# yang-song/score_sde_pytorch

Hardware: AMD Instinct MI355X
Metric: pc_sampler_images_per_sec (higher is better)
Workload: dtype f32 via 3-way bf16 split, fp32 accumulate (the 1x1 / NIN / Linear GEMMs and the attention forward as exact-fp32 products on the BF16 matrix pipe, fp32 softmax; 3x3 convolutions and the attention backward on the fp32-MFMA kernels); 1 GPU; configs/ve/cifar10_ncsnpp_continuous PC sampler (reverse_diffusion+langevin), batch 256/GPU, N=1000, 32x32; 1 step = 1 PC iteration = 2 U-Net evaluations; batch_per_gpu=256, sde_steps=1000, state_finite=True, matrix_mode=bf16x6, parallelism=replicas x1 (no collectives)

## Files before the change

### include/ssde.h

```cpp
#ifndef SSDE_H_
#define SSDE_H_

#include <stddef.h>
#include <stdint.h>

#ifdef __cplusplus
extern "C" {
#endif

#define SSDE_ABI_VERSION 13

enum {
  SSDE_PRO_NONE = 0,
  SSDE_PRO_GN = 1,
  SSDE_PRO_GN_SILU = 2,
  SSDE_PRO_SILU = 3
};

typedef struct ssde_src {
  const float* p0;
  const float* p1;
  int32_t c0, c1;
  int32_t pro_mode;
  int32_t gn_groups;
  const float* gn_mean;
  const float* gn_rstd;
  const float* gn_gamma;
  const float* gn_beta;
  uint32_t drop_thresh;
  float drop_scale;
  const uint32_t* drop_seed;
  uint32_t drop_salt;
  int32_t _pad;
} ssde_src;

typedef struct ssde_conv_args {
  ssde_src main;
  ssde_src aux;
  const float* w_main;
  const float* w_aux;
  int32_t n, h_in, w_in;
  int32_t h_out, w_out, c_out;
  int32_t ksize;
  int32_t stride;
  int32_t pad;
  int32_t tile;
  const float* bias;
  const float* chan_add;
  int32_t chan_add_ld;
  int32_t resid_post;
  const float* resid;
  float out_scale;
  uint32_t flags;
  float* dst;
  float* gn_part;
  float* wino_v;
  const float* gn_in_part0;
  const float* gn_in_part1;
  int32_t gn_in_slices0, gn_in_slices1;
  float gn_in_eps;
  int32_t pad_end;
  float* wino_ws;
  int64_t wino_ws_floats;
} ssde_conv_args;

enum { SSDE_CONVF_V_GIVEN = 1u,
       SSDE_CONVF_BF16X6 = 2u,
       SSDE_CONVF_NO_KSPLIT = 4u,
       SSDE_CONVF_BKC8 = 8u,
       SSDE_CONVF_GEMM_PIPE = 16u,
       SSDE_CONVF_NO_GEMM_PIPE = 32u,
       SSDE_CONVF_X6_BM64 = 64u,
       SSDE_CONVF_X6_PF2 = 128u,
       SSDE_CONVF_NO_SMALL_COUT = 256u,
       SSDE_CONVF_X6_WIDE = 512u,
       SSDE_CONVF_X6_NO_WIDE = 1024u,
       SSDE_CONVF_KSPLIT2 = 2048u,
       SSDE_CONVF_KSPLIT4 = 4096u };
enum { SSDE_TILE_AUTO = 0, SSDE_TILE_256x64 = 1, SSDE_TILE_128x64 = 2, SSDE_TILE_64x64 = 3, SSDE_TILE_256x32 = 4,
       SSDE_TILE_WINOGRAD = 5,
       SSDE_TILE_WINOGRAD4 = 6,
       SSDE_TILE_WINOGRAD4R = 9,
       SSDE_TILE_WINOGRAD4P = 10 };

typedef struct ssde_gn_stats_args {
  const float* p0; const float* p1; int32_t c0, c1;
  int32_t n, hw, groups; float eps;
  float* mean; float* rstd;
  float* scratch;
  int32_t slices;
  uint32_t flags;
} ssde_gn_stats_args;
enum { SSDE_GNSTATF_ANY_WIDTH = 1u };

typedef struct ssde_gn_apply_args {
  ssde_src src;
  int32_t n, hw;
  float* dst;
} ssde_gn_apply_args;

typedef struct ssde_gn_apply_bwd_args {
  ssde_src src;
  const float* dy;
  int32_t n, hw;
  float* sums;
  float* dgamma; float* dbeta;
  float* scratch;
  int32_t slices; int32_t _pad0;
  float* g0; float* g1;
  int32_t acc0, acc1;
} ssde_gn_apply_bwd_args;

typedef struct ssde_gn_finalize_args {
  const float* part0; const float* part1;
  int32_t c0, c1, slices0, slices1;
  int32_t n, groups; float eps; int32_t _pad0;
  float* mean; float* rstd;
} ssde_gn_finalize_args;

#define SSDE_FIR_MAX_TAPS 16
enum {
  SSDE_FIRF_GENERAL = 1,
  SSDE_FIRF_TILED = 2
};
typedef struct ssde_upfirdn_args {
  ssde_src src;
  int32_t n, h_in, w_in, c;
  int32_t h_out, w_out;
  int32_t up, down, pad0, pad1;
  int32_t kh, kw;
  float k[16];
  float* dst;
  int32_t accumulate;
  uint32_t flags;
  float* dst2;
  const float* taps;
} ssde_upfirdn_args;

#define SSDE_ATTN_L_MAX 16384
typedef struct ssde_attn_args {
  const float* qkv; float* dst;
  int32_t n, l, c; float scale;
  uint32_t flags;
  int32_t _pad0;
} ssde_attn_args;
enum { SSDE_ATTNF_BF16X6 = 1u,
       SSDE_ATTNF_STREAM = 2u };
enum { SSDE_ATTN_ROUTE_F32 = 0, SSDE_ATTN_ROUTE_X6 = 1, SSDE_ATTN_ROUTE_STREAM = 2 };

typedef struct ssde_embed_args {
  const float* cond;
  const float* w;
  float* dst;
  int32_t n, dim, kind, _pad0;
} ssde_embed_args;

typedef struct ssde_to_nhwc_args {
  const float* src; float* dst; int32_t n, c, h, w, c_pad; float a, b;
  int32_t mode;
  const float* v;
} ssde_to_nhwc_args;
typedef struct ssde_to_nchw_args {
  const float* src; float* dst; int32_t n, c, h, w, c_src;
  int32_t mode;
  const float* v;
  float alpha;
  int32_t accumulate;
} ssde_to_nchw_args;

typedef struct ssde_bias_act_args {
  const float* src; const float* bias; float* dst;
  int64_t numel; int32_t channels; int32_t inner;
  int32_t act;
  float alpha, scale;
  int32_t grad;
  const float* ref;
} ssde_bias_act_args;

typedef struct ssde_sumsq_args {
  const float* a; const float* b; float* out_a; float* out_b; int32_t n, per;
} ssde_sumsq_args;
typedef struct ssde_randn_args {
  float* dst; int64_t numel; uint64_t seed; const int32_t* step_ptr; int32_t stream_id; int32_t _pad0;
  const uint64_t* seed_ptr;
} ssde_randn_args;
typedef struct ssde_langevin_args {
  float* x; float* x_mean; const float* grad; const float* noise;
  const float* grad_sumsq; const float* noise_sumsq;
  const float* alpha_tab; const int32_t* step_ptr;
  int32_t n, per; float snr; int32_t _pad0;
} ssde_langevin_args;
typedef struct ssde_predictor_args {
  float* x; float* x_mean; const float* score; const float* noise;
  const float* coef; const int32_t* step_ptr;
  int64_t numel;
} ssde_predictor_args;
typedef struct ssde_sample_update_args {
  const float* x; const float* y; const float* z; const float* a; const float* b; const float* c;
  float* x_mean; float* x_out; int32_t n; int32_t per;
} ssde_sample_update_args;
typedef struct ssde_fill_args {
  float* dst; const float* tab; const int32_t* step_ptr; int32_t n; int32_t _pad0;
} ssde_fill_args;
typedef struct ssde_step_inc_args { int32_t* step_ptr; int32_t delta; int32_t _pad0; } ssde_step_inc_args;
typedef struct ssde_project_args {
  float* x; float* x_mean; const float* data; const float* mask; const float* noise;
  const float* coef; const int32_t* step_ptr;
  int32_t n, c, hw;
  int32_t use_matrix;
  float M[9], invM[9];
} ssde_project_args;



typedef struct ssde_wgrad_args {
  ssde_src src;
  const float* g;
  int32_t g_ld, g_off;
  int32_t n, h_in, w_in, h_out, w_out;
  int32_t c_out;
  int32_t ksize;
  int32_t stride, pad;
  int32_t cin_store;
  int32_t transpose_out;
  int32_t splits;
  float scale;
  uint32_t flags;
  float* dw;
  float* scratch;
  int64_t scratch_floats;
  const float* v_pre;
  int32_t pad_end;
  int32_t _pad0;
} ssde_wgrad_args;

enum { SSDE_WGRADF_DIRECT = 1u,
       SSDE_WGRADF_F2 = 2u,
       SSDE_WGRADF_F4_FORCE = 4u,
       SSDE_WGRADF_NO_STREAMK = 8u,
       SSDE_WGRADF_NO_XCD_ORDER = 16u,
       SSDE_WGRADF_1X1_CHUNKED = 32u,
       SSDE_WGRADF_XVEC1 = 64u };

typedef struct ssde_colsum_args {
  const float* g; int32_t g_ld, g_off;
  int32_t n, hw, c;
  float scale;
  float* per_sample;
  int32_t ps_ld, ps_off;
  float* total;
  float* total2;
  float* scratch;
  uint32_t flags;
  int32_t _pad0;
} ssde_colsum_args;
enum { SSDE_COLSUMF_DEFER = 1u };

#define SSDE_FINISH_JOBS 16
typedef struct ssde_colsum_job {
  const float* part;
  float* per_sample;
  float* total; float* total2;
  int32_t n, slices, c, ps_ld, ps_off, _pad0;
} ssde_colsum_job;
typedef struct ssde_colsum_finish_args { int32_t count, _pad0; ssde_colsum_job job[SSDE_FINISH_JOBS]; } ssde_colsum_finish_args;
typedef struct ssde_gn_bwd_job {
  const float* scratch;
  float* dgamma; float* dbeta;
  int32_t rows, c;
} ssde_gn_bwd_job;
typedef struct ssde_gn_bwd_finish_args { int32_t count, _pad0; ssde_gn_bwd_job job[SSDE_FINISH_JOBS]; } ssde_gn_bwd_finish_args;

typedef struct ssde_gn_bwd_reduce_args {
  ssde_src src;
  const float* dp;
  int32_t n, hw;
  float* sums;
  float* dgamma; float* dbeta;
  float* scratch;
  int32_t slices;
  uint32_t flags;
  float* g0; float* g1;
  int32_t acc0, acc1;
  float scale; int32_t _pad1;
} ssde_gn_bwd_reduce_args;

enum { SSDE_GNBWDF_THREE_KERNELS = 1u,
       SSDE_GNBWDF_DEFER_PARAMS = 2u };

typedef struct ssde_prologue_bwd_args {
  ssde_src src;
  const float* dp;
  int32_t dp_ld, dp_off;
  int32_t n, hw;
  const float* sums;
  float scale;
  int32_t acc0, acc1;
  float* g0; float* g1;
} ssde_prologue_bwd_args;

typedef struct ssde_attn_bwd_args {
  const float* qkv;
  const float* o;
  const float* d_o;
  float* dqkv;
  float* stats;
  int32_t n, l, c; float scale;
} ssde_attn_bwd_args;

typedef struct ssde_perturb_args {
  const float* x; const float* z; const float* a; const float* s; float* dst; int32_t n, per;
} ssde_perturb_args;
typedef struct ssde_dsm_loss_args {
  const float* score; const float* z; const float* s; const float* g2;
  float* dscore;
  float* losses;
  float* loss;
  int32_t n, per; int32_t reduce_mean; int32_t likelihood_weighting;
  float grad_scale;
  int32_t _pad0;
} ssde_dsm_loss_args;

typedef struct ssde_sumsq_flat_args { const float* x; int64_t numel; float* partial; float* out; } ssde_sumsq_flat_args;
typedef struct ssde_adam_args {
  float* p; const float* g; float* m; float* v; float* ema;
  int64_t numel;
  const float* hyper;
  const float* gnorm_sq;
} ssde_adam_args;

typedef struct ssde_memset_args { void* dst; int64_t bytes; int32_t value; int32_t _pad0; } ssde_memset_args;

enum { SSDE_PACK_CONV3 = 1, SSDE_PACK_WINO3 = 2, SSDE_PACK_MATRIX = 3, SSDE_PACK_VECTOR = 4,
       SSDE_PACK_WINO4 = 5 ,
       SSDE_PACK_WINO4R = 6 ,
       SSDE_PACK_WINO4P = 7  };
typedef struct ssde_pack_desc {
  const float* src;
  const float* src2;
  float* dst;
  int32_t kind;
  int32_t cout, cin;
  int32_t cout_l, cin_l;
  int32_t flags;
  int32_t r_off, c_off;
  int64_t n;
} ssde_pack_desc;
typedef struct ssde_pack_args { const ssde_pack_desc* table; int32_t count; int32_t kind; int64_t max_n; } ssde_pack_args;
typedef struct ssde_axpy_args {
  const float* x; const float* gate; float* dst; int64_t numel; float alpha; int32_t acc;
} ssde_axpy_args;

typedef struct ssde_rk_coefs { double v[7]; } ssde_rk_coefs;
typedef struct ssde_rk_combine_args {
  const double* y; const double* k; int64_t n; int32_t terms; int32_t _pad0; ssde_rk_coefs coef; double* dst; float* dst32;
  int64_t n32;
} ssde_rk_combine_args;
typedef struct ssde_rk_error_args {
  const double* y; const double* y_new; const double* k; int64_t n; ssde_rk_coefs coef; double atol, rtol;
  double* partial; int32_t partial_len; int32_t _pad0; double* out;
} ssde_rk_error_args;
#define SSDE_RK_MAX_TERMS 12
#define SSDE_RK_MAX_ROWS 13
typedef struct ssde_rk_combine_rows_args {
  const double* y; const double* k; int64_t n; int32_t terms; int32_t _pad0; double coef[SSDE_RK_MAX_TERMS]; double* dst; float* dst32;
  int64_t n32;
} ssde_rk_combine_rows_args;
typedef struct ssde_rk_error_rows_args {
  const double* y; const double* y_new; const double* k; int64_t n; int32_t rows; int32_t pair;
  double coef[SSDE_RK_MAX_ROWS]; double coef2[SSDE_RK_MAX_ROWS]; double h_abs; double atol, rtol;
  double* partial; int32_t partial_len; int32_t _pad0; double* out;
} ssde_rk_error_rows_args;
typedef struct ssde_ode_dyn {
  float label, std;
  float a, g2;
  double* dst;
} ssde_ode_dyn;
typedef struct ssde_pf_drift_args {
  const float* x; const float* score; double* dst; int64_t numel; float a, g2;
  const ssde_ode_dyn* dyn;
} ssde_pf_drift_args;
typedef struct ssde_hutch_div_args {
  const float* gx; const float* eps; double* dst; int64_t dst_off; int32_t n; int32_t per; float a, g2;
  const ssde_ode_dyn* dyn;
} ssde_hutch_div_args;

int ssde_conv2d(const ssde_conv_args* a, void* stream);
int ssde_groupnorm_stats(const ssde_gn_stats_args* a, void* stream);
int ssde_gn_finalize(const ssde_gn_finalize_args* a, void* stream);
int ssde_gn_apply(const ssde_gn_apply_args* a, void* stream);
int ssde_gn_apply_bwd(const ssde_gn_apply_bwd_args* a, void* stream);
int ssde_conv_gn_slices(const ssde_conv_args* a);
int64_t ssde_conv_ws_floats(const ssde_conv_args* a);
int ssde_upfirdn2d(const ssde_upfirdn_args* a, void* stream);
int ssde_attention(const ssde_attn_args* a, void* stream);
int ssde_attention_route(const ssde_attn_args* a);
int ssde_embed(const ssde_embed_args* a, void* stream);
int ssde_to_nhwc(const ssde_to_nhwc_args* a, void* stream);
int ssde_to_nchw(const ssde_to_nchw_args* a, void* stream);
int ssde_fused_bias_act(const ssde_bias_act_args* a, void* stream);
int ssde_sumsq(const ssde_sumsq_args* a, void* stream);
int ssde_randn(const ssde_randn_args* a, void* stream);
int ssde_langevin_update(const ssde_langevin_args* a, void* stream);
int ssde_predictor_update(const ssde_predictor_args* a, void* stream);
int ssde_sample_update(const ssde_sample_update_args* a, void* stream);
int ssde_fill_from_table(const ssde_fill_args* a, void* stream);
int ssde_step_inc(const ssde_step_inc_args* a, void* stream);
int ssde_project_update(const ssde_project_args* a, void* stream);
int ssde_rk_combine(const ssde_rk_combine_args* a, void* stream);
int ssde_rk_error_norm(const ssde_rk_error_args* a, void* stream);
int ssde_rk_combine_rows(const ssde_rk_combine_rows_args* a, void* stream);
int ssde_rk_error_norm_rows(const ssde_rk_error_rows_args* a, void* stream);
int ssde_pf_drift(const ssde_pf_drift_args* a, void* stream);
int ssde_hutch_div(const ssde_hutch_div_args* a, void* stream);
int ssde_conv_wgrad(const ssde_wgrad_args* a, void* stream);
int ssde_wgrad_wants_winograd4(const ssde_wgrad_args* a);
int ssde_colsum(const ssde_colsum_args* a, void* stream);
int ssde_colsum_finish(const ssde_colsum_finish_args* a, void* stream);
int ssde_gn_bwd_finish(const ssde_gn_bwd_finish_args* a, void* stream);
int ssde_gn_bwd_scratch_rows(const ssde_gn_bwd_reduce_args* a);
int ssde_gn_bwd_reduce(const ssde_gn_bwd_reduce_args* a, void* stream);
int ssde_prologue_bwd(const ssde_prologue_bwd_args* a, void* stream);
int ssde_attention_bwd(const ssde_attn_bwd_args* a, void* stream);
int ssde_perturb(const ssde_perturb_args* a, void* stream);
int ssde_dsm_loss(const ssde_dsm_loss_args* a, void* stream);
int ssde_sumsq_flat(const ssde_sumsq_flat_args* a, void* stream);
int ssde_adam_clip_ema(const ssde_adam_args* a, void* stream);
int ssde_memset(const ssde_memset_args* a, void* stream);
int ssde_axpy(const ssde_axpy_args* a, void* stream);
int ssde_pack_weights(const ssde_pack_args* a, void* stream);

enum {
  SSDE_OP_CONV = 1, SSDE_OP_GN_STATS = 2, SSDE_OP_UPFIRDN = 3, SSDE_OP_ATTN = 4, SSDE_OP_EMBED = 5,
  SSDE_OP_TO_NHWC = 6, SSDE_OP_TO_NCHW = 7, SSDE_OP_BIAS_ACT = 8, SSDE_OP_SUMSQ = 9, SSDE_OP_RANDN = 10,
  SSDE_OP_LANGEVIN = 11, SSDE_OP_PREDICTOR = 12, SSDE_OP_FILL = 13, SSDE_OP_STEP_INC = 14,
  SSDE_OP_WGRAD = 15, SSDE_OP_COLSUM = 16, SSDE_OP_GN_BWD_REDUCE = 17, SSDE_OP_PROLOGUE_BWD = 18,
  SSDE_OP_ATTN_BWD = 19, SSDE_OP_PERTURB = 20, SSDE_OP_DSM_LOSS = 21, SSDE_OP_SUMSQ_FLAT = 22,
  SSDE_OP_ADAM = 23, SSDE_OP_MEMSET = 24, SSDE_OP_AXPY = 25, SSDE_OP_PACK = 26, SSDE_OP_PROJECT = 27,
  SSDE_OP_GN_FINALIZE = 28, SSDE_OP_PF_DRIFT = 29, SSDE_OP_HUTCH_DIV = 30, SSDE_OP_COLSUM_FINISH = 31, SSDE_OP_GN_BWD_FINISH = 32,
  SSDE_OP_GN_APPLY = 33, SSDE_OP_GN_APPLY_BWD = 34
};
typedef struct ssde_op {
  int32_t kind; int32_t flops_class;
  union {
    ssde_conv_args conv; ssde_gn_stats_args gn; ssde_upfirdn_args fir; ssde_attn_args attn;
    ssde_embed_args embed; ssde_to_nhwc_args to_nhwc; ssde_to_nchw_args to_nchw;
    ssde_bias_act_args bias_act; ssde_sumsq_args sumsq; ssde_randn_args randn;
    ssde_langevin_args langevin; ssde_predictor_args predictor; ssde_fill_args fill;
    ssde_step_inc_args step_inc;
    ssde_wgrad_args wgrad; ssde_colsum_args colsum; ssde_gn_bwd_reduce_args gn_bwd; ssde_prologue_bwd_args pro_bwd;
    ssde_attn_bwd_args attn_bwd; ssde_perturb_args perturb; ssde_dsm_loss_args dsm_loss;
    ssde_sumsq_flat_args sumsq_flat; ssde_adam_args adam; ssde_memset_args memset; ssde_axpy_args axpy;
    ssde_pack_args pack; ssde_project_args project; ssde_gn_finalize_args gn_fin;
    ssde_pf_drift_args pf_drift; ssde_hutch_div_args hutch_div;
    ssde_colsum_finish_args colsum_fin; ssde_gn_bwd_finish_args gn_bwd_fin;
    ssde_gn_apply_args gn_apply; ssde_gn_apply_bwd_args gn_apply_bwd;
  } u;
} ssde_op;

int ssde_program_run(const ssde_op* ops, int32_t n_ops, void* stream);
int ssde_program_run_timed(const ssde_op* ops, int32_t n_ops, void* stream, float* ms);
int ssde_graph_capture(const ssde_op* ops, int32_t n_ops, void* stream, void** graph_out);
int ssde_graph_launch(void* graph, void* stream);
int ssde_graph_destroy(void* graph);

enum { SSDE_REGION_ZERO = 0,
       SSDE_REGION_CONST = 1 };
enum { SSDE_RELOC_OP = 0, SSDE_RELOC_REFRESH_OP = 1, SSDE_RELOC_REGION = 2 };
enum { SSDE_PLAN_UNET = 0, SSDE_PLAN_PC = 1, SSDE_PLAN_TRAIN = 2,
       SSDE_PLAN_ODE = 3,
       SSDE_PLAN_LIKELIHOOD = 4 };
enum { SSDE_IO_X = 0, SSDE_IO_COND = 1, SSDE_IO_SIGMA = 2, SSDE_IO_STD = 3, SSDE_IO_OUT = 4, SSDE_IO_XMEAN = 5,
       SSDE_IO_STEP = 6, SSDE_IO_SEED = 7,
       SSDE_IO_BATCH = 8, SSDE_IO_Z = 9, SSDE_IO_A = 10, SSDE_IO_S = 11, SSDE_IO_G2 = 12, SSDE_IO_LOSS = 13, SSDE_IO_HYPER = 14,
       SSDE_IO_DROP_SEED = 15, SSDE_IO_GOUT = 16, SSDE_IO_GX = 17, SSDE_IO_GRAD = 18, SSDE_IO_PARAMS = 19,
       SSDE_IO_ODE_DYN = 20, SSDE_IO_ODE_K = 21, SSDE_IO_ODE_STATE = 22, SSDE_IO_ODE_PROBE = 23, SSDE_IO_SLOTS = 24 };
#define SSDE_ODE_PARTIALS 1024
typedef struct ssde_plan_header {
  char magic[8];
  int32_t abi_version, sizeof_op;
  int32_t n_regions, n_ops, n_refresh_ops, n_relocs, n_params;
  int32_t kind;
  int32_t batch, channels, height, width;
  int32_t nfe_per_iteration;
  int32_t sde_steps;
  int32_t io[SSDE_IO_SLOTS];
  int32_t seg[4];
  int64_t n_flat;
  int64_t data_bytes;
// ... 50 lines not shown
```

### score_sde_pytorch_amd/_lib.py

```python
import ctypes as C
import os

_HERE = os.path.dirname(os.path.abspath(__file__))
LIB_PATH = os.environ.get("SSDE_LIB_PATH") or os.path.join(_HERE, "libssde_hip.so")
ABI_VERSION = 13

PRO_NONE, PRO_GN, PRO_GN_SILU, PRO_SILU = 0, 1, 2, 3
TILE_AUTO, TILE_256x64, TILE_128x64, TILE_64x64, TILE_256x32, TILE_WINOGRAD, TILE_WINOGRAD4 = 0, 1, 2, 3, 4, 5, 6
TILE_WINOGRAD4R = 9
TILE_WINOGRAD4P = 10
TILES_WINOGRAD4 = (TILE_WINOGRAD4, TILE_WINOGRAD4R, TILE_WINOGRAD4P)
CONVF_V_GIVEN, CONVF_BF16X6, CONVF_NO_KSPLIT, CONVF_BKC8, CONVF_GEMM_PIPE, CONVF_NO_GEMM_PIPE, CONVF_X6_BM64, CONVF_X6_PF2, \
    CONVF_NO_SMALL_COUT, CONVF_X6_WIDE, CONVF_X6_NO_WIDE, CONVF_KSPLIT2, CONVF_KSPLIT4 = 1, 2, 4, 8, 16, 32, 64, 128, 256, 512, 1024, 2048, 4096
WGRADF_DIRECT, WGRADF_F2, WGRADF_F4_FORCE, WGRADF_NO_STREAMK, WGRADF_NO_XCD_ORDER, WGRADF_1X1_CHUNKED, WGRADF_XVEC1 = 1, 2, 4, 8, 16, 32, 64
GNBWDF_THREE_KERNELS, GNBWDF_DEFER_PARAMS = 1, 2
(OP_CONV, OP_GN_STATS, OP_UPFIRDN, OP_ATTN, OP_EMBED, OP_TO_NHWC, OP_TO_NCHW, OP_BIAS_ACT, OP_SUMSQ,
 OP_RANDN, OP_LANGEVIN, OP_PREDICTOR, OP_FILL, OP_STEP_INC, OP_WGRAD, OP_COLSUM, OP_GN_BWD_REDUCE, OP_PROLOGUE_BWD,
 OP_ATTN_BWD, OP_PERTURB, OP_DSM_LOSS, OP_SUMSQ_FLAT, OP_ADAM, OP_MEMSET, OP_AXPY, OP_PACK, OP_PROJECT,
 OP_GN_FINALIZE, OP_PF_DRIFT, OP_HUTCH_DIV, OP_COLSUM_FINISH, OP_GN_BWD_FINISH, OP_GN_APPLY, OP_GN_APPLY_BWD) = range(1, 35)
GNSTATF_ANY_WIDTH = 1
FIRF_GENERAL, FIRF_TILED = 1, 2
FIR_MAX_TAPS = 16
FINISH_JOBS = 16
COLSUMF_DEFER = 1
PACK_CONV3, PACK_WINO3, PACK_MATRIX, PACK_VECTOR, PACK_WINO4, PACK_WINO4R, PACK_WINO4P = 1, 2, 3, 4, 5, 6, 7

_fp = C.c_void_p


class Src(C.Structure):
    _fields_ = [("p0", _fp), ("p1", _fp), ("c0", C.c_int32), ("c1", C.c_int32),
                ("pro_mode", C.c_int32), ("gn_groups", C.c_int32),
                ("gn_mean", _fp), ("gn_rstd", _fp), ("gn_gamma", _fp), ("gn_beta", _fp),
                ("drop_thresh", C.c_uint32), ("drop_scale", C.c_float), ("drop_seed", _fp),
                ("drop_salt", C.c_uint32), ("_pad", C.c_int32)]


class ConvArgs(C.Structure):
    _fields_ = [("main", Src), ("aux", Src), ("w_main", _fp), ("w_aux", _fp),
                ("n", C.c_int32), ("h_in", C.c_int32), ("w_in", C.c_int32),
                ("h_out", C.c_int32), ("w_out", C.c_int32), ("c_out", C.c_int32),
                ("ksize", C.c_int32), ("stride", C.c_int32), ("pad", C.c_int32), ("tile", C.c_int32),
                ("bias", _fp), ("chan_add", _fp), ("chan_add_ld", C.c_int32), ("resid_post", C.c_int32),
                ("resid", _fp), ("out_scale", C.c_float), ("flags", C.c_uint32), ("dst", _fp), ("gn_part", _fp), ("wino_v", _fp),
                ("gn_in_part0", _fp), ("gn_in_part1", _fp), ("gn_in_slices0", C.c_int32), ("gn_in_slices1", C.c_int32),
                ("gn_in_eps", C.c_float), ("pad_end", C.c_int32), ("wino_ws", _fp), ("wino_ws_floats", C.c_int64)]


class GnStatsArgs(C.Structure):
    _fields_ = [("p0", _fp), ("p1", _fp), ("c0", C.c_int32), ("c1", C.c_int32),
                ("n", C.c_int32), ("hw", C.c_int32), ("groups", C.c_int32), ("eps", C.c_float),
                ("mean", _fp), ("rstd", _fp), ("scratch", _fp), ("slices", C.c_int32), ("flags", C.c_uint32)]


class GnApplyArgs(C.Structure):
    _fields_ = [("src", Src), ("n", C.c_int32), ("hw", C.c_int32), ("dst", _fp)]


class GnApplyBwdArgs(C.Structure):
    _fields_ = [("src", Src), ("dy", _fp), ("n", C.c_int32), ("hw", C.c_int32), ("sums", _fp), ("dgamma", _fp), ("dbeta", _fp),
                ("scratch", _fp), ("slices", C.c_int32), ("_pad0", C.c_int32), ("g0", _fp), ("g1", _fp),
                ("acc0", C.c_int32), ("acc1", C.c_int32)]


class RkCombineArgs(C.Structure):
    _fields_ = [("y", _fp), ("k", _fp), ("n", C.c_int64), ("terms", C.c_int32), ("_pad0", C.c_int32), ("coef", C.c_double * 7),
                ("dst", _fp), ("dst32", _fp), ("n32", C.c_int64)]


class RkErrorArgs(C.Structure):
    _fields_ = [("y", _fp), ("y_new", _fp), ("k", _fp), ("n", C.c_int64), ("coef", C.c_double * 7), ("atol", C.c_double),
                ("rtol", C.c_double), ("partial", _fp), ("partial_len", C.c_int32), ("_pad0", C.c_int32), ("out", _fp)]


class RkCombineRowsArgs(C.Structure):
    _fields_ = [("y", _fp), ("k", _fp), ("n", C.c_int64), ("terms", C.c_int32), ("_pad0", C.c_int32), ("coef", C.c_double * 12),
                ("dst", _fp), ("dst32", _fp), ("n32", C.c_int64)]


class RkErrorRowsArgs(C.Structure):
    _fields_ = [("y", _fp), ("y_new", _fp), ("k", _fp), ("n", C.c_int64), ("rows", C.c_int32), ("pair", C.c_int32),
                ("coef", C.c_double * 13), ("coef2", C.c_double * 13), ("h_abs", C.c_double), ("atol", C.c_double), ("rtol", C.c_double),
                ("partial", _fp), ("partial_len", C.c_int32), ("_pad0", C.c_int32), ("out", _fp)]


class PfDriftArgs(C.Structure):
    _fields_ = [("x", _fp), ("score", _fp), ("dst", _fp), ("numel", C.c_int64), ("a", C.c_float), ("g2", C.c_float), ("dyn", _fp)]


class OdeDyn(C.Structure):
    _fields_ = [("label", C.c_float), ("std", C.c_float), ("a", C.c_float), ("g2", C.c_float), ("dst", _fp)]


class HutchDivArgs(C.Structure):
    _fields_ = [("gx", _fp), ("eps", _fp), ("dst", _fp), ("dst_off", C.c_int64), ("n", C.c_int32), ("per", C.c_int32),
                ("a", C.c_float), ("g2", C.c_float), ("dyn", _fp)]


class GnFinalizeArgs(C.Structure):
    _fields_ = [("part0", _fp), ("part1", _fp), ("c0", C.c_int32), ("c1", C.c_int32), ("slices0", C.c_int32), ("slices1", C.c_int32),
                ("n", C.c_int32), ("groups", C.c_int32), ("eps", C.c_float), ("_pad0", C.c_int32), ("mean", _fp), ("rstd", _fp)]


class UpfirdnArgs(C.Structure):
    _fields_ = [("src", Src), ("n", C.c_int32), ("h_in", C.c_int32), ("w_in", C.c_int32), ("c", C.c_int32),
                ("h_out", C.c_int32), ("w_out", C.c_int32),
                ("up", C.c_int32), ("down", C.c_int32), ("pad0", C.c_int32), ("pad1", C.c_int32),
                ("kh", C.c_int32), ("kw", C.c_int32), ("k", C.c_float * 16), ("dst", _fp),
                ("accumulate", C.c_int32), ("flags", C.c_uint32), ("dst2", _fp), ("taps", _fp)]


class AttnArgs(C.Structure):
    _fields_ = [("qkv", _fp), ("dst", _fp), ("n", C.c_int32), ("l", C.c_int32), ("c", C.c_int32), ("scale", C.c_float),
                ("flags", C.c_uint32), ("_pad0", C.c_int32)]


class EmbedArgs(C.Structure):
    _fields_ = [("cond", _fp), ("w", _fp), ("dst", _fp), ("n", C.c_int32), ("dim", C.c_int32),
                ("kind", C.c_int32), ("_pad0", C.c_int32)]


class ToNhwcArgs(C.Structure):
    _fields_ = [("src", _fp), ("dst", _fp), ("n", C.c_int32), ("c", C.c_int32), ("h", C.c_int32), ("w", C.c_int32),
                ("c_pad", C.c_int32), ("a", C.c_float), ("b", C.c_float), ("mode", C.c_int32), ("v", _fp)]


class ToNchwArgs(C.Structure):
    _fields_ = [("src", _fp), ("dst", _fp), ("n", C.c_int32), ("c", C.c_int32), ("h", C.c_int32), ("w", C.c_int32),
                ("c_src", C.c_int32), ("mode", C.c_int32), ("v", _fp), ("alpha", C.c_float), ("accumulate", C.c_int32)]


class BiasActArgs(C.Structure):
    _fields_ = [("src", _fp), ("bias", _fp), ("dst", _fp), ("numel", C.c_int64), ("channels", C.c_int32),
                ("inner", C.c_int32), ("act", C.c_int32), ("alpha", C.c_float), ("scale", C.c_float), ("grad", C.c_int32),
                ("ref", _fp)]


class SumsqArgs(C.Structure):
    _fields_ = [("a", _fp), ("b", _fp), ("out_a", _fp), ("out_b", _fp), ("n", C.c_int32), ("per", C.c_int32)]


class RandnArgs(C.Structure):
    _fields_ = [("dst", _fp), ("numel", C.c_int64), ("seed", C.c_uint64), ("step_ptr", _fp),
                ("stream_id", C.c_int32), ("_pad0", C.c_int32), ("seed_ptr", _fp)]


class LangevinArgs(C.Structure):
    _fields_ = [("x", _fp), ("x_mean", _fp), ("grad", _fp), ("noise", _fp), ("grad_sumsq", _fp), ("noise_sumsq", _fp),
                ("alpha_tab", _fp), ("step_ptr", _fp), ("n", C.c_int32), ("per", C.c_int32), ("snr", C.c_float),
                ("_pad0", C.c_int32)]


class PredictorArgs(C.Structure):
    _fields_ = [("x", _fp), ("x_mean", _fp), ("score", _fp), ("noise", _fp), ("coef", _fp), ("step_ptr", _fp),
                ("numel", C.c_int64)]


class SampleUpdateArgs(C.Structure):
    _fields_ = [("x", _fp), ("y", _fp), ("z", _fp), ("a", _fp), ("b", _fp), ("c", _fp), ("x_mean", _fp), ("x_out", _fp),
                ("n", C.c_int32), ("per", C.c_int32)]


class FillArgs(C.Structure):
    _fields_ = [("dst", _fp), ("tab", _fp), ("step_ptr", _fp), ("n", C.c_int32), ("_pad0", C.c_int32)]


class StepIncArgs(C.Structure):
    _fields_ = [("step_ptr", _fp), ("delta", C.c_int32), ("_pad0", C.c_int32)]


class ProjectArgs(C.Structure):
    _fields_ = [("x", _fp), ("x_mean", _fp), ("data", _fp), ("mask", _fp), ("noise", _fp), ("coef", _fp), ("step_ptr", _fp),
                ("n", C.c_int32), ("c", C.c_int32), ("hw", C.c_int32), ("use_matrix", C.c_int32),
                ("M", C.c_float * 9), ("invM", C.c_float * 9)]


class WgradArgs(C.Structure):
    _fields_ = [("src", Src), ("g", _fp), ("g_ld", C.c_int32), ("g_off", C.c_int32),
                ("n", C.c_int32), ("h_in", C.c_int32), ("w_in", C.c_int32), ("h_out", C.c_int32), ("w_out", C.c_int32),
                ("c_out", C.c_int32), ("ksize", C.c_int32), ("stride", C.c_int32), ("pad", C.c_int32),
                ("cin_store", C.c_int32), ("transpose_out", C.c_int32), ("splits", C.c_int32), ("scale", C.c_float),
                ("flags", C.c_uint32), ("dw", _fp), ("scratch", _fp), ("scratch_floats", C.c_int64), ("v_pre", _fp),
                ("pad_end", C.c_int32), ("_pad0", C.c_int32)]


class ColsumArgs(C.Structure):
    _fields_ = [("g", _fp), ("g_ld", C.c_int32), ("g_off", C.c_int32), ("n", C.c_int32), ("hw", C.c_int32),
                ("c", C.c_int32), ("scale", C.c_float), ("per_sample", _fp), ("ps_ld", C.c_int32), ("ps_off", C.c_int32),
                ("total", _fp), ("total2", _fp), ("scratch", _fp), ("flags", C.c_uint32), ("_pad0", C.c_int32)]


class ColsumJob(C.Structure):
    _fields_ = [("part", _fp), ("per_sample", _fp), ("total", _fp), ("total2", _fp), ("n", C.c_int32), ("slices", C.c_int32),
                ("c", C.c_int32), ("ps_ld", C.c_int32), ("ps_off", C.c_int32), ("_pad0", C.c_int32)]


class ColsumFinishArgs(C.Structure):
    _fields_ = [("count", C.c_int32), ("_pad0", C.c_int32), ("job", ColsumJob * FINISH_JOBS)]


class GnBwdJob(C.Structure):
    _fields_ = [("scratch", _fp), ("dgamma", _fp), ("dbeta", _fp), ("rows", C.c_int32), ("c", C.c_int32)]


class GnBwdFinishArgs(C.Structure):
    _fields_ = [("count", C.c_int32), ("_pad0", C.c_int32), ("job", GnBwdJob * FINISH_JOBS)]


class GnBwdReduceArgs(C.Structure):
    _fields_ = [("src", Src), ("dp", _fp), ("n", C.c_int32), ("hw", C.c_int32), ("sums", _fp),
                ("dgamma", _fp), ("dbeta", _fp), ("scratch", _fp), ("slices", C.c_int32), ("flags", C.c_uint32),
                ("g0", _fp), ("g1", _fp), ("acc0", C.c_int32), ("acc1", C.c_int32), ("scale", C.c_float), ("_pad1", C.c_int32)]


class PrologueBwdArgs(C.Structure):
    _fields_ = [("src", Src), ("dp", _fp), ("dp_ld", C.c_int32), ("dp_off", C.c_int32), ("n", C.c_int32), ("hw", C.c_int32),
                ("sums", _fp), ("scale", C.c_float), ("acc0", C.c_int32), ("acc1", C.c_int32), ("g0", _fp), ("g1", _fp)]


class AttnBwdArgs(C.Structure):
    _fields_ = [("qkv", _fp), ("o", _fp), ("d_o", _fp), ("dqkv", _fp), ("stats", _fp),
                ("n", C.c_int32), ("l", C.c_int32), ("c", C.c_int32), ("scale", C.c_float)]


class PerturbArgs(C.Structure):
    _fields_ = [("x", _fp), ("z", _fp), ("a", _fp), ("s", _fp), ("dst", _fp), ("n", C.c_int32), ("per", C.c_int32)]


class DsmLossArgs(C.Structure):
    _fields_ = [("score", _fp), ("z", _fp), ("s", _fp), ("g2", _fp), ("dscore", _fp), ("losses", _fp), ("loss", _fp),
                ("n", C.c_int32), ("per", C.c_int32), ("reduce_mean", C.c_int32), ("likelihood_weighting", C.c_int32),
                ("grad_scale", C.c_float), ("_pad0", C.c_int32)]


class SumsqFlatArgs(C.Structure):
    _fields_ = [("x", _fp), ("numel", C.c_int64), ("partial", _fp), ("out", _fp)]


class AdamArgs(C.Structure):
    _fields_ = [("p", _fp), ("g", _fp), ("m", _fp), ("v", _fp), ("ema", _fp), ("numel", C.c_int64),
                ("hyper", _fp), ("gnorm_sq", _fp)]


class MemsetArgs(C.Structure):
    _fields_ = [("dst", _fp), ("bytes", C.c_int64), ("value", C.c_int32), ("_pad0", C.c_int32)]


class AxpyArgs(C.Structure):
    _fields_ = [("x", _fp), ("gate", _fp), ("dst", _fp), ("numel", C.c_int64), ("alpha", C.c_float), ("acc", C.c_int32)]


class PackDesc(C.Structure):
    _fields_ = [("src", _fp), ("src2", _fp), ("dst", _fp), ("kind", C.c_int32), ("cout", C.c_int32), ("cin", C.c_int32),
                ("cout_l", C.c_int32), ("cin_l", C.c_int32), ("flags", C.c_int32), ("r_off", C.c_int32), ("c_off", C.c_int32),
                ("n", C.c_int64)]


class PackArgs(C.Structure):
    _fields_ = [("table", _fp), ("count", C.c_int32), ("kind", C.c_int32), ("max_n", C.c_int64)]


OPS = [(OP_CONV, "conv", ConvArgs, "ssde_conv2d"), (OP_GN_STATS, "gn", GnStatsArgs, "ssde_groupnorm_stats"),
       (OP_UPFIRDN, "fir", UpfirdnArgs, "ssde_upfirdn2d"), (OP_ATTN, "attn", AttnArgs, "ssde_attention"),
       (OP_EMBED, "embed", EmbedArgs, "ssde_embed"), (OP_TO_NHWC, "to_nhwc", ToNhwcArgs, "ssde_to_nhwc"),
       (OP_TO_NCHW, "to_nchw", ToNchwArgs, "ssde_to_nchw"), (OP_BIAS_ACT, "bias_act", BiasActArgs, "ssde_fused_bias_act"),
       (OP_SUMSQ, "sumsq", SumsqArgs, "ssde_sumsq"), (OP_RANDN, "randn", RandnArgs, "ssde_randn"),
       (OP_LANGEVIN, "langevin", LangevinArgs, "ssde_langevin_update"),
       (OP_PREDICTOR, "predictor", PredictorArgs, "ssde_predictor_update"), (OP_FILL, "fill", FillArgs, "ssde_fill_from_table"),
       (OP_STEP_INC, "step_inc", StepIncArgs, "ssde_step_inc"), (OP_WGRAD, "wgrad", WgradArgs, "ssde_conv_wgrad"),
       (OP_COLSUM, "colsum", ColsumArgs, "ssde_colsum"), (OP_GN_BWD_REDUCE, "gn_bwd", GnBwdReduceArgs, "ssde_gn_bwd_reduce"),
       (OP_PROLOGUE_BWD, "pro_bwd", PrologueBwdArgs, "ssde_prologue_bwd"), (OP_ATTN_BWD, "attn_bwd", AttnBwdArgs, "ssde_attention_bwd"),
       (OP_PERTURB, "perturb", PerturbArgs, "ssde_perturb"), (OP_DSM_LOSS, "dsm_loss", DsmLossArgs, "ssde_dsm_loss"),
       (OP_SUMSQ_FLAT, "sumsq_flat", SumsqFlatArgs, "ssde_sumsq_flat"), (OP_ADAM, "adam", AdamArgs, "ssde_adam_clip_ema"),
       (OP_MEMSET, "memset", MemsetArgs, "ssde_memset"), (OP_AXPY, "axpy", AxpyArgs, "ssde_axpy"),
       (OP_PACK, "pack", PackArgs, "ssde_pack_weights"), (OP_PROJECT, "project", ProjectArgs, "ssde_project_update"),
       (OP_GN_FINALIZE, "gn_fin", GnFinalizeArgs, "ssde_gn_finalize"), (OP_PF_DRIFT, "pf_drift", PfDriftArgs, "ssde_pf_drift"),
       (OP_HUTCH_DIV, "hutch_div", HutchDivArgs, "ssde_hutch_div"), (OP_COLSUM_FINISH, "colsum_fin", ColsumFinishArgs, "ssde_colsum_finish"),
       (OP_GN_BWD_FINISH, "gn_bwd_fin", GnBwdFinishArgs, "ssde_gn_bwd_finish"), (OP_GN_APPLY, "gn_apply", GnApplyArgs, "ssde_gn_apply"),
       (OP_GN_APPLY_BWD, "gn_apply_bwd", GnApplyBwdArgs, "ssde_gn_apply_bwd")]


class _OpUnion(C.Union):
    _fields_ = [(member, args) for _, member, args, _ in OPS]


class Op(C.Structure):
    _fields_ = [("kind", C.c_int32), ("flops_class", C.c_int32), ("u", _OpUnion)]


_UNION_FIELD = {kind: member for kind, member, _, _ in OPS}
ARGS = {kind: args for kind, _, args, _ in OPS}

EXPORTS = ["ssde_conv2d", "ssde_groupnorm_stats", "ssde_upfirdn2d", "ssde_attention", "ssde_attention_route", "ssde_embed", "ssde_to_nhwc",
           "ssde_to_nchw", "ssde_fused_bias_act", "ssde_sumsq", "ssde_randn", "ssde_langevin_update",
           "ssde_predictor_update", "ssde_fill_from_table", "ssde_step_inc", "ssde_program_run",
           "ssde_program_run_timed", "ssde_graph_capture", "ssde_graph_launch", "ssde_graph_destroy",
           "ssde_abi_version", "ssde_sizeof_op", "ssde_last_error", "ssde_conv_lds_bytes",
           "ssde_conv_wgrad", "ssde_colsum", "ssde_gn_bwd_reduce", "ssde_prologue_bwd", "ssde_attention_bwd",
           "ssde_perturb", "ssde_dsm_loss", "ssde_sumsq_flat", "ssde_adam_clip_ema", "ssde_memset", "ssde_axpy",
           "ssde_wgrad_scratch_floats", "ssde_wgrad_wants_winograd4", "ssde_pack_weights", "ssde_project_update", "ssde_gn_finalize", "ssde_conv_gn_slices", "ssde_conv_ws_floats", "ssde_rk_combine", "ssde_rk_error_norm", "ssde_rk_combine_rows", "ssde_rk_error_norm_rows", "ssde_pf_drift", "ssde_hutch_div", "ssde_sample_update", "ssde_mfma_probe", "ssde_colsum_finish", "ssde_gn_bwd_finish", "ssde_gn_bwd_scratch_rows",
           "ssde_gn_apply", "ssde_gn_apply_bwd",
           "ssde_plan_load", "ssde_plan_load_file", "ssde_plan_destroy", "ssde_plan_info", "ssde_plan_param",
           "ssde_plan_refresh_weights", "ssde_unet_forward", "ssde_pc_reset", "ssde_pc_run", "ssde_pc_state",
           "ssde_train_step", "ssde_train_forward", "ssde_unet_backward", "ssde_plan_copy_io",
           "ssde_ode_reset", "ssde_ode_eval", "ssde_ode_solve", "ssde_ode_solve_method", "ssde_ode_state"]

_lib = None


def conv_route_flags(env=None):
    e = os.environ if env is None else env
    f = 0
    if e.get("SSDE_MATRIX", "").startswith("b"):
        f |= CONVF_BF16X6
    if e.get("SSDE_CONV_KSPLIT", "1") == "0":
        f |= CONVF_NO_KSPLIT
    if e.get("SSDE_CONV_BKC64", "") == "8":
        f |= CONVF_BKC8
    if e.get("SSDE_GEMM_PIPE", "") == "0":
        f |= CONVF_NO_GEMM_PIPE
    if e.get("SSDE_GEMM_PIPE", "") == "2":
        f |= CONVF_GEMM_PIPE
    if e.get("SSDE_X6_BM", "") == "64":
        f |= CONVF_X6_BM64
    if e.get("SSDE_X6_PF", "") == "2":
        f |= CONVF_X6_PF2
    if e.get("SSDE_CONV_SMALL", "1") == "0":
        f |= CONVF_NO_SMALL_COUT
    if e.get("SSDE_X6_WIDE", "") == "1":
        f |= CONVF_X6_WIDE
    if e.get("SSDE_X6_WIDE", "") == "0":
        f |= CONVF_X6_NO_WIDE
    return f


ATTNF_BF16X6, ATTNF_STREAM = 1, 2
ATTN_ROUTE_F32, ATTN_ROUTE_X6, ATTN_ROUTE_STREAM = 0, 1, 2
ATTN_L_MAX = 16384


def attn_route_flags(env=None):
    e = os.environ if env is None else env
    x6 = ATTNF_BF16X6 if e.get("SSDE_MATRIX", "").startswith("b") and e.get("SSDE_ATTN_X6", "1") != "0" else 0
    return x6 | (ATTNF_STREAM if e.get("SSDE_ATTN_STREAM", "0") == "1" else 0)


def wgrad_route_flags(env=None):
    e = os.environ if env is None else env
    f = {"0": WGRADF_DIRECT, "2": WGRADF_F2, "44": WGRADF_F4_FORCE}.get(e.get("SSDE_WGRAD_WINOGRAD", ""), 0)
    if e.get("SSDE_WGRAD4_STREAMK", "1") == "0":
        f |= WGRADF_NO_STREAMK
    if e.get("SSDE_WGRAD4_XCD", "1") == "0":
        f |= WGRADF_NO_XCD_ORDER
    if e.get("SSDE_WGRAD_1X1_PIPELINED", "1") == "0":
        f |= WGRADF_1X1_CHUNKED
    if e.get("SSDE_WGRAD4_XVEC", "2") == "1":
        f |= WGRADF_XVEC1
    return f


def gn_bwd_route_flags(env=None):
    e = os.environ if env is None else env
    return GNBWDF_THREE_KERNELS if e.get("SSDE_GN_BWD_FUSED", "1") == "0" else 0


class SsdeError(RuntimeError):
    pass


def bind(lib):
    for name in EXPORTS:
        if not hasattr(lib, name):
            raise SsdeError("libssde_hip.so does not export %s" % name)
    lib.ssde_last_error.restype = C.c_char_p
    lib.ssde_program_run.argtypes = [C.POINTER(Op), C.c_int32, C.c_void_p]
    lib.ssde_program_run_timed.argtypes = [C.POINTER(Op), C.c_int32, C.c_void_p, C.POINTER(C.c_float)]
    lib.ssde_graph_capture.argtypes = [C.POINTER(Op), C.c_int32, C.c_void_p, C.POINTER(C.c_void_p)]
    lib.ssde_graph_launch.argtypes = [C.c_void_p, C.c_void_p]
    lib.ssde_graph_destroy.argtypes = [C.c_void_p]
    for _, _, typ, name in OPS:
        if name is not None:
            getattr(lib, name).argtypes = [C.POINTER(typ), C.c_void_p]
    lib.ssde_rk_combine.argtypes = [C.POINTER(RkCombineArgs), C.c_void_p]
    lib.ssde_rk_error_norm.argtypes = [C.POINTER(RkErrorArgs), C.c_void_p]
    lib.ssde_rk_combine_rows.argtypes = [C.POINTER(RkCombineRowsArgs), C.c_void_p]
    lib.ssde_rk_error_norm_rows.argtypes = [C.POINTER(RkErrorRowsArgs), C.c_void_p]
    lib.ssde_sample_update.argtypes = [C.POINTER(SampleUpdateArgs), C.c_void_p]
    lib.ssde_conv_lds_bytes.argtypes = [C.POINTER(ConvArgs)]
    lib.ssde_attention_route.argtypes = [C.POINTER(AttnArgs)]
    lib.ssde_conv_gn_slices.argtypes = [C.POINTER(ConvArgs)]
    lib.ssde_conv_ws_floats.argtypes = [C.POINTER(ConvArgs)]
    lib.ssde_conv_ws_floats.restype = C.c_int64
    lib.ssde_wgrad_scratch_floats.argtypes = [C.POINTER(WgradArgs)]
    lib.ssde_wgrad_scratch_floats.restype = C.c_int64
    lib.ssde_wgrad_wants_winograd4.argtypes = [C.POINTER(WgradArgs)]
    lib.ssde_gn_bwd_scratch_rows.argtypes = [C.POINTER(GnBwdReduceArgs)]
    if lib.ssde_abi_version() != ABI_VERSION:
        raise SsdeError("ABI mismatch: library %d, binding %d" % (lib.ssde_abi_version(), ABI_VERSION))
    if lib.ssde_sizeof_op() != C.sizeof(Op):
        raise SsdeError("struct layout mismatch: sizeof(ssde_op) library %d, ctypes %d" % (lib.ssde_sizeof_op(), C.sizeof(Op)))
    return lib


def load():
    global _lib
    if _lib is not None:
        return _lib
    if not os.path.exists(LIB_PATH):
        raise SsdeError(
            "libssde_hip.so not found at %s -- build it with `python -c 'import __graft_entry__ as g; g.build()'` "
            "(score_sde_pytorch_amd has no CPU/eager fallback)" % LIB_PATH)
    lib = bind(C.CDLL(LIB_PATH))
    _lib = lib
    return lib


def check(rc, what=""):
    if rc != 0:
        msg = load().ssde_last_error()
        raise SsdeError("%s failed (%d): %s" % (what or "libssde_hip call", rc, msg.decode() if msg else "?"))


def pointer_offsets(struct_cls, base=0):
    out = []
    for name, typ in struct_cls._fields_:
        off = base + getattr(struct_cls, name).offset
        if typ is C.c_void_p:
            out.append(off)
        elif isinstance(typ, type) and issubclass(typ, C.Structure):
            out.extend(pointer_offsets(typ, off))
        elif isinstance(typ, type) and issubclass(typ, C.Array) and issubclass(typ._type_, C.Structure):
            for i in range(typ._length_):
                out.extend(pointer_offsets(typ._type_, off + i * C.sizeof(typ._type_)))
    return out


_OP_PTRS = {}


def _op_pointer_offsets(kind):
    if kind not in _OP_PTRS:
        _OP_PTRS[kind] = pointer_offsets(ARGS[kind], Op.u.offset)
    return _OP_PTRS[kind]


def pointers_at(raw, offsets, base=0):
    for off in offsets:
        addr = int.from_bytes(raw[base + off:base + off + 8], "little")
        if addr:
            yield base + off, addr


def op_pointers(op):
    return pointers_at(bytes(op), _op_pointer_offsets(int(op.kind)))


def make_op(kind, args, flops_class=0):
    op = Op()
    op.kind = kind
    op.flops_class = flops_class
    setattr(op.u, _UNION_FIELD[kind], args)
    return op


def make(kind, **fields):
# ... 14 lines not shown
```

### score_sde_pytorch_amd/csrc/backward.hip

```cpp
#include "ssde_common.h"

namespace {

inline unsigned grid_for(size_t total, int block = 256, unsigned cap = 256 * 16) {
  size_t b = (total + block - 1) / block;
  if (b < 1) b = 1;
  return (unsigned)(b > cap ? cap : b);
}

__global__ __launch_bounds__(256) void colsum_kernel(const float* __restrict__ g, int g_ld, int g_off, int hw, int c,
                                                     float scale, float* __restrict__ out, int out_ld, int out_off) {
  SSDE_LDS(smem);
  float4* red = reinterpret_cast<float4*>(smem);
  const int n = blockIdx.z, slices = gridDim.y, slice = blockIdx.y;
  const int cl = blockIdx.x * 64 + (threadIdx.x & 63);
  const int pl = threadIdx.x >> 6;
  const int col = g_off + cl * 4;
  const int per_slice = (hw + slices - 1) / slices;
  const int p0 = slice * per_slice, p1 = min(hw, p0 + per_slice);
  float4 s = make_float4(0.f, 0.f, 0.f, 0.f);
  if (cl * 4 < c && col + 4 <= g_ld) {
    const float* base = g + (size_t)n * hw * g_ld + col;
    int px = p0 + pl;
    for (; px + 12 < p1; px += 16) {
// ... 743 lines not shown
}

extern "C" int ssde_sumsq_flat(const ssde_sumsq_flat_args* a, void* stream) {
  SSDE_REQUIRE(a && a->x && a->partial && a->out && a->numel > 0, "sumsq_flat: bad args (partial needs %d floats)", kSumsqBlocks);
  hipStream_t st = static_cast<hipStream_t>(stream);
  const int blocks = (int)grid_for((size_t)a->numel / 4, 256, kSumsqBlocks);
  hipLaunchKernelGGL(sumsq_partial_kernel, dim3(blocks), dim3(256), 64, st, a->x, (size_t)a->numel, a->partial);
  SSDE_LAUNCH_CHECK();
  hipLaunchKernelGGL(sumsq_final_kernel, dim3(1), dim3(256), 64, st, a->partial, blocks, a->out);
  SSDE_LAUNCH_CHECK();
  return SSDE_OK;
}

extern "C" int ssde_adam_clip_ema(const ssde_adam_args* a, void* stream) {
  SSDE_REQUIRE(a && a->p && a->g && a->m && a->v && a->hyper && a->numel > 0, "adam: bad args");
  hipLaunchKernelGGL(adam_kernel, dim3(grid_for((size_t)a->numel, 256, 256 * 32)), dim3(256), 0, static_cast<hipStream_t>(stream),
                     a->p, a->g, a->m, a->v, a->ema, (size_t)a->numel, a->hyper, a->gnorm_sq);
  SSDE_LAUNCH_CHECK();
  return SSDE_OK;
}

extern "C" int ssde_memset(const ssde_memset_args* a, void* stream) {
  SSDE_REQUIRE(a && a->dst && a->bytes >= 0, "memset: bad args");
  if (a->bytes == 0) return SSDE_OK;
  SSDE_HIP_CHECK(hipMemsetAsync(a->dst, a->value, (size_t)a->bytes, static_cast<hipStream_t>(stream)));
  return SSDE_OK;
}

extern "C" int ssde_axpy(const ssde_axpy_args* a, void* stream) {
  SSDE_REQUIRE(a && a->x && a->dst && a->numel > 0, "axpy: bad args");
  hipLaunchKernelGGL(axpy_kernel, dim3(grid_for((size_t)a->numel)), dim3(256), 0, static_cast<hipStream_t>(stream),
                     a->x, a->gate, a->dst, (size_t)a->numel, a->alpha, a->acc);
  SSDE_LAUNCH_CHECK();
  return SSDE_OK;
}

namespace {

__device__ __forceinline__ float pack_w3(const ssde_pack_desc& d, int co, int ci, int ky, int kx) {
  if (d.flags & 1) {
    if (ci >= d.cout || co >= d.cin) return 0.f;
    return d.src[((size_t)(ci * d.cin + co) * 3 + (2 - ky)) * 3 + (2 - kx)];
  }
  if (co >= d.cout || ci >= d.cin) return 0.f;
  return d.src[((size_t)(co * d.cin + ci) * 3 + ky) * 3 + kx];
}

__global__ __launch_bounds__(256) void pack_conv3_kernel(const ssde_pack_desc* __restrict__ table) {
  const ssde_pack_desc d = table[blockIdx.y];
  const int cpad = (d.cout_l + 63) / 64 * 64;
  for (size_t idx = (size_t)blockIdx.x * 256 + threadIdx.x; idx < (size_t)d.n; idx += (size_t)gridDim.x * 256) {
    const int e = (int)(idx & 7);
    const int co = (int)((idx >> 3) % cpad);
    const size_t r = (idx >> 3) / cpad;
    const int tap = (int)(r % 9), c8 = (int)(r / 9);
    d.dst[idx] = pack_w3(d, co, c8 * 8 + e, tap / 3, tap % 3);
  }
}

__global__ __launch_bounds__(256) void pack_wino3_kernel(const ssde_pack_desc* __restrict__ table) {
  const ssde_pack_desc d = table[blockIdx.y];
  const int ntl = (d.cout_l + 63) / 64;
  const float G[4][3] = {{1.f, 0.f, 0.f}, {0.5f, 0.5f, 0.5f}, {0.5f, -0.5f, 0.5f}, {0.f, 0.f, 1.f}};
  const size_t items = (size_t)d.n >> 5;
  for (size_t it = (size_t)blockIdx.x * 256 + threadIdx.x; it < items; it += (size_t)gridDim.x * 256) {
    const int cs = (int)(it & 63);
    const int q = (int)((it >> 6) & 3);
    const size_t r = it >> 8;
    const int nt = (int)(r % ntl), c8 = (int)(r / ntl);
    const int co = nt * 64 + (cs ^ ((q & 1) << 4));
    float u[2][16];
#pragma unroll
    for (int e = 0; e < 2; ++e) {
      const int ci = c8 * 8 + 2 * q + e;
      float w[3][3];
#pragma unroll
      for (int k = 0; k < 3; ++k)
#pragma unroll
        for (int l = 0; l < 3; ++l) w[k][l] = pack_w3(d, co, ci, k, l);
#pragma unroll
      for (int pa = 0; pa < 4; ++pa)
#pragma unroll
        for (int pb = 0; pb < 4; ++pb) {
          float acc = 0.f;
#pragma unroll
          for (int k = 0; k < 3; ++k) {
            float t = 0.f;
#pragma unroll
            for (int l = 0; l < 3; ++l) t += w[k][l] * G[pb][l];
            acc += G[pa][k] * t;
          }
          u[e][pa * 4 + pb] = acc;
        }
    }
#pragma unroll
    for (int pos = 0; pos < 16; ++pos)
      *reinterpret_cast<float2*>(d.dst + ((((r * 16 + pos) * 4 + q) * 64 + cs) << 1)) = make_float2(u[0][pos], u[1][pos]);
  }
}

template <int kForm>
__global__ __launch_bounds__(256) void pack_wino4_kernel(const ssde_pack_desc* __restrict__ table) {
  const ssde_pack_desc d = table[blockIdx.y];
  const int ntl = (d.cout_l + 63) / 64;
  const size_t nq = (size_t)d.n / ((size_t)36 * ntl * 256);
  const double G[6][3] = {{0.25, 0.0, 0.0}, {-1.0 / 6, -1.0 / 6, -1.0 / 6}, {-1.0 / 6, 1.0 / 6, -1.0 / 6},
                          {1.0 / 24, 1.0 / 12, 1.0 / 6}, {1.0 / 24, -1.0 / 12, 1.0 / 6}, {0.0, 0.0, 1.0}};
  const size_t items = (size_t)d.n / 36;
  for (size_t it = (size_t)blockIdx.x * 256 + threadIdx.x; it < items; it += (size_t)gridDim.x * 256) {
    const int e = (int)(it & 3), cs = (int)((it >> 2) & 63);
    const size_t r = it >> 8;
    const int nt = (int)(r % ntl), c4 = (int)(r / ntl);
    const int co = nt * 64 + cs, ci = c4 * 4 + e;
    double w[3][3], t[6][3];
#pragma unroll
    for (int k = 0; k < 3; ++k)
#pragma unroll
      for (int l = 0; l < 3; ++l) w[k][l] = (double)pack_w3(d, co, ci, k, l);
#pragma unroll
    for (int a = 0; a < 6; ++a)
#pragma unroll
      for (int l = 0; l < 3; ++l) t[a][l] = G[a][0] * w[0][l] + G[a][1] * w[1][l] + G[a][2] * w[2][l];
#pragma unroll
    for (int a = 0; a < 6; ++a)
#pragma unroll
      for (int b = 0; b < 6; ++b)
      {
        const int pos = a * 6 + b, wv = (pos & 3) * 2 + (cs >> 5), j = pos >> 2;
        const float u = (float)(t[a][0] * G[b][0] + t[a][1] * G[b][1] + t[a][2] * G[b][2]);
        if (kForm == 0) {
          d.dst[(((r * 8 + wv) * 9 + j) * 32 + (cs & 31)) * 4 + e] = u;
        } else if (kForm == 2) {
          d.dst[(((size_t)pos * nq + c4) * ((size_t)ntl * 64) + co) * 4 + e] = u;
        } else {
          const int lane = (e >> 1) * 32 + (cs & 31), half = cs >> 5;
          const int w = pos < 32 ? (pos >> 2) : 2 * (pos - 32) + half;
          const size_t base = (r * 8 + w) * (size_t)(9 * 32 * 4);
          d.dst[base + (pos < 32 ? ((pos & 3) * 64 + lane) * 4 + half * 2 + (e & 1) : 1024 + lane * 2 + (e & 1))] = u;
        }
      }
  }
}

__global__ __launch_bounds__(256) void pack_matrix_kernel(const ssde_pack_desc* __restrict__ table) {
  const ssde_pack_desc d = table[blockIdx.y];
  const int ld = (d.cout_l + 63) / 64 * 64;
  for (size_t idx = (size_t)blockIdx.x * 256 + threadIdx.x; idx < (size_t)d.n; idx += (size_t)gridDim.x * 256) {
    const int i = (int)(idx / d.cin), j = (int)(idx % d.cin);
    const int row = ((d.flags & 1) ? j : i) + d.r_off, col = ((d.flags & 1) ? i : j) + d.c_off;
    d.dst[((size_t)(col >> 3) * ld + row) * 8 + (col & 7)] = d.src[idx];
  }
}

__global__ __launch_bounds__(256) void pack_vector_kernel(const ssde_pack_desc* __restrict__ table) {
  const ssde_pack_desc d = table[blockIdx.y];
  for (size_t idx = (size_t)blockIdx.x * 256 + threadIdx.x; idx < (size_t)d.n; idx += (size_t)gridDim.x * 256)
    d.dst[d.r_off + idx] = d.src[idx] + (d.src2 ? d.src2[idx] : 0.f);
}

}

extern "C" int ssde_pack_weights(const ssde_pack_args* a, void* stream) {
  SSDE_REQUIRE(a && a->table && a->count > 0 && a->max_n > 0, "pack_weights: bad args");
  size_t bx = ((size_t)a->max_n + 255) / 256;
  if (bx > 256) bx = 256;
  const dim3 grid((unsigned)bx, (unsigned)a->count);
  hipStream_t st = static_cast<hipStream_t>(stream);
  switch (a->kind) {
    case SSDE_PACK_CONV3: hipLaunchKernelGGL(pack_conv3_kernel, grid, dim3(256), 0, st, a->table); break;
    case SSDE_PACK_WINO3: hipLaunchKernelGGL(pack_wino3_kernel, grid, dim3(256), 0, st, a->table); break;
    case SSDE_PACK_WINO4: hipLaunchKernelGGL(pack_wino4_kernel<0>, grid, dim3(256), 0, st, a->table); break;
    case SSDE_PACK_WINO4R: hipLaunchKernelGGL(pack_wino4_kernel<1>, grid, dim3(256), 0, st, a->table); break;
    case SSDE_PACK_WINO4P: hipLaunchKernelGGL(pack_wino4_kernel<2>, grid, dim3(256), 0, st, a->table); break;
    case SSDE_PACK_MATRIX: hipLaunchKernelGGL(pack_matrix_kernel, grid, dim3(256), 0, st, a->table); break;
    case SSDE_PACK_VECTOR: hipLaunchKernelGGL(pack_vector_kernel, grid, dim3(256), 0, st, a->table); break;
    default: ssde_set_error("pack_weights: unknown kind %d", a->kind); return SSDE_EINVAL;
  }
  SSDE_LAUNCH_CHECK();
  return SSDE_OK;
}
```

### score_sde_pytorch_amd/csrc/conv1x1.hip

```cpp
#include "ssde_common.h"

typedef float f32x16 __attribute__((ext_vector_type(16)));

#ifdef SSDE_GEMM_TRACE
__device__ unsigned long long* g_gemm_trace;
extern "C" int ssde_debug_gemm_trace(void* buf) {
  return hipMemcpyToSymbol(HIP_SYMBOL(g_gemm_trace), &buf, sizeof(buf)) == hipSuccess ? 0 : -5;
}
#define SSDE_GT(slot)                                                                  \
  do {                                                                                 \
    if (gt_on) g_gemm_trace[(slot)] = __builtin_amdgcn_s_memtime();                    \
  } while (0)
__device__ unsigned long long* g_gemm_wg_trace;
extern "C" int ssde_debug_gemm_wg_trace(void* buf) {
  return hipMemcpyToSymbol(HIP_SYMBOL(g_gemm_wg_trace), &buf, sizeof(buf)) == hipSuccess ? 0 : -5;
}
#define SSDE_GW(slot)                                                                                          \
  do {                                                                                                         \
    if (threadIdx.x == 0 && g_gemm_wg_trace != nullptr) {                                                      \
      g_gemm_wg_trace[(size_t)blockIdx.x * 4 + (slot)] = __builtin_amdgcn_s_memtime();                         \
      if ((slot) == 0) g_gemm_wg_trace[(size_t)blockIdx.x * 4 + 3] = __builtin_amdgcn_s_getreg((4 << 0) | (0 << 6) | (31 << 11)) | ((unsigned long long)__builtin_amdgcn_s_getreg((20 << 0) | (0 << 6) | (3 << 11)) << 32); \
    }                                                                                                          \
  } while (0)
#else
// ... 61 lines not shown
  }
  bool bok[NI];
#pragma unroll
  for (int i = 0; i < NI; ++i) bok[i] = (n0 + r0 + i * RS) < p.CoutPad;
  const float* bptr = p.wpk + ((size_t)n0 + r0) * 8 + (f & 1) * 4;

  float4 av[NI], bv[NI];
  float mu[NI], rs[NI];
  float4 gam = make_float4(1.f, 1.f, 1.f, 1.f), bet = make_float4(0.f, 0.f, 0.f, 0.f);
  bool k_ok = false;
  int c_cur = 0;

  auto load_stage = [&](int st) {
    const int c_base = st * BK;
    const bool second = c_base >= s.c0;
    const float* base = second ? s.p1 : s.p0;
    const int C = second ? s.c1 : s.c0;
    const int cthr = (second ? c_base - s.c0 : c_base) + f * 4;
    c_cur = c_base + f * 4;
    k_ok = c_cur < p.K;
    const float* ap = base + (k_ok ? cthr : 0);
#pragma unroll
    for (int i = 0; i < NI; ++i) av[i] = *reinterpret_cast<const float4*>(ap + (size_t)arow[i] * C);
    const int cin8 = min(st * 2 + (f >> 1), ncin8 - 1);
    const float* bp = bptr + (size_t)cin8 * p.CoutPad * 8;
#pragma unroll
    for (int i = 0; i < NI; ++i) bv[i] = *reinterpret_cast<const float4*>(bp + (bok[i] ? i * RS * 8 : 0));
    if (kGn) {
      const int cg = k_ok ? c_cur : 0;
      gam = *reinterpret_cast<const float4*>(s.gn_gamma + cg);
      bet = *reinterpret_cast<const float4*>(s.gn_beta + cg);
#pragma unroll
      for (int i = 0; i < NI; ++i) {
        const int gi = aimg[i] * s.gn_groups + cg / cpg;
        mu[i] = s.gn_mean[gi];
        rs[i] = s.gn_rstd[gi];
      }
    }
  };
  auto store_stage = [&](int st, float* buf) {
    const int cin8 = st * 2 + (f >> 1);
#pragma unroll
    for (int i = 0; i < NI; ++i) {
      float4 v = make_float4(0.f, 0.f, 0.f, 0.f);
      if (aok[i] && k_ok)
        v = ssde_pro_apply(av[i], mu[i], rs[i], gam, bet, (uint32_t)arow[i] * (uint32_t)Ctot + (uint32_t)c_cur, pro);
      float* d = buf + (r0 + i * RS) * LDK + f * 4;
      *reinterpret_cast<float2*>(d) = make_float2(v.x, v.y);
      *reinterpret_cast<float2*>(d + 2) = make_float2(v.z, v.w);
      float4 w = make_float4(0.f, 0.f, 0.f, 0.f);
      if (bok[i] && cin8 < ncin8) w = bv[i];
      float* e = buf + (BM + r0 + i * RS) * LDK + f * 4;
      *reinterpret_cast<float2*>(e) = make_float2(w.x, w.y);
      *reinterpret_cast<float2*>(e + 2) = make_float2(w.z, w.w);
    }
  };

  f32x16 acc[2][2];
#pragma unroll
  for (int a = 0; a < 2; ++a)
#pragma unroll
    for (int b = 0; b < 2; ++b)
#pragma unroll
      for (int r = 0; r < 16; ++r) acc[a][b][r] = 0.f;

  int aoff[2], boff[2];
#pragma unroll
  for (int a = 0; a < 2; ++a) aoff[a] = (wm0 + a * 32 + li) * LDK + 2 * lh;
#pragma unroll
  for (int b = 0; b < 2; ++b) boff[b] = (BM + wn0 + b * 32 + li) * LDK + 2 * lh;

  SSDE_GT(1);
  load_stage(0);
  store_stage(0, smem);
  __syncthreads();
  SSDE_GT(2);
  for (int st = 0; st < nst; ++st) {
    const float* cur = smem + (st & 1) * kStage;
    const bool has_next = st + 1 < nst;
    if (has_next) load_stage(st + 1);
    float2 af[2][2], bf[2][2];
#pragma unroll
    for (int a = 0; a < 2; ++a) af[0][a] = *reinterpret_cast<const float2*>(cur + aoff[a]);
#pragma unroll
    for (int b = 0; b < 2; ++b) bf[0][b] = *reinterpret_cast<const float2*>(cur + boff[b]);
#pragma unroll
    for (int t = 0; t < BK / 4; ++t) {
      const int c = t & 1;
      if (t + 1 < BK / 4) {
#pragma unroll
        for (int a = 0; a < 2; ++a) af[c ^ 1][a] = *reinterpret_cast<const float2*>(cur + aoff[a] + (t + 1) * 4);
#pragma unroll
        for (int b = 0; b < 2; ++b) bf[c ^ 1][b] = *reinterpret_cast<const float2*>(cur + boff[b] + (t + 1) * 4);
      }
#pragma unroll
      for (int a = 0; a < 2; ++a)
#pragma unroll
        for (int b = 0; b < 2; ++b) acc[a][b] = __builtin_amdgcn_mfma_f32_32x32x2f32(af[c][a].x, bf[c][b].x, acc[a][b], 0, 0, 0);
#pragma unroll
      for (int a = 0; a < 2; ++a)
#pragma unroll
        for (int b = 0; b < 2; ++b) acc[a][b] = __builtin_amdgcn_mfma_f32_32x32x2f32(af[c][a].y, bf[c][b].y, acc[a][b], 0, 0, 0);
      if (t + 1 < BK / 4) __builtin_amdgcn_sched_group_barrier(0x100, 4, 0);
      __builtin_amdgcn_sched_group_barrier(0x008, 8, 0);
    }
    if (st < 8) SSDE_GT(4 + st * 4);
    if (has_next) store_stage(st + 1, smem + ((st + 1) & 1) * kStage);
    if (st < 8) SSDE_GT(5 + st * 4);
    __syncthreads();
    if (st < 8) SSDE_GT(6 + st * 4);
  }
  SSDE_GT(40);

  constexpr int LDT = BN + 4;
  SsdeEpi e{p.bias, p.chan_add, p.chan_add_ld, p.resid, p.resid_post, p.scale, p.dst, p.Cout, p.gn_part};
#pragma unroll
  for (int half = 0; half < 2; ++half) {
    if ((wave >> 1) == half) {
#pragma unroll
      for (int b = 0; b < 2; ++b)
#pragma unroll
        for (int a = 0; a < 2; ++a)
#pragma unroll
          for (int r = 0; r < 16; ++r) {
            const int m = a * 32 + (r & 3) + 8 * (r >> 2) + 4 * lh;
            smem[m * LDT + wn0 + b * 32 + li] = acc[a][b][r];
          }
    }
    __syncthreads();
    ssde_store_tile<64, BN, kThreads, SSDE_GEMM_BATCH>(smem, LDT, n0, e, [&](int row, size_t& pix, int& img) {
      const int m = m0 + half * 64 + row;
      if (m >= p.M) return false;
      pix = (size_t)m;
      img = m / p.HW;
      return true;
    }, p.gn_part ? (p.HW >= 64 ? (m0 >> 6) + half : (m0 + half * 64) / p.HW) : -1, p.HW >= 64 ? 30 : p.lHW, p.gn_entries);
    SSDE_GT(41 + half * 2);
    __syncthreads();
    SSDE_GT(42 + half * 2);
  }
}

#ifndef SSDE_X6_PF2_OCC_LOSS
#define SSDE_X6_PF2_OCC_LOSS 1
#endif
constexpr int XBK = 16;
template <int kBM, int kBN = 128> struct X6 {
  static constexpr int kPlaneA = kBM * XBK * 2, kPlaneB = kBN * XBK * 2;
  static constexpr int kStageBytes = 3 * kPlaneA + 3 * kPlaneB;
  static constexpr int NA = kBM / 64;
  static constexpr int NBW = kBN / 64;
};

template <bool kGn, int kBM, int kPF, int kBN = 128>
__global__ __launch_bounds__(kThreads, kBN == 256 ? 2 : (kBM == 64 ? 4 : 3) - (kPF == 2 ? SSDE_X6_PF2_OCC_LOSS : 0)) void gemm1x1_bf16x6_kernel(const GemmParams p) {
  using X = X6<kBM, kBN>;
  constexpr int NA = X::NA, NB = X::NBW, NBW = X::NBW, RS = 64;
  SSDE_LDS(smem);
  char* lds = reinterpret_cast<char*>(smem);
  const int tid = threadIdx.x, wave = tid >> 6, lane = tid & 63;
  const int li = lane & 31, lh = lane >> 5;
  const int xcd = blockIdx.x & 7, lin = blockIdx.x >> 3;
  const int nt = lin % p.n_tiles, mt = (lin / p.n_tiles) * 8 + xcd;
#ifdef SSDE_GEMM_TRACE
  const bool gt_on = tid == 0 && blockIdx.x == 0 && g_gemm_trace != nullptr;
#endif
  SSDE_GT(0);
  if (mt >= p.m_tiles) return;
  SSDE_GW(0);
  const int m0 = mt * kBM, n0 = nt * kBN;
  const int wm0 = (wave >> 1) * (kBM / 2), wn0 = (wave & 1) * (kBN / 2);
  const ssde_src& s = p.src;
  SsdePro pro = ssde_pro_decode(s);
  pro.gn = kGn;
  const int Ctot = s.c0 + s.c1;
  const int cpg = kGn ? Ctot / s.gn_groups : 1;
  const int nst = (p.K + XBK - 1) / XBK;
  const int ncin8 = (p.K + 7) >> 3;

  const int f = tid & 3, r0 = tid >> 2;
  int arow[NA], aimg[NA];
  bool aok[NA];
#pragma unroll
  for (int i = 0; i < NA; ++i) {
    const int m = m0 + r0 + i * RS;
    aok[i] = m < p.M;
    arow[i] = aok[i] ? m : 0;
    aimg[i] = arow[i] / p.HW;
  }
  bool bok[NB];
#pragma unroll
  for (int i = 0; i < NB; ++i) bok[i] = (n0 + r0 + i * RS) < p.CoutPad;
  const float* bptr = p.wpk + ((size_t)n0 + r0) * 8 + (f & 1) * 4;

  struct ARegs { float4 av[NA]; };
  struct StageRegs {
    float4 bv[NB];
    float mu[NA], rs[NA];
    float4 gam, bet;
  };
  auto load_a = [&](int st, ARegs& A) __attribute__((always_inline)) {
    const int c_base = st * XBK;
    const bool second = c_base >= s.c0;
    const float* base = second ? s.p1 : s.p0;
    const int C = second ? s.c1 : s.c0;
    const int cthr = (second ? c_base - s.c0 : c_base) + f * 4;
    const float* ap = base + (c_base + f * 4 < p.K ? cthr : 0);
#pragma unroll
    for (int i = 0; i < NA; ++i) A.av[i] = *reinterpret_cast<const float4*>(ap + (size_t)arow[i] * C);
  };
  auto load_rest = [&](int st, StageRegs& R) __attribute__((always_inline)) {
    const int c_cur = st * XBK + f * 4;
    const int cin8 = min(st * 2 + (f >> 1), ncin8 - 1);
    const float* bp = bptr + (size_t)cin8 * p.CoutPad * 8;
#pragma unroll
    for (int i = 0; i < NB; ++i) R.bv[i] = *reinterpret_cast<const float4*>(bp + (bok[i] ? i * RS * 8 : 0));
    R.gam = make_float4(1.f, 1.f, 1.f, 1.f); R.bet = make_float4(0.f, 0.f, 0.f, 0.f);
#pragma unroll
    for (int i = 0; i < NA; ++i) { R.mu[i] = 0.f; R.rs[i] = 1.f; }
    if (kGn) {
      const int cg = c_cur < p.K ? c_cur : 0;
      R.gam = *reinterpret_cast<const float4*>(s.gn_gamma + cg);
      R.bet = *reinterpret_cast<const float4*>(s.gn_beta + cg);
#pragma unroll
      for (int i = 0; i < NA; ++i) {
        const int gi = aimg[i] * s.gn_groups + cg / cpg;
        R.mu[i] = s.gn_mean[gi];
        R.rs[i] = s.gn_rstd[gi];
      }
    }
  };
  auto store_stage = [&](int st, const ARegs& A, const StageRegs& R, char* buf) __attribute__((always_inline)) {
    const int cin8 = st * 2 + (f >> 1);
    const int c_cur = st * XBK + f * 4;
    const bool k_ok = c_cur < p.K;
    uint2 q0, q1, q2;
#pragma unroll
    for (int i = 0; i < NA; ++i) {
      float4 v = make_float4(0.f, 0.f, 0.f, 0.f);
      if (aok[i] && k_ok)
        v = ssde_pro_apply(A.av[i], R.mu[i], R.rs[i], R.gam, R.bet, (uint32_t)arow[i] * (uint32_t)Ctot + (uint32_t)c_cur, pro);
      char* d = buf + (r0 + i * RS) * (XBK * 2) + f * 8;
      ssde_split3(v, q0, q1, q2);
      *reinterpret_cast<uint2*>(d) = q0;
      *reinterpret_cast<uint2*>(d + X::kPlaneA) = q1;
      *reinterpret_cast<uint2*>(d + 2 * X::kPlaneA) = q2;
    }
#pragma unroll
    for (int i = 0; i < NB; ++i) {
      float4 w = make_float4(0.f, 0.f, 0.f, 0.f);
      if (bok[i] && cin8 < ncin8) w = R.bv[i];
      char* d = buf + 3 * X::kPlaneA + (r0 + i * RS) * (XBK * 2) + f * 8;
      ssde_split3(w, q0, q1, q2);
      *reinterpret_cast<uint2*>(d) = q0;
      *reinterpret_cast<uint2*>(d + X::kPlaneB) = q1;
      *reinterpret_cast<uint2*>(d + 2 * X::kPlaneB) = q2;
    }
  };

  f32x16 acc[NA][NBW];
#pragma unroll
  for (int a = 0; a < NA; ++a)
#pragma unroll
    for (int b = 0; b < NBW; ++b)
#pragma unroll
      for (int r = 0; r < 16; ++r) acc[a][b][r] = 0.f;
  const int aoff = (wm0 + li) * (XBK * 2) + lh * 16, boff = 3 * X::kPlaneA + (wn0 + li) * (XBK * 2) + lh * 16;
  auto mfma_stage = [&](const char* cur) __attribute__((always_inline)) {
    ssde_u32x4 A[NA][3];
#pragma unroll
    for (int q = 0; q < 3; ++q)
#pragma unroll
      for (int a = 0; a < NA; ++a) A[a][q] = *reinterpret_cast<const ssde_u32x4*>(cur + aoff + q * X::kPlaneA + a * 32 * (XBK * 2));
    constexpr int TI[6] = {0, 2, 1, 0, 1, 0}, TJ[6] = {2, 0, 1, 1, 0, 0};
#pragma unroll
    for (int b0 = 0; b0 < NBW; b0 += 2) {
      ssde_u32x4 B[2][3];
#pragma unroll
      for (int q = 0; q < 3; ++q)
#pragma unroll
        for (int b = 0; b < 2; ++b) B[b][q] = *reinterpret_cast<const ssde_u32x4*>(cur + boff + q * X::kPlaneB + (b0 + b) * 32 * (XBK * 2));
#pragma unroll
      for (int t = 0; t < 6; ++t)
#pragma unroll
        for (int a = 0; a < NA; ++a)
#pragma unroll
          for (int b = 0; b < 2; ++b)
            acc[a][b0 + b] = __builtin_amdgcn_mfma_f32_32x32x16_bf16(__builtin_bit_cast(ssde_bf16x8, A[a][TI[t]]),
                                                                     __builtin_bit_cast(ssde_bf16x8, B[b][TJ[t]]), acc[a][b0 + b], 0, 0, 0);
    }
  };

  SSDE_GT(1);
  char* buf0 = lds;
  char* buf1 = lds + X::kStageBytes;
  StageRegs R;
  if constexpr (kPF == 1) {
    ARegs A0;
    load_a(0, A0); load_rest(0, R);
    store_stage(0, A0, R, buf0);
    __syncthreads();
    SSDE_GT(2);
    for (int st = 0; st < nst; ++st) {
      const bool has_next = st + 1 < nst;
      if (has_next) { load_a(st + 1, A0); load_rest(st + 1, R); }
      mfma_stage((st & 1) ? buf1 : buf0);
      if (st < 8) SSDE_GT(4 + st * 4);
      if (has_next) store_stage(st + 1, A0, R, (st & 1) ? buf0 : buf1);
      if (st < 8) SSDE_GT(5 + st * 4);
      __syncthreads();
      if (st < 8) SSDE_GT(6 + st * 4);
    }
  } else {
    ARegs A0, A1;
    const int last = nst - 1;
    load_a(0, A0); load_rest(0, R);
    load_a(min(1, last), A1);
    store_stage(0, A0, R, buf0);
    __syncthreads();
    SSDE_GT(2);
    for (int st = 0; st < nst; st += 2) {
      load_rest(min(st + 1, last), R);
      __builtin_amdgcn_sched_barrier(0);
      load_a(min(st + 2, last), A0);
      __builtin_amdgcn_sched_barrier(0);
      mfma_stage(buf0);
      if (st < 8) SSDE_GT(4 + st * 4);
      if (st + 1 < nst) store_stage(st + 1, A1, R, buf1);
      if (st < 8) SSDE_GT(5 + st * 4);
      __syncthreads();
      if (st < 8) SSDE_GT(6 + st * 4);
      if (st + 1 >= nst) break;
      load_rest(min(st + 2, last), R);
      __builtin_amdgcn_sched_barrier(0);
      load_a(min(st + 3, last), A1);
      __builtin_amdgcn_sched_barrier(0);
      mfma_stage(buf1);
      if (st + 1 < 8) SSDE_GT(4 + (st + 1) * 4);
      if (st + 2 < nst) store_stage(st + 2, A0, R, buf0);
      if (st + 1 < 8) SSDE_GT(5 + (st + 1) * 4);
      __syncthreads();
      if (st + 1 < 8) SSDE_GT(6 + (st + 1) * 4);
    }
  }
  SSDE_GT(40);
  SSDE_GW(1);

  constexpr int LDT = kBN + 4;
  SsdeEpi e{p.bias, p.chan_add, p.chan_add_ld, p.resid, p.resid_post, p.scale, p.dst, p.Cout, p.gn_part};
#pragma unroll
  for (int half = 0; half < kBM / 64; ++half) {
    if (kBM == 64 || (wave >> 1) == half) {
#pragma unroll
      for (int b = 0; b < NBW; ++b)
#pragma unroll
        for (int a = 0; a < NA; ++a)
#pragma unroll
          for (int r = 0; r < 16; ++r) {
            const int m = (kBM == 64 ? wm0 : 0) + a * 32 + (r & 3) + 8 * (r >> 2) + 4 * lh;
            smem[m * LDT + wn0 + b * 32 + li] = acc[a][b][r];
          }
    }
    __syncthreads();
    ssde_store_tile<64, kBN, kThreads, SSDE_GEMM_BATCH>(smem, LDT, n0, e, [&](int row, size_t& pix, int& img) {
      const int m = m0 + half * 64 + row;
      if (m >= p.M) return false;
      pix = (size_t)m;
      img = m / p.HW;
      return true;
    }, p.gn_part ? (p.HW >= 64 ? (m0 >> 6) + half : (m0 + half * 64) / p.HW) : -1, p.HW >= 64 ? 30 : p.lHW, p.gn_entries);
    SSDE_GT(41 + half * 2);
    __syncthreads();
    SSDE_GT(42 + half * 2);
  }
  SSDE_GW(2);
}

constexpr int kSlabLd = 68;
constexpr int kSlabFloats = 8 * kSlabLd;

template <bool kGn, bool kX6>
__global__ __launch_bounds__(kThreads, 2) void gemm1x1_pipe_kernel(const GemmParams p) {
  SSDE_LDS(smem);
  constexpr int kStageB = kX6 ? X6<128>::kStageBytes : kStage * 4;
  constexpr int KB = 16;
  char* lds = reinterpret_cast<char*>(smem);
  const int tid = threadIdx.x, wave = tid >> 6, lane = tid & 63;
  const int li = lane & 31, lh = lane >> 5;
  float* slab = reinterpret_cast<float*>(lds + 2 * kStageB) + wave * kSlabFloats;
  const int wm0 = (wave >> 1) * 64, wn0 = (wave & 1) * 64;
  const ssde_src& s = p.src;
  SsdePro pro = ssde_pro_decode(s);
  pro.gn = kGn;
  const int Ctot = s.c0 + s.c1;
  const int cpg = kGn ? Ctot / s.gn_groups : 1;
  const int nst = (p.K + KB - 1) / KB;
  const int ncin8 = (p.K + 7) >> 3;
  const int f = tid & 3, r0 = tid >> 2;
  constexpr int NI = 2, RS = 64;
  const int d_row = lane >> 4, d_c4 = lane & 15;

  struct Pending {
    int m0, n0, done;
    bool valid;
    float4 bias4;
    float4 rnext[2];
    float st_p, st_s1, st_s2, st_n;
  };
  Pending pd;
  pd.valid = false; pd.done = 8; pd.m0 = pd.n0 = 0;
  pd.bias4 = make_float4(0.f, 0.f, 0.f, 0.f);
  pd.rnext[0] = pd.rnext[1] = make_float4(0.f, 0.f, 0.f, 0.f);
  pd.st_p = pd.st_s1 = pd.st_s2 = pd.st_n = 0.f;

  auto unit_row = [&](int u, int k) {
    int r = wm0 + (u >> 2) * 32 + (u & 3) * 8 + d_row;
    SSDE_OPAQUE_VGPR(r);
    return r + 4 * k;
  };
  auto fetch_resid = [&](int u) __attribute__((always_inline)) {
#pragma unroll
    for (int k = 0; k < 2; ++k) {
      const int m = pd.m0 + unit_row(u, k), j = pd.n0 + wn0 + d_c4 * 4;
      pd.rnext[k] = make_float4(0.f, 0.f, 0.f, 0.f);
      if (p.resid && u < 8 && m < p.M && j < p.Cout) pd.rnext[k] = *reinterpret_cast<const float4*>(p.resid + (size_t)m * p.Cout + j);
    }
  };
  auto drain_unit = [&](auto A_, auto Q_, f32x16 (&acc)[2][2]) __attribute__((always_inline)) {
    constexpr int a = decltype(A_)::value, q = decltype(Q_)::value, u = a * 4 + q;
    const float4 rr[2] = {pd.rnext[0], pd.rnext[1]};
    fetch_resid(u + 1);
    SSDE_WAVE_SYNC();
#pragma unroll
    for (int b = 0; b < 2; ++b)
#pragma unroll
      for (int r = 0; r < 4; ++r) slab[(r + 4 * lh) * kSlabLd + b * 32 + li] = acc[a][b][4 * q + r];
    SSDE_WAVE_SYNC();
    const int j = pd.n0 + wn0 + d_c4 * 4;
    const int img = p.chan_add ? (pd.m0 + unit_row(u, 0) - d_row) / p.HW : 0;
#pragma unroll
    for (int k = 0; k < 2; ++k) {
      const float4 t = *reinterpret_cast<const float4*>(slab + (d_row + 4 * k) * kSlabLd + d_c4 * 4);
      const int m = pd.m0 + unit_row(u, k);
      if (m < p.M && j < p.Cout) {
        float4 ca = make_float4(0.f, 0.f, 0.f, 0.f);
        if (p.chan_add) ca = *reinterpret_cast<const float4*>(p.chan_add + (size_t)img * p.chan_add_ld + j);
        float v[4] = {t.x + pd.bias4.x + ca.x, t.y + pd.bias4.y + ca.y, t.z + pd.bias4.z + ca.z, t.w + pd.bias4.w + ca.w};
        if (!p.resid_post) { v[0] += rr[k].x; v[1] += rr[k].y; v[2] += rr[k].z; v[3] += rr[k].w; }
#pragma unroll
        for (int e = 0; e < 4; ++e) v[e] *= p.scale;
        if (p.resid_post) { v[0] += rr[k].x; v[1] += rr[k].y; v[2] += rr[k].z; v[3] += rr[k].w; }
        *reinterpret_cast<float4*>(p.dst + (size_t)m * p.Cout + j) = make_float4(v[0], v[1], v[2], v[3]);
        if (p.gn_part) {
          if (pd.st_n == 0.f) pd.st_p = v[0];
          const float d0 = v[0] - pd.st_p, d1 = v[1] - pd.st_p, d2 = v[2] - pd.st_p, d3 = v[3] - pd.st_p;
          pd.st_s1 += (d0 + d1) + (d2 + d3);
          pd.st_s2 += (d0 * d0 + d1 * d1) + (d2 * d2 + d3 * d3);
          pd.st_n += 4.f;
        }
      }
    }
  };
  auto drain_next = [&](f32x16 (&acc)[2][2]) __attribute__((always_inline)) {
    using std::integral_constant;
    switch (pd.done) {
      case 0: drain_unit(integral_constant<int, 0>{}, integral_constant<int, 0>{}, acc); break;
      case 1: drain_unit(integral_constant<int, 0>{}, integral_constant<int, 1>{}, acc); break;
      case 2: drain_unit(integral_constant<int, 0>{}, integral_constant<int, 2>{}, acc); break;
      case 3: drain_unit(integral_constant<int, 0>{}, integral_constant<int, 3>{}, acc); break;
      case 4: drain_unit(integral_constant<int, 1>{}, integral_constant<int, 0>{}, acc); break;
      case 5: drain_unit(integral_constant<int, 1>{}, integral_constant<int, 1>{}, acc); break;
      case 6: drain_unit(integral_constant<int, 1>{}, integral_constant<int, 2>{}, acc); break;
      default: drain_unit(integral_constant<int, 1>{}, integral_constant<int, 3>{}, acc); break;
    }
    ++pd.done;
  };
  auto finish_tile = [&](f32x16 (&acc)[2][2]) __attribute__((always_inline)) {
    while (pd.done < 8) drain_next(acc);
    if (p.gn_part) {
      float n = pd.st_n, m = 0.f, M2 = 0.f;
      if (n > 0.f) { const float rn = __builtin_amdgcn_rcpf(n); m = pd.st_p + pd.st_s1 * rn; M2 = pd.st_s2 - pd.st_s1 * pd.st_s1 * rn; M2 = M2 < 0.f ? 0.f : M2; }
      for (int o = 16; o < 64; o <<= 1) {
        const float nb = __shfl_xor(n, o, 64), mb = __shfl_xor(m, o, 64), Mb = __shfl_xor(M2, o, 64);
        if (lane & o) { float tn = nb, tm = mb, tM = Mb; ssde_stat_merge(tn, tm, tM, n, m, M2); n = tn; m = tm; M2 = tM; }
        else ssde_stat_merge(n, m, M2, nb, mb, Mb);
      }
      const int entry = (pd.m0 + wm0) >> 6, j = pd.n0 + wn0 + 4 * lane;
      if (lane < 16 && j < p.Cout && entry < p.gn_entries) {
#pragma unroll
        for (int slot = 0; slot < 4; ++slot) {
          float* o = p.gn_part + (((size_t)entry * 4 + slot) * (p.Cout >> 2) + (j >> 2)) * 3;
          o[0] = slot == 0 ? m : 0.f; o[1] = slot == 0 ? M2 : 0.f; o[2] = slot == 0 ? n : 0.f;
        }
      }
    }
    pd.valid = false;
  };

  auto run_tile = [&](int vb, f32x16 (&acc)[2][2], f32x16 (&old)[2][2]) __attribute__((always_inline)) {
    const int xcd = vb & 7, lin = vb >> 3;
    const int nt = lin % p.n_tiles, mt = (lin / p.n_tiles) * 8 + xcd;
    const int m0 = mt * BM, n0 = nt * BN;
    int arow[NI], aimg[NI];
    bool aok[NI], bok[NI];
#pragma unroll
    for (int i = 0; i < NI; ++i) {
      const int m = m0 + r0 + i * RS;
      aok[i] = m < p.M;
      arow[i] = aok[i] ? m : 0;
      aimg[i] = arow[i] / p.HW;
      bok[i] = (n0 + r0 + i * RS) < p.CoutPad;
    }
    const float* bptr = p.wpk + ((size_t)n0 + r0) * 8 + (f & 1) * 4;
    float4 av[NI], bv[NI];
    float mu[NI] = {0.f, 0.f}, rs[NI] = {1.f, 1.f};
    float4 gam = make_float4(1.f, 1.f, 1.f, 1.f), bet = make_float4(0.f, 0.f, 0.f, 0.f);
    auto load_stage = [&](int st) __attribute__((always_inline)) {
      const int c_base = st * KB;
      const bool second = c_base >= s.c0;
      const float* base = second ? s.p1 : s.p0;
      const int C = second ? s.c1 : s.c0;
      const int cthr = (second ? c_base - s.c0 : c_base) + f * 4;
      const int c_cur = c_base + f * 4;
      const float* ap = base + (c_cur < p.K ? cthr : 0);
#pragma unroll
      for (int i = 0; i < NI; ++i) av[i] = *reinterpret_cast<const float4*>(ap + (size_t)arow[i] * C);
      const int cin8 = min(st * 2 + (f >> 1), ncin8 - 1);
      const float* bp = bptr + (size_t)cin8 * p.CoutPad * 8;
#pragma unroll
      for (int i = 0; i < NI; ++i) bv[i] = *reinterpret_cast<const float4*>(bp + (bok[i] ? i * RS * 8 : 0));
      if (kGn) {
        const int cg = c_cur < p.K ? c_cur : 0;
        gam = *reinterpret_cast<const float4*>(s.gn_gamma + cg);
        bet = *reinterpret_cast<const float4*>(s.gn_beta + cg);
#pragma unroll
        for (int i = 0; i < NI; ++i) {
          const int gi = aimg[i] * s.gn_groups + cg / cpg;
          mu[i] = s.gn_mean[gi];
          rs[i] = s.gn_rstd[gi];
        }
      }
    };
    auto store_stage = [&](int st, char* buf) __attribute__((always_inline)) {
      const int cin8 = st * 2 + (f >> 1), c_cur = st * KB + f * 4;
      const bool k_ok = c_cur < p.K;
#pragma unroll
      for (int i = 0; i < NI; ++i) {
        float4 v = make_float4(0.f, 0.f, 0.f, 0.f);
        if (aok[i] && k_ok)
          v = ssde_pro_apply(av[i], mu[i], rs[i], gam, bet, (uint32_t)arow[i] * (uint32_t)Ctot + (uint32_t)c_cur, pro);
        float4 w = make_float4(0.f, 0.f, 0.f, 0.f);
        if (bok[i] && cin8 < ncin8) w = bv[i];
        if constexpr (kX6) {
          using X = X6<128>;
          uint2 q0, q1, q2;
          char* d = buf + (r0 + i * RS) * (KB * 2) + f * 8;
          ssde_split3(v, q0, q1, q2);
          *reinterpret_cast<uint2*>(d) = q0;
          *reinterpret_cast<uint2*>(d + X::kPlaneA) = q1;
          *reinterpret_cast<uint2*>(d + 2 * X::kPlaneA) = q2;
          ssde_split3(w, q0, q1, q2);
          *reinterpret_cast<uint2*>(d + 3 * X::kPlaneA) = q0;
          *reinterpret_cast<uint2*>(d + 3 * X::kPlaneA + X::kPlaneB) = q1;
          *reinterpret_cast<uint2*>(d + 3 * X::kPlaneA + 2 * X::kPlaneB) = q2;
        } else {
          float* fb = reinterpret_cast<float*>(buf);
          float* d = fb + (r0 + i * RS) * LDK + f * 4;
          *reinterpret_cast<float2*>(d) = make_float2(v.x, v.y);
          *reinterpret_cast<float2*>(d + 2) = make_float2(v.z, v.w);
          float* e = fb + (BM + r0 + i * RS) * LDK + f * 4;
          *reinterpret_cast<float2*>(e) = make_float2(w.x, w.y);
          *reinterpret_cast<float2*>(e + 2) = make_float2(w.z, w.w);
        }
      }
    };
    auto mfma_stage = [&](const char* cur) __attribute__((always_inline)) {
      if constexpr (kX6) {
        using X = X6<128>;
        const int aoff = (wm0 + li) * (KB * 2) + lh * 16, boff = 3 * X::kPlaneA + (wn0 + li) * (KB * 2) + lh * 16;
        ssde_u32x4 A[2][3], B[2][3];
#pragma unroll
        for (int q = 0; q < 3; ++q)
#pragma unroll
          for (int a = 0; a < 2; ++a) {
            A[a][q] = *reinterpret_cast<const ssde_u32x4*>(cur + aoff + q * X::kPlaneA + a * 32 * (KB * 2));
            B[a][q] = *reinterpret_cast<const ssde_u32x4*>(cur + boff + q * X::kPlaneB + a * 32 * (KB * 2));
          }
        constexpr int TI[6] = {0, 2, 1, 0, 1, 0}, TJ[6] = {2, 0, 1, 1, 0, 0};
#pragma unroll
        for (int t = 0; t < 6; ++t)
#pragma unroll
          for (int a = 0; a < 2; ++a)
#pragma unroll
            for (int b = 0; b < 2; ++b)
              acc[a][b] = __builtin_amdgcn_mfma_f32_32x32x16_bf16(__builtin_bit_cast(ssde_bf16x8, A[a][TI[t]]),
                                                                  __builtin_bit_cast(ssde_bf16x8, B[b][TJ[t]]), acc[a][b], 0, 0, 0);
      } else {
        const float* cf = reinterpret_cast<const float*>(cur);
        int aoff[2], boff[2];
#pragma unroll
        for (int a = 0; a < 2; ++a) { aoff[a] = (wm0 + a * 32 + li) * LDK + 2 * lh; boff[a] = (BM + wn0 + a * 32 + li) * LDK + 2 * lh; }
        float2 af[2][2], bf[2][2];
#pragma unroll
        for (int a = 0; a < 2; ++a) { af[0][a] = *reinterpret_cast<const float2*>(cf + aoff[a]); bf[0][a] = *reinterpret_cast<const float2*>(cf + boff[a]); }
#pragma unroll
        for (int t = 0; t < KB / 4; ++t) {
          const int c = t & 1;
          if (t + 1 < KB / 4) {
#pragma unroll
            for (int a = 0; a < 2; ++a) {
              af[c ^ 1][a] = *reinterpret_cast<const float2*>(cf + aoff[a] + (t + 1) * 4);
              bf[c ^ 1][a] = *reinterpret_cast<const float2*>(cf + boff[a] + (t + 1) * 4);
            }
          }
#pragma unroll
          for (int a = 0; a < 2; ++a)
#pragma unroll
            for (int b = 0; b < 2; ++b) acc[a][b] = __builtin_amdgcn_mfma_f32_32x32x2f32(af[c][a].x, bf[c][b].x, acc[a][b], 0, 0, 0);
#pragma unroll
          for (int a = 0; a < 2; ++a)
#pragma unroll
            for (int b = 0; b < 2; ++b) acc[a][b] = __builtin_amdgcn_mfma_f32_32x32x2f32(af[c][a].y, bf[c][b].y, acc[a][b], 0, 0, 0);
        }
      }
    };
#pragma unroll
    for (int a = 0; a < 2; ++a)
#pragma unroll
      for (int b = 0; b < 2; ++b)
#pragma unroll
        for (int r = 0; r < 16; ++r) acc[a][b][r] = 0.f;
    char* buf0 = lds;
    char* buf1 = lds + kStageB;
    load_stage(0);
    store_stage(0, buf0);
    __syncthreads();
    for (int st = 0; st < nst; ++st) {
      const bool has_next = st + 1 < nst;
      if (has_next) load_stage(st + 1);
      mfma_stage((st & 1) ? buf1 : buf0);
      if (pd.valid) {
        const int target = ((st + 1) * 8 + nst - 1) / nst;
        while (pd.done < target && pd.done < 8) drain_next(old);
      }
      if (has_next) store_stage(st + 1, (st & 1) ? buf0 : buf1);
      __syncthreads();
    }
    if (pd.valid) finish_tile(old);
    pd.valid = true; pd.done = 0; pd.m0 = m0; pd.n0 = n0;
    pd.st_p = pd.st_s1 = pd.st_s2 = pd.st_n = 0.f;
    pd.bias4 = make_float4(0.f, 0.f, 0.f, 0.f);
    const int j = n0 + wn0 + d_c4 * 4;
    if (p.bias && j < p.Cout) pd.bias4 = *reinterpret_cast<const float4*>(p.bias + j);
    fetch_resid(0);
  };

  f32x16 acc[2][2], old[2][2];
  const int total_vb = ((p.m_tiles + 7) / 8) * 8 * p.n_tiles;
  for (int vb = blockIdx.x; vb < total_vb; vb += gridDim.x) {
    if (((vb >> 3) / p.n_tiles) * 8 + (vb & 7) >= p.m_tiles) continue;
    run_tile(vb, acc, old);
#pragma unroll
    for (int a = 0; a < 2; ++a)
#pragma unroll
      for (int b = 0; b < 2; ++b) old[a][b] = acc[a][b];
  }
  if (pd.valid) finish_tile(old);
}

struct GemmPlan {
  GemmParams p;
  bool gn, x6, pipe;
  int xbm, xpf, xbn;
  int grid;
};

int gemm_plan(const ssde_conv_args* a, GemmPlan* g, ssde_conv_plan* pl) {
  const ssde_src& s = a->aux;
  if (int rc = ssde_src_check(s, "conv1x1", "", 32, SSDE_SRC_GN)) return rc;
  g->gn = s.pro_mode == SSDE_PRO_GN || s.pro_mode == SSDE_PRO_GN_SILU;
  SSDE_REQUIRE(a->w_aux && a->dst, "conv1x1: null weights / destination");
  GemmParams& p = g->p;
  p.src = s; p.wpk = a->w_aux;
  p.M = a->n * a->h_out * a->w_out; p.HW = a->h_out * a->w_out; p.K = s.c0 + s.c1;
  p.Cout = a->c_out; p.CoutPad = ssde_cdiv(a->c_out, 64) * 64;
  p.m_tiles = ssde_cdiv(p.M, BM); p.n_tiles = ssde_cdiv(a->c_out, BN);
  ssde_fill_epilogue(p, a);
  const bool gn_ok = a->c_out % 4 == 0 && (p.HW % 64 == 0 || (p.HW >= 8 && p.HW < 64 && 64 % p.HW == 0));
  SSDE_REQUIRE(!a->gn_part || gn_ok, "conv1x1: GroupNorm partials need H*W %% 64 == 0 or a power of two in 8..32");
  pl->gn_slices = !gn_ok ? 0 : p.HW % 64 == 0 ? (p.HW / 64) * 4 : 4;
  pl->ws_floats = 0;
  p.lHW = ssde_ilog2(p.HW);
  p.gn_entries = p.HW >= 64 ? a->n * (p.HW / 64) : a->n;
  const bool x6 = g->x6 = (a->flags & SSDE_CONVF_BF16X6) != 0;
  {
    const int total = ssde_cdiv(p.m_tiles, 8) * 8 * p.n_tiles;
    const int wgs = (2 * ssde_num_cus() + 7) / 8 * 8;
    const bool pipe_ok = !(a->flags & SSDE_CONVF_NO_GEMM_PIPE) && a->c_out % 4 == 0 && (!a->gn_part || p.HW % 64 == 0) && (!a->chan_add || p.HW % 8 == 0);
    const bool wide_first = a->c_out >= 512 && a->c_out % 256 == 0 && !(a->flags & (SSDE_CONVF_X6_NO_WIDE | SSDE_CONVF_X6_BM64 | SSDE_CONVF_X6_PF2)) &&
                            (long long)ssde_cdiv(p.M, 128) * (a->c_out / 256) >= 2ll * ssde_num_cus();
    const bool pays = x6 && p.K >= 512 && (long long)p.m_tiles * p.n_tiles > wgs && !wide_first;
    g->pipe = pipe_ok && x6 && (pays || (a->flags & SSDE_CONVF_GEMM_PIPE));
    if (g->pipe) {
      pl->lds_bytes = 2 * X6<128>::kStageBytes + 4 * kSlabFloats * 4;
      g->grid = total < wgs ? total : wgs;
      return SSDE_OK;
    }
  }
  int xbm = 128, xpf = 1, xbn = BN;
  if (x6) {
    if (a->flags & SSDE_CONVF_X6_BM64) xbm = 64;
    if (a->flags & SSDE_CONVF_X6_PF2) xpf = 2;
    if ((long long)ssde_cdiv(p.M, 128) * ssde_cdiv(a->c_out, BN) <= ssde_num_cus() && !(a->flags & SSDE_CONVF_X6_WIDE)) xbm = 64;
    const bool wide_fits = a->c_out % 256 == 0 && xbm == 128 && xpf == 1;
    const bool wide_pays = (long long)ssde_cdiv(p.M, 128) * (a->c_out / 256) >= 2ll * ssde_num_cus();
    if (!(a->flags & SSDE_CONVF_X6_NO_WIDE) && wide_fits && (wide_pays || (a->flags & SSDE_CONVF_X6_WIDE))) xbn = 256;
    p.m_tiles = ssde_cdiv(p.M, xbm);
    p.n_tiles = ssde_cdiv(a->c_out, xbn);
  }
  g->xbm = xbm; g->xpf = xpf; g->xbn = xbn;
  const int lds_ops = x6 ? 2 * (xbn == 256 ? X6<128, 256>::kStageBytes : xbm == 64 ? X6<64>::kStageBytes : X6<128>::kStageBytes) : 2 * kStage * 4;
  const int lds_epi = 64 * (xbn + 4) * 4;
  pl->lds_bytes = lds_ops > lds_epi ? lds_ops : lds_epi;
  g->grid = ssde_cdiv(p.m_tiles, 8) * 8 * p.n_tiles;
  return SSDE_OK;
}

template <auto Kfn>
int gemm_go(const GemmPlan& g, int lds, hipStream_t st) {
  return ssde_launch_lds<Kfn>("conv1x1", dim3(g.grid), dim3(kThreads), lds, st, g.p);
}

}

bool ssde_conv1x1_wants(const ssde_conv_args* a) {
  if (a->ksize != 0 || a->aux.p0 == nullptr || a->tile != SSDE_TILE_AUTO) return false;
  const long long M = (long long)a->n * a->h_out * a->w_out;
  return a->c_out >= 96 && M >= 128 && M < (1ll << 31);
}

int ssde_conv1x1_plan(const ssde_conv_args* a, ssde_conv_plan* pl) {
  GemmPlan g;
  return gemm_plan(a, &g, pl);
}

int ssde_conv1x1_launch(const ssde_conv_args* a, hipStream_t st) {
  GemmPlan g;
  ssde_conv_plan pl;
  if (int rc = gemm_plan(a, &g, &pl)) return rc;
  const int lds = pl.lds_bytes;
  const bool gn = g.gn;
  if (g.pipe) return gn ? gemm_go<gemm1x1_pipe_kernel<true, true>>(g, lds, st) : gemm_go<gemm1x1_pipe_kernel<false, true>>(g, lds, st);
  if (!g.x6) return gn ? gemm_go<gemm1x1_kernel<true>>(g, lds, st) : gemm_go<gemm1x1_kernel<false>>(g, lds, st);
  if (g.xbn == 256) return gn ? gemm_go<gemm1x1_bf16x6_kernel<true, 128, 1, 256>>(g, lds, st) : gemm_go<gemm1x1_bf16x6_kernel<false, 128, 1, 256>>(g, lds, st);
  if (g.xbm == 128 && g.xpf == 1) return gn ? gemm_go<gemm1x1_bf16x6_kernel<true, 128, 1>>(g, lds, st) : gemm_go<gemm1x1_bf16x6_kernel<false, 128, 1>>(g, lds, st);
  if (g.xbm == 128) return gn ? gemm_go<gemm1x1_bf16x6_kernel<true, 128, 2>>(g, lds, st) : gemm_go<gemm1x1_bf16x6_kernel<false, 128, 2>>(g, lds, st);
  if (g.xpf == 1) return gn ? gemm_go<gemm1x1_bf16x6_kernel<true, 64, 1>>(g, lds, st) : gemm_go<gemm1x1_bf16x6_kernel<false, 64, 1>>(g, lds, st);
  return gn ? gemm_go<gemm1x1_bf16x6_kernel<true, 64, 2>>(g, lds, st) : gemm_go<gemm1x1_bf16x6_kernel<false, 64, 2>>(g, lds, st);
}
```

### score_sde_pytorch_amd/csrc/conv_mfma.hip

```cpp
#include "ssde_common.h"

typedef float f32x16 __attribute__((ext_vector_type(16)));

namespace {

struct ConvGeom {
  int N, Hin, Win, Hout, Wout, Cout, CoutPad;
  int stride, pad;
  int lTW, lTH;
  int tiles_x, tiles_per_img;
  int m_tiles, n_tiles;
};

struct ConvKParams {
  ssde_src main, aux;
  const float* w_main;
  const float* w_aux;
  ConvGeom g;
  const float* bias;
  const float* chan_add;
  int chan_add_ld;
  const float* resid;
  int resid_post;
  float scale;
// ... 321 lines not shown
  int gn_slices;
};

int halo_px(int bm, int w_out, int h_out, int stride, int ks, int* lTW, int* lTH) {
  int tw = ssde_pow2_floor(w_out < 16 ? w_out : 16);
  int th = bm / tw; if (th > h_out) th = h_out;
  th = ssde_pow2_floor(th);
  *lTW = ssde_ilog2(tw); *lTH = ssde_ilog2(th);
  const int imgs = bm / (tw * th);
  return imgs * ((th - 1) * stride + ks) * ((tw - 1) * stride + ks);
}

int make_plan(const ssde_conv_args* a, ConvPlan* pl) {
  SSDE_REQUIRE(a && a->dst, "conv: null args");
  pl->has3 = a->ksize != 0;
  pl->has1 = a->aux.p0 != nullptr;
  SSDE_REQUIRE(pl->has3 || pl->has1, "conv: neither a k x k nor a 1 x 1 source");
  SSDE_REQUIRE(a->ksize == 0 || a->ksize == 3, "conv: ksize must be 0 or 3 (1x1 goes through aux)");
  SSDE_REQUIRE(a->n > 0 && a->h_out > 0 && a->w_out > 0 && a->c_out > 0, "conv: bad output shape");
  if (pl->has3) {
    if (int rc = ssde_src_check(a->main, "conv", "main ", 32, SSDE_SRC_NEEDS_C0 | SSDE_SRC_GN)) return rc;
    SSDE_REQUIRE(a->w_main, "conv: w_main missing");
    SSDE_REQUIRE(a->stride == 1 || a->stride == 2, "conv: stride must be 1 or 2");
    SSDE_REQUIRE(a->pad_end == 0 || a->pad_end == 1, "conv: pad_end must be 0 or 1 (got %d)", a->pad_end);
    SSDE_REQUIRE((a->h_in + 2 * a->pad + a->pad_end - 3) / a->stride + 1 >= a->h_out &&
                 (a->w_in + 2 * a->pad + a->pad_end - 3) / a->stride + 1 >= a->w_out,
                 "conv: output %dx%d larger than input %dx%d stride %d pad %d pad_end %d allows", a->h_out, a->w_out, a->h_in, a->w_in,
                 a->stride, a->pad, a->pad_end);
  }
  if (pl->has1) {
    if (int rc = ssde_src_check(a->aux, "conv", "aux ", 32, SSDE_SRC_NEEDS_C0 | SSDE_SRC_GN)) return rc;
    SSDE_REQUIRE(a->w_aux, "conv: w_aux missing");
  }
  const int M = a->n * a->h_out * a->w_out;
  int tile = a->tile;
  if (tile == SSDE_TILE_AUTO) {
    if (a->c_out <= 32) tile = SSDE_TILE_256x32;
    else {
      const int nt = ssde_cdiv(a->c_out, 64);
      if (ssde_cdiv(M, 256) * nt >= 512) tile = SSDE_TILE_256x64;
      else if (ssde_cdiv(M, 128) * nt >= 384) tile = SSDE_TILE_128x64;
      else tile = SSDE_TILE_64x64;
    }
    if (a->w_out * a->h_out * a->n < kTiles[tile].bm && tile != SSDE_TILE_256x32) tile = SSDE_TILE_64x64;
  }
  SSDE_REQUIRE(tile >= 1 && tile <= 4, "conv: bad tile id %d", tile);
  int lTW = 0, lTH = 0;
  pl->bkc = 8;
  const bool deep_ok = !(a->flags & SSDE_CONVF_BKC8);
  if (pl->has3) {
    while (true) {
      const int px = halo_px(kTiles[tile].bm, a->w_out, a->h_out, a->stride, 3, &lTW, &lTH);
      pl->bkc = (deep_ok && tile == SSDE_TILE_64x64 && px * (SSDE_CONV_BKC64 / 4) <= 5 * kThreads) ? SSDE_CONV_BKC64 : 8;
      if (px * 2 <= 5 * kThreads) break;
      SSDE_REQUIRE(tile != SSDE_TILE_64x64, "conv: halo too large for any tile");
      tile = (tile == SSDE_TILE_256x32) ? SSDE_TILE_64x64 : tile + 1;
    }
  } else {
    halo_px(kTiles[tile].bm, a->w_out, a->h_out, 1, 1, &lTW, &lTH);
  }
  const int bm = kTiles[tile].bm, bn = kTiles[tile].bn;
  const int tw = 1 << lTW, th = 1 << lTH, imgs = bm / (tw * th);

  ConvKParams& kp = pl->kp;
  kp.main = a->main; kp.aux = a->aux; kp.w_main = a->w_main; kp.w_aux = a->w_aux;
  ConvGeom& g = kp.g;
  g.N = a->n; g.Hin = a->h_in; g.Win = a->w_in; g.Hout = a->h_out; g.Wout = a->w_out;
  g.Cout = a->c_out; g.CoutPad = ssde_cdiv(a->c_out, 64) * 64;
  g.stride = pl->has3 ? a->stride : 1; g.pad = pl->has3 ? a->pad : 0;
  g.lTW = lTW; g.lTH = lTH;
  g.tiles_x = ssde_cdiv(a->w_out, tw);
  g.tiles_per_img = g.tiles_x * ssde_cdiv(a->h_out, th);
  g.m_tiles = ssde_cdiv(a->n, imgs) * g.tiles_per_img;
  g.n_tiles = ssde_cdiv(a->c_out, bn);
  ssde_fill_epilogue(kp, a);
  const bool gn_ok = a->c_out % 4 == 0 && (imgs == 1 || (g.tiles_per_img == 1 && tw * th >= kThreads / (bn / 4)));
  pl->gn_slices = gn_ok ? g.tiles_per_img * (kThreads / 64) : 0;
  SSDE_REQUIRE(!a->gn_part || pl->gn_slices > 0, "conv: GroupNorm partials need one image per tile and c_out %% 4 == 0");

  int lds = 0;
  if (pl->has3) {
    const int px = imgs * ((th - 1) * g.stride + 3) * ((tw - 1) * g.stride + 3);
    const int lda = pl->bkc + 4;
    lds = (((px * lda + 3) & ~3) + 9 * bn * lda) * 4;
  }
  if (pl->has1) {
    const int l1 = (bm * 36 + bn * 36) * 4;
    if (l1 > lds) lds = l1;
  }
  const int epi_bytes = bm * (bn + 4) * 4 + 16;
  pl->lds_bytes = lds > epi_bytes ? lds : epi_bytes;
  pl->tile = tile;
  const bool split_ok = !(a->flags & SSDE_CONVF_NO_KSPLIT);
  const int wgs = ssde_cdiv(g.m_tiles, 8) * 8 * g.n_tiles;
  const int ctot = pl->has3 ? a->main.c0 + a->main.c1 : 0;
  kp.ksplit = (split_ok && pl->has3 && tile == SSDE_TILE_64x64 && wgs <= 320 && ctot >= 128 && a->c_out % 4 == 0 &&
               a->resid != a->dst && g.m_tiles * g.n_tiles <= kSyncSlots / 4) ? 2 : 1;
  kp.sync = nullptr;
  pl->grid = wgs * kp.ksplit;
  return SSDE_OK;
}

template <int WM, int WN, int TM, int TN, int BKC3 = 8>
int launch_cfg(ConvPlan& pl, hipStream_t st) {
  dim3 grid(pl.grid), block(kThreads);
  if (pl.kp.ksplit == 2) {
    pl.kp.sync = ssde_conv_sync_slots(pl.kp.g.m_tiles * pl.kp.g.n_tiles);
    SSDE_REQUIRE(pl.kp.sync, "conv: no hand-over slots for a split reduction");
  }
  if (pl.has3 && pl.has1) return ssde_launch_lds<conv_mfma_kernel<WM, WN, TM, TN, true, true, BKC3>>("conv", grid, block, pl.lds_bytes, st, pl.kp);
  if (pl.has3) return ssde_launch_lds<conv_mfma_kernel<WM, WN, TM, TN, true, false, BKC3>>("conv", grid, block, pl.lds_bytes, st, pl.kp);
  return ssde_launch_lds<conv_mfma_kernel<WM, WN, TM, TN, false, true, BKC3>>("conv", grid, block, pl.lds_bytes, st, pl.kp);
}

int direct_plan(const ssde_conv_args* a, ssde_conv_plan* out) {
  ConvPlan pl;
  if (int rc = make_plan(a, &pl)) return rc;
  *out = ssde_conv_plan{pl.lds_bytes, pl.gn_slices, 0};
  return SSDE_OK;
}

int direct_launch(const ssde_conv_args* a, hipStream_t st) {
  ConvPlan pl;
  if (int rc = make_plan(a, &pl)) return rc;
  switch (pl.tile) {
    case SSDE_TILE_256x64: return launch_cfg<4, 1, 2, 2>(pl, st);
    case SSDE_TILE_128x64: return launch_cfg<4, 1, 1, 2>(pl, st);
    case SSDE_TILE_64x64:  return pl.bkc == 8 ? launch_cfg<2, 2, 1, 1>(pl, st) : launch_cfg<2, 2, 1, 1, SSDE_CONV_BKC64>(pl, st);
    case SSDE_TILE_256x32: return launch_cfg<4, 1, 2, 1>(pl, st);
  }
  ssde_set_error("conv: unreachable tile %d", pl.tile);
  return SSDE_EINVAL;
}

template <int TILE> bool wants_tile(const ssde_conv_args* a) { return a->tile == TILE; }
const ssde_conv_route kRoutes[] = {
    {"f2", wants_tile<SSDE_TILE_WINOGRAD>, ssde_conv_wino_plan, ssde_conv_wino_launch, false},
    {"f4", wants_tile<SSDE_TILE_WINOGRAD4>, ssde_conv_wino4_plan, ssde_conv_wino4_launch, false},
    {"f4r", wants_tile<SSDE_TILE_WINOGRAD4R>, ssde_conv_wino4r_plan, ssde_conv_wino4r_launch, false},
    {"f4p", wants_tile<SSDE_TILE_WINOGRAD4P>, ssde_conv_wino4p_plan, ssde_conv_wino4p_launch, false},
    {"1x1", [](const ssde_conv_args* a) { return a->dst && ssde_conv1x1_wants(a); }, ssde_conv1x1_plan, ssde_conv1x1_launch, true},
    {"small", [](const ssde_conv_args* a) { return a->dst && ssde_conv_small_wants(a); }, ssde_conv_small_plan, ssde_conv_small_launch, true},
    {"direct", [](const ssde_conv_args*) { return true; }, direct_plan, direct_launch, true},
};

const ssde_conv_route* route_of(const ssde_conv_args* a) {
  const ssde_conv_route* r = kRoutes + sizeof(kRoutes) / sizeof(kRoutes[0]) - 1;
  if (!a) return r;
  for (r = kRoutes; !r->wants(a); ++r) {}
  if (a->pad_end != 0 && !r->takes_pad_end) {
    ssde_set_error("conv: pad_end %d with Winograd tile %d (end padding runs on the direct kernel only)", a->pad_end, a->tile);
    return nullptr;
  }
  return r;
}

}

unsigned* ssde_conv_sync_slots(int need) {
  static std::atomic<unsigned> cursor{0};
  if (need <= 0 || need > kSyncSlots / 4) return nullptr;
  unsigned cur = cursor.load(std::memory_order_relaxed), at, next;
  do {
    at = cur % (unsigned)kSyncSlots;
    if (at + (unsigned)need > (unsigned)kSyncSlots) at = 0;
    next = at + (unsigned)need;
  } while (!cursor.compare_exchange_weak(cur, next, std::memory_order_relaxed));
  unsigned* base = nullptr;
  if (hipGetSymbolAddress(reinterpret_cast<void**>(&base), HIP_SYMBOL(g_conv_sync)) != hipSuccess) return nullptr;
  return base + 2 * (size_t)at;
}

extern "C" int ssde_conv2d(const ssde_conv_args* a, void* stream) {
  const ssde_conv_route* r = route_of(a);
  if (!r) return SSDE_EINVAL;
  if (a && a->gn_in_part0 && !ssde_wino4_xform_merges_gn(a)) {
    const ssde_src& s = a->main;
    SSDE_REQUIRE(s.gn_mean && s.gn_rstd && s.gn_groups > 0 && a->ksize != 0, "conv: gn_in_part0 needs a k x k main source with a GroupNorm prologue");
    ssde_gn_finalize_args f;
    f.part0 = a->gn_in_part0; f.part1 = s.c1 > 0 ? a->gn_in_part1 : nullptr;
    f.c0 = s.c0; f.c1 = s.c1; f.slices0 = a->gn_in_slices0; f.slices1 = s.c1 > 0 ? a->gn_in_slices1 : 0;
    f.n = a->n; f.groups = s.gn_groups; f.eps = a->gn_in_eps;
    f.mean = const_cast<float*>(s.gn_mean); f.rstd = const_cast<float*>(s.gn_rstd);
    if (int rc = ssde_gn_finalize(&f, stream)) return rc;
  }
  if (a && a->tile == SSDE_TILE_WINOGRAD4R && !(a->flags & SSDE_CONVF_V_GIVEN)) {
    ssde_conv_plan pl;
    if (int rc = r->plan(a, &pl)) return rc;
    if (int rc = ssde_wino4_xform_vq_launch(a, stream)) return rc;
  }
  return r->launch(a, static_cast<hipStream_t>(stream));
}

extern "C" int ssde_conv_gn_slices(const ssde_conv_args* a) {
  if (!a || a->c_out % 4 != 0) return 0;
  ssde_conv_args q = *a;
  q.gn_part = nullptr;
  const ssde_conv_route* r = route_of(&q);
  ssde_conv_plan pl;
  return r && r->plan(&q, &pl) == SSDE_OK ? pl.gn_slices : 0;
}

extern "C" int64_t ssde_conv_ws_floats(const ssde_conv_args* a) {
  const ssde_conv_route* r = route_of(a);
  if (!r) return SSDE_EINVAL;
  ssde_conv_plan pl = {0, 0, 0};
  const int rc = r->plan(a, &pl);
  return rc && a && a->tile == SSDE_TILE_WINOGRAD4P ? rc : pl.ws_floats;
}

extern "C" int ssde_conv_lds_bytes(const ssde_conv_args* a) {
  const ssde_conv_route* r = route_of(a);
  ssde_conv_plan pl;
  if (int rc = r ? r->plan(a, &pl) : SSDE_EINVAL) return rc;
  return pl.lds_bytes;
}
```

### score_sde_pytorch_amd/engine.py

```python
import ctypes as C
import math
import os
from typing import Callable, NamedTuple

import numpy as np
import torch

from . import _lib as L

_FLT = 4
INV_SQRT2 = float(1.0 / np.sqrt(2.0))

FC_OTHER, FC_CONV3, FC_CONV1, FC_ATTN, FC_GN, FC_FIR = 0, 1, 2, 3, 4, 5

W4P_MIN_BATCH = 16


class Buf:
    __slots__ = ("shape", "numel", "name", "persistent", "tensor", "first", "last")

    def __init__(self, shape, name="", persistent=False):
        self.shape = tuple(int(s) for s in shape)
        self.numel = int(np.prod(self.shape))
        self.name = name
        self.persistent = persistent
        self.tensor = None
        self.first = None
        self.last = None


def _walk_refs(value, fn):
    if isinstance(value, Buf):
        fn(value)
    elif isinstance(value, tuple) and len(value) == 2 and isinstance(value[0], Buf):
        fn(value[0])
    elif isinstance(value, dict):
        for v in value.values():
            _walk_refs(v, fn)
    elif isinstance(value, list):
        for v in value:
            _walk_refs(v, fn)


def _ptr(value):
    if value is None:
        return None
    off = 0
    if isinstance(value, tuple):
        value, off = value
    t = value.tensor if isinstance(value, Buf) else value
    assert t is not None, "buffer without storage"
    return t.data_ptr() + off * _FLT


def _fill(struct, fields):
    for k, v in fields.items():
        if k.startswith("_"):
            continue
        cur = getattr(struct, k)
        if isinstance(v, dict):
            _fill(cur, v)
        elif isinstance(v, (list, tuple)) and not (len(v) == 2 and isinstance(v[0], (Buf, torch.Tensor))):
            for i, x in enumerate(v):
                if isinstance(x, dict):
                    _fill(cur[i], x)
                else:
                    cur[i] = x
        elif isinstance(v, (Buf, torch.Tensor, tuple)) or v is None:
            setattr(struct, k, _ptr(v))
        else:
            setattr(struct, k, v)


_ROUTE = {L.OP_CONV: L.conv_route_flags, L.OP_WGRAD: L.wgrad_route_flags, L.OP_GN_BWD_REDUCE: L.gn_bwd_route_flags,
          L.OP_ATTN: L.attn_route_flags}


class ProgramBuilder:
    def __init__(self, device):
        self.device = device
        self.specs = []
        self.keep = []
        self.fir_taps = {}

    def buf(self, *shape, name="", persistent=False):
        return Buf(shape, name, persistent)

    def tensor(self, t):
        self.keep.append(t)
        return t

    def add(self, kind, fields, fclass=FC_OTHER, flops=0.0):
        self.specs.append((kind, fields, fclass, float(flops)))

    def extend(self, other):
        self.specs.extend(other.specs)
        self.keep.extend(other.keep)

    def finalize(self):
        bufs = {}
        fused_fir = _fir_pairs(self.specs)
        for i, (_, fields, _, _) in enumerate(self.specs):
            def mark(b, i=i):
                if b.first is None:
                    b.first = i
                b.last = i
                bufs[id(b)] = b
            _walk_refs(fields, mark)
            if fused_fir.get(i) is not None:
                _walk_refs({"dst2": fused_fir[i]}, mark)
        by_first, by_last = {}, {}
        for b in bufs.values():
            by_first.setdefault(b.first, []).append(b)
            by_last.setdefault(b.last, []).append(b)
        free, blocks = [], []
        for i in range(len(self.specs)):
            for b in by_first.get(i, []):
                if b.tensor is not None:
                    continue
                need = (b.numel + 1023) // 1024 * 1024
                if b.persistent:
                    b.tensor = torch.zeros(need, dtype=torch.float32, device=self.device)
                    blocks.append(b.tensor)
                    continue
                best = None
                for j, t in enumerate(free):
                    if t.numel() >= need and (best is None or t.numel() < free[best].numel()):
                        best = j
                if best is not None and free[best].numel() <= 2 * need:
                    b.tensor = free.pop(best)
                else:
                    b.tensor = torch.zeros(need, dtype=torch.float32, device=self.device)
                    blocks.append(b.tensor)
            for b in by_last.get(i, []):
                if not b.persistent:
                    free.append(b.tensor)
        self.blocks = blocks
        self.arena_bytes = sum(t.numel() for t in blocks) * _FLT
        ops, classes, flops, starts = [], [], [], []
        for si, (kind, fields, fclass, fl) in enumerate(self.specs):
            starts.append(len(ops))
            if si in fused_fir:
                if fused_fir[si] is None:
                    continue
                fields = dict(fields, dst2=fused_fir[si])
            for sub_fields, sub_class, sub_fl in _expand(kind, fields, fclass, fl):
                args = L.ARGS[kind]()
                _fill(args, sub_fields)
                if kind in _ROUTE and "flags" not in sub_fields:
                    args.flags = _ROUTE[kind]()
                ops.append(L.make_op(kind, args, sub_class))
                classes.append(sub_class)
                flops.append(sub_fl)
        prog = Program(L.op_array(ops), classes, flops, self)
        prog.spec_start = starts + [len(ops)]
        return prog


def _fir_pairs(specs):
    out = {}
    if os.environ.get("SSDE_FUSE_FIR", "1") == "0":
        return out
    same = ("n", "h_in", "w_in", "c", "h_out", "w_out", "up", "down", "pad0", "pad1", "kh", "kw", "k")
    for i in range(len(specs) - 1):
        (k0, f0, _, _), (k1, f1, _, _) = specs[i], specs[i + 1]
        if k0 != L.OP_UPFIRDN or k1 != L.OP_UPFIRDN or i in out:
            continue
        s0, s1 = f0["src"], f1["src"]
        if s0["p0"] is not s1["p0"] or s0["p1"] is not s1["p1"] or s0["c0"] != s1["c0"] or s0["c1"] != s1["c1"]:
            continue
        if s0["pro_mode"] == L.PRO_NONE or s1["pro_mode"] != L.PRO_NONE or f0["dst"] is f1["dst"]:
            continue
        if f0.get("accumulate") or f1.get("accumulate") or any(f0[k] != f1[k] for k in same) or f0.get("taps") is not f1.get("taps"):
            continue
        out[i], out[i + 1] = f1["dst"], None
    return out


def _expand(kind, fields, fclass, fl):
    if kind != L.OP_CONV or fields.get("_split_tmp") is None:
        return [(fields, fclass, fl)]
    px = fields["n"] * fields["h_out"] * fields["w_out"]
    fl1 = 2.0 * px * (fields["aux"]["c0"] + fields["aux"]["c1"]) * fields["c_out"]
    a = dict(fields)
    a.update(aux=_NOSRC, w_aux=None, resid=None, resid_post=0, out_scale=1.0, dst=fields["_split_tmp"], gn_part=None)
    b = dict(fields)
    b.update(main=_NOSRC, w_main=None, ksize=0, bias=None, chan_add=None, chan_add_ld=0, resid=fields["_split_tmp"],
             resid_post=0, tile=L.TILE_AUTO, wino_v=None, gn_in_part0=None, gn_in_part1=None, gn_in_slices0=0, gn_in_slices1=0,
             wino_ws=None, wino_ws_floats=0)
    return [(a, fclass, fl - fl1), (b, FC_CONV1, fl1)]


class OpList(list):
    __slots__ = ("classes", "flops")


class Program:
    def __init__(self, ops, classes, flops, owner):
        self.ops, self.n = ops, len(ops)
        self.classes, self.flops = classes, flops
        self._owner = owner
        self._graph = None

    @classmethod
    def of(cls, parts, owner):
        ops, classes, flops = [], [], []
        for part in parts:
            if isinstance(part, Program):
                part = part[:]
            elif isinstance(part, L.Op):
                part = [part]
            ops.extend(part)
            classes.extend(getattr(part, "classes", None) or [FC_OTHER] * len(part))
            flops.extend(getattr(part, "flops", None) or [0.0] * len(part))
        return cls(L.op_array(ops), classes, flops, owner)

    def __getitem__(self, span):
        out = OpList(self.ops[span])
        out.classes, out.flops = self.classes[span], self.flops[span]
        return out

    def _at(self, start):
        return C.cast(C.byref(self.ops, start * C.sizeof(L.Op)), C.POINTER(L.Op))

    def _launch(self, ops_ptr, count, stream=None):
        lib = L.load()
        if not torch.cuda.is_available():
            raise RuntimeError("libssde_hip programs run on the MI355X only (no CPU fallback)")
        st = torch.cuda.current_stream().cuda_stream if stream is None else stream
        L.check(lib.ssde_program_run(ops_ptr, count, C.c_void_p(st)), "ssde_program_run")

    def run(self, stream=None):
        self._launch(self.ops, self.n, stream)

    def run_range(self, start, count, stream=None):
        assert 0 <= start and start + count <= self.n
        self._launch(self._at(start), count, stream)

    def run_range_timed(self, start, count):
        lib = L.load()
        ms = (C.c_float * count)()
        st = torch.cuda.current_stream().cuda_stream
        L.check(lib.ssde_program_run_timed(self._at(start), count, C.c_void_p(st), ms), "ssde_program_run_timed")
        return list(ms)

    def run_timed(self):
        return self.run_range_timed(0, self.n)

    def capture(self, stream):
        lib = L.load()
        h = C.c_void_p()
        L.check(lib.ssde_graph_capture(self.ops, self.n, C.c_void_p(stream.cuda_stream), C.byref(h)), "ssde_graph_capture")
        self._graph = h
        return h

    def replay(self, stream):
        L.check(L.load().ssde_graph_launch(self._graph, C.c_void_p(stream.cuda_stream)), "ssde_graph_launch")

    def replay_from_current(self, side, times=1):
        cur = torch.cuda.current_stream()
        apart = side.cuda_stream != cur.cuda_stream
        if apart:
            side.wait_stream(cur)
        if self._graph is None:
            self.capture(side)
        for _ in range(times):
            self.replay(side)
        if apart:
            cur.wait_stream(side)

    def __del__(self):
        if getattr(self, "_graph", None):
            try:
                L.load().ssde_graph_destroy(self._graph)
            except Exception:
                pass


class PinnedRing:

    def __init__(self, slots, length, dtype, pinned=None):
        pinned = torch.cuda.is_available() if pinned is None else pinned
        self.bufs = [torch.zeros(length, dtype=dtype, pin_memory=pinned) for _ in range(slots)]
        self.events = [None] * slots
        self.next = 0

    def upload(self, dst, write):
        i = self.next % len(self.bufs)
        self.next += 1
        if self.events[i] is not None:
            self.events[i].synchronize()
        write(self.bufs[i])
        dst.copy_(self.bufs[i], non_blocking=True)
        if dst.is_cuda:
            self.events[i] = self.events[i] or torch.cuda.Event()
            self.events[i].record(torch.cuda.current_stream(dst.device))


def pack_conv_weight(w):
    cout, cin, kh, kw = w.shape
    cin8, cpad, t = (cin + 7) // 8, (cout + 63) // 64 * 64, kh * kw
    full = torch.zeros(cin8 * 8, t, cpad, dtype=torch.float32, device=w.device)
    full[:cin, :, :cout] = w.detach().to(torch.float32).permute(1, 2, 3, 0).reshape(cin, t, cout)
    return full.reshape(cin8, 8, t, cpad).permute(0, 2, 3, 1).contiguous()


_WINO_G = torch.tensor([[1.0, 0.0, 0.0], [0.5, 0.5, 0.5], [0.5, -0.5, 0.5], [0.0, 0.0, 1.0]])


def pack_wino_weight(w):
    cout, cin = w.shape[0], w.shape[1]
    G = _WINO_G.to(w.device, torch.float32)
    u = torch.einsum("ak,ockl,bl->ocab", G, w.detach().to(torch.float32), G)
    c8, nt = (cin + 7) // 8, (cout + 63) // 64
    full = torch.zeros(nt * 64, c8 * 8, 16, dtype=torch.float32, device=w.device)
    full[:cout, :cin] = u.reshape(cout, cin, 16)
    full = full.reshape(nt, 64, c8, 4, 2, 16)
    co = torch.arange(64, device=w.device)
    out = torch.empty(c8, nt, 16, 4, 64, 2, dtype=torch.float32, device=w.device)
    for q in range(4):
        src = full[:, :, :, q]
        out[:, :, :, q, co ^ ((q & 1) << 4)] = src.permute(2, 0, 4, 1, 3)
    return out.contiguous()


_WINO4_G = torch.tensor([[1 / 4, 0, 0], [-1 / 6, -1 / 6, -1 / 6], [-1 / 6, 1 / 6, -1 / 6], [1 / 24, 1 / 12, 1 / 6],
                         [1 / 24, -1 / 12, 1 / 6], [0, 0, 1]], dtype=torch.float64)


def _wino4_u(w):
    cout, cin = w.shape[0], w.shape[1]
    G = _WINO4_G.to(w.device)
    u = torch.einsum("ak,ockl,bl->ocab", G, w.detach().to(torch.float64), G).to(torch.float32)
    full = torch.zeros((cout + 63) // 64 * 64, (cin + 3) // 4 * 4, 36, dtype=torch.float32, device=w.device)
    full[:cout, :cin] = u.reshape(cout, cin, 36)
    return full


def pack_wino4_weight(w):
    return _wino4_u(w).reshape(-1, 2, 32, (w.shape[1] + 3) // 4, 4, 9, 4).permute(3, 0, 6, 1, 5, 2, 4).contiguous()


def pack_wino4r_weight(w):
    c4, nt = (w.shape[1] + 3) // 4, (w.shape[0] + 63) // 64
    v = _wino4_u(w).reshape(nt, 2, 32, c4, 2, 2, 36)
    fp = v[..., :32].reshape(nt, 2, 32, c4, 2, 2, 8, 4).permute(3, 0, 6, 7, 4, 2, 1, 5).reshape(c4, nt, 8, 4 * 64 * 4)
    hp = v[..., 32:].permute(3, 0, 6, 1, 4, 2, 5).reshape(c4, nt, 8, 64 * 2)
    return torch.cat([fp, hp], dim=3).contiguous()


def pack_wino4p_weight(w):
    return _wino4_u(w).unflatten(1, (-1, 4)).permute(3, 1, 0, 2).contiguous()


def pack_matrix(w):
    return pack_conv_weight(w.reshape(w.shape[0], w.shape[1], 1, 1))


class Conv3Route(NamedTuple):
    name: str
    tile: int
    pack_kind: int
    pack: Callable
    takes_v: bool
    needs_ws: bool


DIRECT = Conv3Route("direct", L.TILE_AUTO, L.PACK_CONV3, pack_conv_weight, False, False)
F2 = Conv3Route("f2", L.TILE_WINOGRAD, L.PACK_WINO3, pack_wino_weight, False, False)
F4 = Conv3Route("f4", L.TILE_WINOGRAD4, L.PACK_WINO4, pack_wino4_weight, True, False)
F4R = Conv3Route("f4r", L.TILE_WINOGRAD4R, L.PACK_WINO4R, pack_wino4r_weight, True, False)
F4P = Conv3Route("f4p", L.TILE_WINOGRAD4P, L.PACK_WINO4P, pack_wino4p_weight, False, True)
CONV3_ROUTES = (DIRECT, F2, F4, F4R, F4P)


def conv3_route_of_tile(tile):
    return next((r for r in CONV3_ROUTES if r.tile == tile), DIRECT)


def wino4_v_floats(n, h, w, c):
    return 36 * n * (h // 4) * (w // 4) * c


class _Entry:
    __slots__ = ("packed", "sources", "fn", "stamp", "recipe")

    def __init__(self, packed, sources, fn, stamp, recipe):
        self.packed, self.sources, self.fn, self.stamp, self.recipe = packed, sources, fn, stamp, recipe


class WeightStore:

    def __init__(self, device):
        self.device = device
        self.entries = []
        self.meta = {}
        self._tables = None

    def add(self, sources, fn, meta=None, recipe=None):
        lazy = recipe is not None and self._on_device() and os.environ.get("SSDE_TORCH_PACK", "0") != "1"
        with torch.no_grad():
            if lazy:
                try:
                    shape = fn(*[torch.empty(s.shape, dtype=s.dtype, device="meta") for s in sources]).shape
                except Exception:
                    shape = fn(*[torch.zeros(s.shape, dtype=s.dtype) for s in sources]).shape
                packed = torch.zeros(tuple(shape), dtype=torch.float32, device=self.device)
            else:
                packed = fn(*[s.detach() for s in sources]).to(self.device).contiguous()
        self.entries.append(_Entry(packed, list(sources), fn, None if lazy else self._stamp(sources), recipe))
        if meta is not None:
            self.meta[id(packed)] = meta
        self._tables = None
        return packed

    def _on_device(self):
        return self.device.type == "cuda" if isinstance(self.device, torch.device) else str(self.device).startswith("cuda")

    def conv3(self, param, cin_pad=None, cout_pad=None, route=DIRECT):
        def logical(w):
            w = w.to(torch.float32)
            if cin_pad and w.shape[1] < cin_pad:
                w = torch.nn.functional.pad(w, (0, 0, 0, 0, 0, cin_pad - w.shape[1]))
            if cout_pad and w.shape[0] < cout_pad:
                w = torch.nn.functional.pad(w, (0, 0, 0, 0, 0, 0, 0, cout_pad - w.shape[0]))
            return w
        cout_l, cin_l = max(param.shape[0], cout_pad or 0), max(param.shape[1], cin_pad or 0)
        meta = dict(kind="conv3", sources=[param], logical=logical, dims=(cout_l, cin_l),
                    parts=[dict(param=param, row0=0, rows=param.shape[0], transpose=False)], cin_store=param.shape[1])
        recipe = [dict(kind=route.pack_kind, src=param, cout=param.shape[0], cin=param.shape[1], cout_l=cout_l, cin_l=cin_l, flags=0, n="dst")]
        return self.add([param], lambda w: route.pack(logical(w)), meta, recipe)

    def matrix(self, parts, cin_pad=None):
        params = [p for p, _ in parts]

        def logical(*ws):
            ms = []
            for w, (_, tr) in zip(ws, parts):
                w = w.to(torch.float32)
                w = w.t() if tr else w.reshape(w.shape[0], -1)
                ms.append(w)
            m = torch.cat(ms, dim=0) if len(ms) > 1 else ms[0]
            if cin_pad and m.shape[1] < cin_pad:
                m = torch.nn.functional.pad(m, (0, cin_pad - m.shape[1]))
            return m
        rows, desc = 0, []
        for p_, tr in parts:
            n_rows = p_.shape[1] if tr else p_.shape[0]
            cin = p_.shape[0] if tr else int(np.prod(p_.shape[1:]))
            desc.append(dict(param=p_, row0=rows, rows=n_rows, transpose=tr))
            rows += n_rows
        meta = dict(kind="matrix", sources=params, logical=logical, parts=desc, cin_store=cin,
                    dims=(rows, max(cin, cin_pad or 0)))
        recipe = [dict(kind=L.PACK_MATRIX, src=d["param"], cout=d["param"].shape[0], cin=int(np.prod(d["param"].shape[1:])),
                       cout_l=rows, cin_l=0, flags=int(d["transpose"]), r_off=d["row0"], c_off=0, n="src") for d in desc]
        return self.add(params, lambda *ws: pack_matrix(logical(*ws)), meta, recipe)

    def vector(self, params, mode="cat", pad_to=None):
        def fn(*vs):
            vs = [v.to(torch.float32) for v in vs]
            x = torch.cat(vs) if mode == "cat" else sum(vs[1:], vs[0])
            if pad_to and x.numel() < pad_to:
                x = torch.nn.functional.pad(x, (0, pad_to - x.numel()))
            return x.clone()
        off, desc = 0, []
        for p_ in params:
            desc.append(dict(param=p_, off=0 if mode == "sum" else off, n=p_.numel()))
            off += p_.numel()
        if mode == "sum":
            assert len(params) == 2
            recipe = [dict(kind=L.PACK_VECTOR, src=params[0], src2=params[1], r_off=0, n="src")]
        else:
            recipe = [dict(kind=L.PACK_VECTOR, src=d["param"], r_off=d["off"], n="src") for d in desc]
        return self.add(params, fn, dict(kind="vector", mode=mode, sources=list(params), parts=desc), recipe)

    def derived(self, packed, route=None):
        meta = self.meta[id(packed)]
        key = (id(packed), route)
        if key not in self.meta:
            cout_l, cin_l = meta["dims"]
            if meta["kind"] == "conv3":
                p_ = meta["sources"][0]
                fn = lambda w: route.pack(w.permute(1, 0, 2, 3).flip(2, 3))
                recipe = [dict(kind=route.pack_kind, src=p_, cout=p_.shape[0], cin=p_.shape[1],
                               cout_l=cin_l, cin_l=cout_l, flags=1, n="dst")]
            else:
                fn = lambda m: pack_matrix(m.t().contiguous())
                recipe = [dict(kind=L.PACK_MATRIX, src=d["param"], cout=d["param"].shape[0], cin=int(np.prod(d["param"].shape[1:])),
                               cout_l=cin_l, cin_l=0, flags=int(not d["transpose"]), r_off=0, c_off=d["row0"], n="src")
                          for d in meta["parts"]]
            self.meta[key] = self.add(meta["sources"], lambda *ws: fn(meta["logical"](*ws)), None, recipe)
        return self.meta[key]

    def _source_addresses(self):
        return tuple(s.data_ptr() for e in self.entries if e.recipe is not None for s in e.sources)

    def _build_tables(self):
        descs = {}
        for e in self.entries:
            packed, recipe = e.packed, e.recipe
            if recipe is None:
                continue
            for r in recipe:
                d = L.PackDesc()
                src = r["src"]
                d.src, d.dst, d.kind = src.data_ptr(), packed.data_ptr(), r["kind"]
                d.src2 = r["src2"].data_ptr() if r.get("src2") is not None else None
                d.cout, d.cin = r.get("cout", 0), r.get("cin", 0)
                d.cout_l, d.cin_l, d.flags = r.get("cout_l", 0), r.get("cin_l", 0), r.get("flags", 0)
                d.r_off, d.c_off = r.get("r_off", 0), r.get("c_off", 0)
                d.n = packed.numel() if r["n"] == "dst" else src.numel()
                descs.setdefault(r["kind"], []).append(d)
        tables = []
        for kind, ds in sorted(descs.items()):
            arr = (L.PackDesc * len(ds))(*ds)
            raw = torch.frombuffer(bytearray(bytes(arr)), dtype=torch.uint8).to(self.device)
            args = L.PackArgs()
            args.table, args.count, args.kind, args.max_n = raw.data_ptr(), len(ds), kind, max(int(x.n) for x in ds)
            tables.append((args, raw))
        self._tables = (tables, self._source_addresses())

    def pack_tables(self):
        if self._tables is None or self._tables[1] != self._source_addresses():
            self._build_tables()
        return self._tables[0]

    def pack_ops(self):
        return [L.make_op(L.OP_PACK, args) for args, _ in self.pack_tables()]

    def device_refresh(self):
        from . import hipops
        tables = self.pack_tables()
        lib = L.load()
        for args, _ in tables:
            L.check(lib.ssde_pack_weights(C.byref(args), hipops._stream()), "ssde_pack_weights")
        return bool(tables)

    @staticmethod
    def _stamp(sources):
        return tuple((s.data_ptr(), s._version, getattr(getattr(s, "_ssde_flat", None), "generation", 0)) for s in sources)

    def mark_fresh(self):
        for e in self.entries:
            st = self._stamp(e.sources)
            if e.recipe is None and st != e.stamp:
                self._torch_pack(e)
            e.stamp = st

    def _torch_pack(self, e):
        with torch.no_grad():
            e.packed.copy_(e.fn(*[s.detach() for s in e.sources]).to(self.device))

    def refresh(self, force=False, on_device=None):
        if on_device is None:
            on_device = self._on_device()
        stamps = [self._stamp(e.sources) for e in self.entries]
        stale = [force or st != e.stamp for e, st in zip(self.entries, stamps)]
        done_on_device = on_device and any(old and e.recipe is not None for e, old in zip(self.entries, stale)) and self.device_refresh()
        for e, st, old in zip(self.entries, stamps, stale):
            if old and not (done_on_device and e.recipe is not None):
                self._torch_pack(e)
            e.stamp = st


def _src(t, c, t2=None, c2=0, pro=L.PRO_NONE, gn=None, drop=None):
    d = dict(p0=t, p1=t2, c0=c, c1=c2, pro_mode=pro, gn_groups=0, gn_mean=None, gn_rstd=None, gn_gamma=None, gn_beta=None,
             drop_thresh=0, drop_scale=1.0, drop_seed=None, drop_salt=0)
    if gn is not None:
        d.update(gn_groups=gn["groups"], gn_mean=gn["mean"], gn_rstd=gn["rstd"], gn_gamma=gn["gamma"], gn_beta=gn["beta"])
        d["_gn"] = gn
    if drop is not None:
        p, seed_t, salt = drop
        d.update(drop_thresh=min(int(round(p * 2.0 ** 32)), 2 ** 32 - 1), drop_scale=1.0 / (1.0 - p), drop_seed=seed_t,
                 drop_salt=salt & 0xFFFFFFFF)
    return d


_NOSRC = dict(p0=None, p1=None, c0=0, c1=0, pro_mode=0, gn_groups=0, gn_mean=None, gn_rstd=None, gn_gamma=None, gn_beta=None,
              drop_thresh=0, drop_scale=1.0, drop_seed=None, drop_salt=0)


def fir_taps(k, gain=1.0):
    k = np.asarray(k, dtype=np.float32)
    if k.ndim == 1:
        k = np.outer(k, k)
    k = k / np.sum(k)
    return (k * gain).astype(np.float32)


class Lowering:

    def __init__(self, builder, weights, batch):
        self.b, self.w, self.n = builder, weights, batch
        self.parts = {}
        dev = getattr(builder, "device", None)
        self.cus = 256
        if os.environ.get("SSDE_NUM_CUS"):
            self.cus = int(os.environ["SSDE_NUM_CUS"])
        elif dev is not None and torch.device(dev).type == "cuda" and torch.cuda.is_available():
            self.cus = int(torch.cuda.get_device_properties(torch.device(dev)).multi_processor_count)

    def _gn_slices(self, fields):
        if os.environ.get("SSDE_GN_FUSE", "1") == "0":
            return 0
        return int(L.load().ssde_conv_gn_slices(C.byref(self._query_args(fields))))

    def _query_args(self, fields, last=True):
        sub = _expand(L.OP_CONV, fields, 0, 0.0)[-1 if last else 0][0]
        a = L.ConvArgs()
        dummy = 0x1000
        for src_name in ("main", "aux"):
            src, dst = sub[src_name], getattr(a, src_name)
            dst.p0 = dummy if src["p0"] is not None else None
            dst.p1 = dummy if src["p1"] is not None else None
            dst.c0, dst.c1, dst.pro_mode, dst.gn_groups = src["c0"], src["c1"], src["pro_mode"], src["gn_groups"]
            if src["gn_groups"]:
                dst.gn_mean = dst.gn_rstd = dst.gn_gamma = dst.gn_beta = dummy
            if src["drop_thresh"]:
                dst.drop_thresh, dst.drop_seed = src["drop_thresh"], dummy
        a.w_main = dummy if sub["w_main"] is not None else None
        a.w_aux = dummy if sub["w_aux"] is not None else None
        for k in ("n", "h_in", "w_in", "h_out", "w_out", "c_out", "ksize", "stride", "pad", "tile"):
            setattr(a, k, sub[k])
        a.pad_end = sub.get("pad_end", 0)
        a.dst = dummy
        a.flags = sub.get("flags", L.conv_route_flags())
        return a

    def gn_stats(self, t, c, hw, gn_module, t2=None, c2=0):
        ctot = c + c2
        groups = gn_module.num_groups
        mean = self.b.buf(self.n, groups, name="gn_mean")
        rstd = self.b.buf(self.n, groups, name="gn_rstd")
        p0, p1 = self.parts.get(id(t)), (self.parts.get(id(t2)) if t2 is not None else None)
        if p0 is not None and p0[2] == c and (t2 is None or (p1 is not None and p1[2] == c2)) and (ctot // groups) % 4 == 0:
            fin = dict(part0=p0[0], part1=p1[0] if p1 else None, c0=c, c1=c2, slices0=p0[1], slices1=p1[1] if p1 else 0,
                       n=self.n, groups=groups, eps=float(gn_module.eps), mean=mean, rstd=rstd)
            gamma = self.w.vector([gn_module.weight])
            beta = self.w.vector([gn_module.bias])
            assert ctot == gn_module.num_channels
            gn = dict(groups=groups, mean=mean, rstd=rstd, gamma=gamma, beta=beta, pending=fin)
            if os.environ.get("SSDE_GN_MERGE_IN_CONSUMER", "0") != "1":
                self._materialize_stats(gn)
            return gn
        slices = max(1, min(int(math.ceil(256 / self.n)), hw // 64)) if hw >= 128 else 1
        scratch = self.b.buf(self.n * slices * groups * 2, name="gn_scratch") if slices > 1 else None
        self.b.add(L.OP_GN_STATS, dict(p0=t, p1=t2, c0=c, c1=c2, n=self.n, hw=hw, groups=groups, eps=float(gn_module.eps),
                                       mean=mean, rstd=rstd, scratch=scratch, slices=slices), FC_GN)
        gamma = self.w.vector([gn_module.weight])
        beta = self.w.vector([gn_module.bias])
        assert ctot == gn_module.num_channels
        return dict(groups=groups, mean=mean, rstd=rstd, gamma=gamma, beta=beta, narrow=(ctot // groups) % 4 != 0)

    def src(self, t, c, hw, t2=None, c2=0, pro=L.PRO_NONE, gn=None, drop=None):
        if not (gn is not None and gn.get("narrow")) and not (t2 is not None and c % 32 != 0):
            return _src(t, c, t2, c2, pro=pro, gn=gn, drop=drop)
        self._materialize_stats(gn)
        ctot = c + c2
        dst = self.b.buf(self.n, hw, ctot, name="gn_applied")
        self.b.add(L.OP_GN_APPLY, dict(src=_src(t, c, t2, c2, pro=pro, gn=gn, drop=drop), n=self.n, hw=hw, dst=dst), FC_GN)
        return _src(dst, ctot)

    def _materialize_stats(self, gn, fields=None):
        fin = gn.get("pending") if gn else None
        if fin is None:
            return
        gn["pending"] = None
        if fields is not None:
            fields.update(gn_in_part0=fin["part0"], gn_in_part1=fin["part1"], gn_in_slices0=fin["slices0"],
                          gn_in_slices1=fin["slices1"], gn_in_eps=fin["eps"])
        else:
            self.b.add(L.OP_GN_FINALIZE, fin, FC_GN)

    def conv(self, dst, h_out, w_out, c_out, main=None, w_main=None, h_in=0, w_in=0, stride=1, pad=1,
             aux=None, w_aux=None, bias=None, chan_add=None, chan_add_ld=0, resid=None, scale=1.0, resid_post=0, route=None,
             stats=False, pad_end=0):
        route = route or DIRECT
        assert route is DIRECT or (main is not None and stride == 1 and pad == 1 and pad_end == 0 and (h_in, w_in) == (h_out, w_out))
        split_tmp = self.b.buf(self.n, h_out, w_out, c_out, name="wino_tmp") if route is not DIRECT and aux is not None else None
        px = self.n * h_out * w_out
        flops = 0.0
        if main is not None:
            flops += 2.0 * px * 9 * (main["c0"] + main["c1"]) * c_out
        if aux is not None:
            flops += 2.0 * px * (aux["c0"] + aux["c1"]) * c_out
        fields = dict(
            main=main if main is not None else _NOSRC, aux=aux if aux is not None else _NOSRC,
            w_main=w_main, w_aux=w_aux, n=self.n, h_in=h_in, w_in=w_in, h_out=h_out, w_out=w_out, c_out=c_out,
            ksize=3 if main is not None else 0, stride=stride, pad=pad, pad_end=pad_end, tile=route.tile, bias=bias, chan_add=chan_add,
            chan_add_ld=chan_add_ld, resid_post=resid_post, resid=resid, out_scale=float(scale), dst=dst, gn_part=None,
            wino_v=None, _split_tmp=split_tmp)
        if route.takes_v:
            v_floats = wino4_v_floats(self.n, h_out, w_out, main["c0"] + main["c1"])
            takes = getattr(self, "emit_wino_v", False) and v_floats * 4 < 2 ** 32 and self._wgrad_takes_wino4(fields)
            if route is F4R or takes:
                fields["wino_v"] = self.b.buf(v_floats, name="wino_v")
                fields["_v_for_wgrad"] = bool(takes)
        if route.needs_ws:
            need = int(L.load().ssde_conv_ws_floats(C.byref(self._query_args(fields, last=False))))
            if need <= 0:
                raise L.SsdeError("conv(winograd 4x4, position-batched): %s" % L.load().ssde_last_error().decode())
            fields.update(wino_ws=self.b.buf(need, name="wino_ws"), wino_ws_floats=need)
        if aux is not None:
            self._materialize_stats(aux.get("_gn"))
        if main is not None:
            self._materialize_stats(main.get("_gn"), fields if route is F4R and h_in * w_in >= 64 else None)
        if stats and isinstance(dst, Buf):
            slices = self._gn_slices(fields)
            if slices > 0:
                part = self.b.buf(self.n, slices, c_out // 4, 3, name="gn_part")
                fields["gn_part"] = part
                self.parts[id(dst)] = (part, slices, c_out)
        self.b.add(L.OP_CONV, fields, FC_CONV3 if main is not None else FC_CONV1, flops)

    def _wino4_two_kernels(self, h, w, c_out, c_in):
        return os.environ.get("SSDE_WINO4_TWO", "2") != "0" and wino4_v_floats(self.n, h, w, c_in) * 4 < 2 ** 32 and c_in % 8 == 0

    def _wgrad_takes_wino4(self, f):
        if os.environ.get("SSDE_WINO_V_FROM_FORWARD", "1") == "0":
            return False
        meta = self.w.meta.get(id(f["w_main"]))
        if meta is None or len(meta["parts"]) != 1 or meta["parts"][0]["transpose"]:
            return False
        a = L.WgradArgs()
        s = f["main"]
        a.src.c0, a.src.c1, a.src.pro_mode, a.src.gn_groups = s["c0"], s["c1"], s["pro_mode"], s["gn_groups"]
        a.g_ld, a.g_off = f["c_out"], meta["parts"][0]["row0"]
        a.n, a.h_in, a.w_in, a.h_out, a.w_out = f["n"], f["h_in"], f["w_in"], f["h_out"], f["w_out"]
        a.c_out, a.ksize, a.stride, a.pad = meta["parts"][0]["rows"], 3, f["stride"], f["pad"]
        a.pad_end = f.get("pad_end", 0)
        a.cin_store, a.transpose_out = meta["cin_store"], 0
        a.flags = L.wgrad_route_flags()
        return bool(L.load().ssde_wgrad_wants_winograd4(C.byref(a)))

    def conv3_route(self, h, w, c_out, c_in, aux=False):
        mode = os.environ.get("SSDE_WINOGRAD", "1")
        if mode == "0":
            return DIRECT
        if mode == "1" and h == 4 and w == 4 and not aux and c_in % 32 == 0 and c_out % 64 == 0 and self.n >= W4P_MIN_BATCH:
            return F4P
        legal2 = h % 2 == 0 and w % 2 == 0 and h >= 8 and w >= 8 and c_out >= 32 and c_in >= 8 and c_in % 8 == 0
        legal4 = h % 4 == 0 and w % 4 == 0 and h >= 8 and w >= 8 and c_out >= 32 and c_in >= 8 and c_in % 4 == 0
        two = lambda: self._wino4_two_kernels(h, w, c_out, c_in)
        if mode == "4" and legal4:
            return F4R if two() else F4
        if mode == "2" or mode == "4":
            return F2 if legal2 else DIRECT
        n_tiles = -(-c_out // 64)
        if mode != "3" and legal4 and h >= 16 and w >= 16 and -(-(self.n * h * w) // 512) * n_tiles >= self.cus:
            return F4R if two() else F4
        if mode != "3" and legal4 and c_in % 16 == 0 and c_in >= 256 and c_out % 4 == 0 and os.environ.get("SSDE_CONV_KSPLIT", "1") != "0":
            wgs4 = -(-(-(-(self.n * h * w) // 512)) // 8) * 8 * n_tiles
            if self.cus // 2 < wgs4 * 2 <= self.cus and two():
                return F4R
            if c_in % 32 == 0 and self.cus // 2 < wgs4 * 4 <= self.cus and two():
                return F4R
        return F2 if legal2 and -(-(self.n * h * w) // 256) * n_tiles >= self.cus // 2 else DIRECT

    def upfirdn(self, src, n_ch, h_in, w_in, taps, up=1, down=1, pad=(0, 0), name="fir"):
        kh, kw = taps.shape
        h_out = (h_in * up + pad[0] + pad[1] - kh) // down + 1
        w_out = (w_in * up + pad[0] + pad[1] - kw) // down + 1
        dst = self.b.buf(self.n, h_out, w_out, n_ch, name=name)
        self._materialize_stats(src.get("_gn"))
        self.b.add(L.OP_UPFIRDN, dict(src=src, n=self.n, h_in=h_in, w_in=w_in, c=n_ch, h_out=h_out, w_out=w_out,
                                      up=up, down=down, pad0=pad[0], pad1=pad[1], dst=dst, **self.fir_kernel_fields(taps)), FC_FIR)
        return dst, h_out, w_out

    def fir_kernel_fields(self, taps):
        taps = np.ascontiguousarray(taps, dtype=np.float32)
        kh, kw = taps.shape
        if not (1 <= kh <= L.FIR_MAX_TAPS and 1 <= kw <= L.FIR_MAX_TAPS):
            raise ValueError("upfirdn2d: a %dx%d kernel (fir_kernel of %d taps); at most %d taps per axis"
                             % (kh, kw, max(kh, kw), L.FIR_MAX_TAPS))
        k16, t = [0.0] * 16, None
        if kh <= 4 and kw <= 4:
            k16[:kh * kw] = [float(v) for v in taps.reshape(-1).tolist()]
        else:
            key = (kh, kw, taps.tobytes())
            t = self.b.fir_taps.get(key)
            if t is None:
                t = self.b.fir_taps[key] = self.b.tensor(torch.from_numpy(taps.copy()).to(self.b.device))
        return dict(kh=kh, kw=kw, k=k16, taps=t)


def fir_pads(n_taps, up=False, conv=1):
    p = n_taps - 2 + (conv - 1)
    return ((p + 1) // 2 + (1 if up else 0), p // 2)


class UNetEngine:

    def __init__(self, model, batch, height, width, device, vp_score=False, train=False, input_grad=False,
                 finalize=True):
        L.load()
        self.train, self.input_grad = train, input_grad
        self.model, self.n, self.h, self.w, self.device = model, batch, height, width, device
        cfg = model.config
        self.cfg = cfg
        self.b = ProgramBuilder(device)
        self.weights = WeightStore(device)
        self.low = Lowering(self.b, self.weights, batch)
        self.low.emit_wino_v = bool(getattr(self, "param_grads", False))
        self.channels = model.channels
        self.x_in = self.b.buf(batch, self.channels, height, width, name="x_in", persistent=True)
        self.cond = self.b.buf(batch, name="cond", persistent=True)
        self.sig = self.b.buf(batch, name="sigma", persistent=True) \
            if (model.embedding_type == "positional" and cfg.model.scale_by_sigma) else self.cond
        self.out = self.b.buf(batch, self.channels, height, width, name="out", persistent=True)
        self.vp_score = vp_score
        self.std = self.b.buf(batch, name="std", persistent=True) if vp_score else None
        if vp_score and cfg.model.scale_by_sigma:
            raise NotImplementedError("scale_by_sigma together with a VP score head is not lowered")
        self.drop_seed = None
        if train and float(cfg.model.dropout) > 0:
            self.drop_seed = torch.zeros(1, dtype=torch.int32, device=device)
            self.b.tensor(self.drop_seed)
        self._n_res = 0
        self._emb = self._tproj = None
        self._lower()
        if finalize:
            self.program = self.b.finalize()

    @property
    def cond_only_ops(self):
        return int(self.program.spec_start[getattr(self, "_cond_specs", 0)])

    def _lower(self):
        idx = self._lower_cond()
        body = {"ncsnpp": self._lower_ncsnpp, "ddpm": self._lower_ddpm}[getattr(self.model, "family", "ncsnpp")]
        o, hh, ww = body(idx)
        mode = 2 if self.vp_score else (1 if self.cfg.model.scale_by_sigma else 0)
        vec = self.std if mode == 2 else (self.sig if mode == 1 else None)
        self.b.add(L.OP_TO_NCHW, dict(src=o, dst=self.out, n=self.n, c=self.channels, h=hh, w=ww, c_src=4, mode=mode, v=vec))

    def _lower_cond(self):
        model, b, low, n = self.model, self.b, self.low, self.n
        mods = list(model.all_modules)
        nf = model.nf
        idx = 0
        if not model.conditional and getattr(model, "family", "ncsnpp") == "ddpm":
            self._cond_specs = 0
            self.cond.tensor = torch.zeros((n + 1023) // 1024 * 1024, dtype=torch.float32, device=self.device)
            return idx

        if model.embedding_type == "fourier":
            emb_dim = 2 * nf
            table = self.weights.add([mods[idx].W], lambda w: w.to(torch.float32).clone()); idx += 1
            kind = 0
        else:
            emb_dim = nf
            half = nf // 2
            e = math.log(10000) / (half - 1)
            freqs = torch.exp(torch.arange(half, dtype=torch.float32) * -e)
            table = b.tensor(freqs.to(self.device))
            kind = 1
        emb = b.buf(n, emb_dim, name="emb", persistent=True)
        self._emb = emb
        b.add(L.OP_EMBED, dict(cond=self.cond, w=table, dst=emb, n=n, dim=emb_dim, kind=kind))
        temb = None
        if model.conditional:
            lin0, lin1 = mods[idx], mods[idx + 1]; idx += 2
            t0 = b.buf(n, 4 * nf, name="temb0", persistent=True)
            low.conv(t0, 1, 1, 4 * nf, aux=_src(emb, emb_dim), w_aux=self.weights.matrix([(lin0.weight, False)]),
                     bias=self.weights.vector([lin0.bias]))
            temb = b.buf(n, 4 * nf, name="temb", persistent=True)
            low.conv(temb, 1, 1, 4 * nf, aux=_src(t0, 4 * nf, pro=L.PRO_SILU),
                     w_aux=self.weights.matrix([(lin1.weight, False)]),
                     bias=self.weights.vector([lin1.bias]))
            dense = [m.Dense_0 for m in mods if getattr(m, "kind", "") == "res"]
            self._tproj_off, off = {}, 0
            for d in dense:
                self._tproj_off[id(d)] = off
                off += d.out_features
            self._tproj_ld = off
            wd = self.weights.matrix([(d.weight, False) for d in dense])
            bd = self.weights.vector([d.bias for d in dense])
            self._tproj = b.buf(n, off, name="tproj", persistent=True)
            low.conv(self._tproj, 1, 1, off, aux=_src(temb, 4 * nf, pro=L.PRO_SILU), w_aux=wd, bias=bd)
        self._cond_specs = len(b.specs)
        return idx

    def _lower_input(self, conv_in):
        b, n, nf = self.b, self.n, self.model.nf
        H, W = self.h, self.w
        cpad = 4
        x0 = b.buf(n, H, W, cpad, name="x_nhwc")
        self._x0 = x0
        a, sh = (1.0, 0.0) if self.cfg.data.centered else (2.0, -1.0)
        b.add(L.OP_TO_NHWC, dict(src=self.x_in, dst=x0, n=n, c=self.channels, h=H, w=W, c_pad=cpad, a=a, b=sh))
        h = b.buf(n, H, W, nf, name="h0")
        self.low.conv(h, H, W, nf, main=_src(x0, cpad), w_main=self._w3(conv_in, cin_pad=cpad), h_in=H, w_in=W,
                      bias=self._bias(conv_in), stats=True)
        return h

    def _lower_head(self, gn_m, conv_m, h, cur_c, hh, ww):
        gn = self.low.gn_stats(h, cur_c, hh * ww, gn_m)
        o = self.b.buf(self.n, hh, ww, 4, name="head")
        self.low.conv(o, hh, ww, 4, main=self.low.src(h, cur_c, hh * ww, pro=L.PRO_GN_SILU, gn=gn), w_main=self._w3(conv_m, cout_pad=4),
                      h_in=hh, w_in=ww, bias=self._bias(conv_m, pad_to=4))
        return o

    def _lower_ncsnpp(self, idx):
        model, b, low, n = self.model, self.b, self.low, self.n
        mods = list(model.all_modules)
        nf = model.nf
        skip_scale = INV_SQRT2 if model.skip_rescale else 1.0
        fir, fk = model.fir, model.fir_kernel
        H, W = self.h, self.w
        cpad = 4
        h = self._lower_input(mods[idx]); idx += 1
        x0 = self._x0
        pyr, pyr_c = (x0, cpad) if model.progressive_input != "none" else (None, 0)
        hs = [(h, nf, H, W)]
        cur_c = nf

        def is_attn(res):
            return res in model.attn_resolutions

        for lvl in range(model.num_resolutions):
            for _ in range(model.num_res_blocks):
                t, c, hh, ww = hs[-1]
                h, cur_c = self._res(mods[idx], t, c, hh, ww); idx += 1
                if is_attn(ww):
                    h = self._attn(mods[idx], h, cur_c, hh, ww); idx += 1
                hs.append((h, cur_c, hh, ww))
            if lvl != model.num_resolutions - 1:
                t, c, hh, ww = hs[-1]
                h, cur_c = self._res(mods[idx], t, c, hh, ww); idx += 1
                hh, ww = hh // 2, ww // 2
                if model.progressive_input == "input_skip":
                    taps = fir_taps(fk) if fir else fir_taps([1, 1])
                    pd = fir_pads(taps.shape[0])
                    pyr, _, _ = low.upfirdn(_src(pyr, pyr_c), pyr_c, hh * 2, ww * 2, taps, down=2, pad=pd, name="pyr_down")
                    comb = mods[idx]; idx += 1
                    if comb.method != "sum":
                        raise NotImplementedError("progressive_combine='cat' is not lowered (no shipped config uses it)")
                    hn = b.buf(n, hh, ww, cur_c, name="combine")
                    low.conv(hn, hh, ww, cur_c, aux=_src(pyr, pyr_c), w_aux=self._w1(comb.Conv_0, cin_pad=pyr_c),
                             bias=self._bias(comb.Conv_0), resid=h, scale=1.0, stats=True)
                    h = hn
                elif model.progressive_input == "residual":
                    down = mods[idx]; idx += 1
                    if not fir:
                        raise NotImplementedError("progressive_input='residual' without FIR is not lowered")
                    pf, ph, pw = low.upfirdn(_src(pyr, pyr_c), pyr_c, hh * 2, ww * 2, fir_taps(fk), pad=fir_pads(len(fk), conv=3),
                                             name="pyr_fir")
                    hn = b.buf(n, hh, ww, cur_c, name="pyr")
                    low.conv(hn, hh, ww, cur_c, main=_src(pf, pyr_c), w_main=self._w3(down.Conv2d_0, cin_pad=pyr_c),
                             h_in=ph, w_in=pw, stride=2, pad=0, bias=self._bias(down.Conv2d_0), resid=h, scale=skip_scale,
                             stats=True)
                    pyr, pyr_c, h = hn, cur_c, hn
                hs.append((h, cur_c, hh, ww))

        t, c, hh, ww = hs[-1]
        h, cur_c = self._res(mods[idx], t, c, hh, ww); idx += 1
# ... 212 lines not shown
```

### score_sde_pytorch_amd/plan_export.py

```python
import bisect
import ctypes as C
import struct

import torch

from . import _lib as L
from . import engine as E

MAGIC = b"SSDEPLN1"
REGION_ZERO, REGION_CONST = 0, 1
RELOC_OP, RELOC_REFRESH_OP, RELOC_REGION = 0, 1, 2
PLAN_UNET, PLAN_PC, PLAN_TRAIN, PLAN_ODE, PLAN_LIKELIHOOD = 0, 1, 2, 3, 4
IO_X, IO_COND, IO_SIGMA, IO_STD, IO_OUT, IO_XMEAN, IO_STEP, IO_SEED = range(8)
(IO_BATCH, IO_Z, IO_A, IO_S, IO_G2, IO_LOSS, IO_HYPER, IO_DROP_SEED, IO_GOUT, IO_GX, IO_GRAD, IO_PARAMS) = range(8, 20)
IO_ODE_DYN, IO_ODE_K, IO_ODE_STATE, IO_ODE_PROBE = range(20, 24)
IO_SLOTS = 24
ODE_PARTIALS = 1024
ODE_METHODS = {"RK45": 0, "RK23": 1, "DOP853": 2}


class PlanHeader(C.Structure):
    _fields_ = [("magic", C.c_char * 8), ("abi_version", C.c_int32), ("sizeof_op", C.c_int32),
                ("n_regions", C.c_int32), ("n_ops", C.c_int32), ("n_refresh_ops", C.c_int32), ("n_relocs", C.c_int32),
                ("n_params", C.c_int32), ("kind", C.c_int32),
                ("batch", C.c_int32), ("channels", C.c_int32), ("height", C.c_int32), ("width", C.c_int32),
                ("nfe_per_iteration", C.c_int32), ("sde_steps", C.c_int32), ("io", C.c_int32 * IO_SLOTS), ("seg", C.c_int32 * 4),
                ("n_flat", C.c_int64), ("data_bytes", C.c_int64)]


class PlanRegion(C.Structure):
    _fields_ = [("bytes", C.c_int64), ("data_offset", C.c_int64), ("kind", C.c_int32), ("_pad0", C.c_int32), ("name", C.c_char * 32)]


class PlanReloc(C.Structure):
    _fields_ = [("target_kind", C.c_int32), ("target", C.c_int32), ("byte_offset", C.c_int64), ("region", C.c_int32),
                ("_pad0", C.c_int32), ("offset", C.c_int64)]


class PlanParam(C.Structure):
    _fields_ = [("name", C.c_char * 96), ("region", C.c_int32), ("_pad0", C.c_int32), ("offset", C.c_int64), ("numel", C.c_int64)]


_op_pointer_offsets = L._op_pointer_offsets


class _Regions:

    def __init__(self):
        self.by_ptr, self.list = {}, []

    def add(self, t, kind, name):
        if t is None:
            return None
        st = t.untyped_storage()
        key = st.data_ptr()
        if key in self.by_ptr:
            r = self.list[self.by_ptr[key]]
            r["kind"] = max(r["kind"], kind)
            return self.by_ptr[key]
        self.by_ptr[key] = len(self.list)
        self.list.append(dict(ptr=key, bytes=st.nbytes(), kind=kind, name=name, keep=t))
        return len(self.list) - 1

    def freeze(self):
        self._starts = sorted((r["ptr"], i) for i, r in enumerate(self.list))
        self._keys = [s for s, _ in self._starts]

    def find(self, addr):
        i = bisect.bisect_right(self._keys, addr) - 1
        if i >= 0:
            rid = self._starts[i][1]
            r = self.list[rid]
            if r["ptr"] <= addr <= r["ptr"] + r["bytes"]:
                return rid, addr - r["ptr"]
        raise ValueError("plan export: pointer 0x%x lies in no known tensor" % addr)

    def data(self, rid):
        r = self.list[rid]
        t = r["keep"]
        flat = torch.empty(0, dtype=torch.uint8).set_(t.untyped_storage().cpu() if t.is_cuda else t.untyped_storage())
        return bytes(flat.numpy().tobytes())


def _collect_unet(regions, eng):
    for i, blk in enumerate(eng.b.blocks):
        regions.add(blk, REGION_ZERO, "arena%d" % i)
    for i, t in enumerate(eng.b.keep):
        regions.add(t, REGION_CONST, "table%d" % i)
    for i, e in enumerate(eng.weights.entries):
        regions.add(e.packed, REGION_CONST, "packed%d" % i)
        for s in e.sources:
            regions.add(s.detach(), REGION_CONST, "param")
    for i, (_, raw) in enumerate(eng.weights.pack_tables()):
        regions.add(raw, REGION_CONST, "packtab%d" % i)


def _emit(kind, regions, ops, n_ops, eng_unet, model, io_tensors, batch, shape, nfe, sde_steps, seg=(0, 0, 0, 0), n_flat=0):
    regions.freeze()
    relocs = []

    def relocate(raw, offsets, target_kind, index, base=0):
        for off, addr in L.pointers_at(raw, offsets, base):
            relocs.append((target_kind, index, off) + regions.find(addr))
            struct.pack_into("<Q", raw, off, 0)
        return raw

    op_bytes = bytearray()
    for i in range(n_ops):
        op_bytes += relocate(bytearray(bytes(ops[i])), _op_pointer_offsets(int(ops[i].kind)), RELOC_OP, i)
    refresh = bytearray()
    tables = eng_unet.weights.pack_tables()
    desc_ptrs = L.pointer_offsets(L.PackDesc)
    table_patches = {}
    for j, ((args, raw_t), op) in enumerate(zip(tables, eng_unet.weights.pack_ops())):
        refresh += relocate(bytearray(bytes(op)), _op_pointer_offsets(L.OP_PACK), RELOC_REFRESH_OP, j)
        tid, toff0 = regions.find(raw_t.data_ptr())
        tb = bytearray(regions.data(tid))
        for d in range(int(args.count)):
            relocate(tb, desc_ptrs, RELOC_REGION, tid, toff0 + d * C.sizeof(L.PackDesc))
        table_patches[tid] = bytes(tb)
    params = []
    for name, p in model.named_parameters():
        try:
            rid, roff = regions.find(p.data_ptr())
        except ValueError:
            continue
        params.append((name, rid, roff, p.numel()))
    data = bytearray()
    reg_structs = []
    for rid, r in enumerate(regions.list):
        rs = PlanRegion()
        rs.bytes, rs.kind, rs.name = r["bytes"], r["kind"], r["name"].encode()[:31]
        rs.data_offset = -1
        if r["kind"] == REGION_CONST:
            while len(data) % 16:
                data.append(0)
            rs.data_offset = len(data)
            data += table_patches.get(rid) or regions.data(rid)
        reg_structs.append(rs)
    hdr = PlanHeader()
    hdr.magic, hdr.abi_version, hdr.sizeof_op = MAGIC, L.ABI_VERSION, C.sizeof(L.Op)
    hdr.n_regions, hdr.n_ops, hdr.n_refresh_ops, hdr.n_relocs, hdr.n_params = len(reg_structs), n_ops, len(tables), len(relocs), len(params)
    hdr.kind, hdr.batch = kind, batch
    hdr.channels, hdr.height, hdr.width = shape
    hdr.nfe_per_iteration, hdr.sde_steps = nfe, sde_steps
    for k in range(4):
        hdr.seg[k] = int(seg[k])
    hdr.n_flat = int(n_flat)
    for slot in range(IO_SLOTS):
        t = io_tensors.get(slot)
        hdr.io[slot] = -1
        if t is not None:
            rid, roff = regions.find(t.data_ptr())
            assert roff == 0, "plan I/O tensors must start their storage"
            hdr.io[slot] = rid
    hdr.data_bytes = len(data)
    out = bytearray(bytes(hdr))
    for rs in reg_structs:
        out += bytes(rs)
    out += op_bytes + refresh
    for tk, tgt, boff, rid, roff in relocs:
        q = PlanReloc()
        q.target_kind, q.target, q.byte_offset, q.region, q.offset = tk, tgt, boff, rid, roff
        out += bytes(q)
    for name, rid, roff, numel in params:
        q = PlanParam()
        q.name, q.region, q.offset, q.numel = name.encode()[:95], rid, roff, numel
        out += bytes(q)
    out += data
    return bytes(out)


def export_unet_plan(eng):
    eng.weights.refresh()
    regions = _Regions()
    _collect_unet(regions, eng)
    io = {IO_X: eng.x_in.tensor, IO_COND: eng.cond.tensor, IO_OUT: eng.out.tensor}
    if eng.sig is not eng.cond:
        io[IO_SIGMA] = eng.sig.tensor
    if eng.std is not None:
        io[IO_STD] = eng.std.tensor
    return _emit(PLAN_UNET, regions, eng.program.ops, eng.program.n, eng, eng.model, io, eng.n, (eng.channels, eng.h, eng.w), 1, 0)


def export_pc_plan(sampler, with_rng=True):
    eng = sampler.unet
    eng.weights.refresh()
    prog = sampler.step_program(with_rng=with_rng)
    regions = _Regions()
    _collect_unet(regions, eng)
    for name in ("x_mean", "z_c", "z_p", "gss", "zss", "step", "seed_word", "proj_data", "proj_mask", "z_pc", "z_pp"):
        t = getattr(sampler, name, None)
        if t is not None:
            regions.add(t, REGION_ZERO, name)
    for k, t in sampler.tabs.items():
        regions.add(t, REGION_CONST, "tab_" + k)
    io = {IO_X: eng.x_in.tensor, IO_COND: eng.cond.tensor, IO_OUT: eng.out.tensor, IO_XMEAN: sampler.x_mean,
          IO_STEP: sampler.step, IO_SEED: sampler.seed_word}
    if eng.std is not None:
        io[IO_STD] = eng.std.tensor
    B, Cc, H, W = sampler.shape
    return _emit(PLAN_PC, regions, prog.ops, prog.n, eng, sampler.model, io, B, (Cc, H, W), sampler.nfe_per_step(), sampler.sde.N)


def export_train_plan(fs, optimizer=None, ema=None):
    eng = fs.eng
    eng.weights.refresh()
    regions = _Regions()
    _collect_unet(regions, eng)
    regions.add(fs.flat.data, REGION_CONST, "flat_params")
    regions.add(fs.flat.grad, REGION_ZERO, "flat_grad")
    for name in ("z", "batch", "a", "s", "g2", "losses", "loss", "hyper", "gnorm", "partial"):
        regions.add(getattr(fs, name), REGION_ZERO, name)
    parts = [fs._head[0], eng.program[:eng.n_fwd], fs._head[1], eng.program[eng.n_fwd:]]
    seg0 = fs._head[0].n
    seg1 = seg0 + eng.n_fwd
    seg2 = seg1 + fs._head[1].n
    seg3 = 0
    if optimizer is not None:
        m, v = optimizer.flatten_like(fs.flat)
        regions.add(m, REGION_CONST, "adam_m")
        regions.add(v, REGION_CONST, "adam_v")
        if ema is not None:
            regions.add(ema.flatten_like(fs.flat), REGION_CONST, "ema")
        seg3 = seg2 + eng.program.n - eng.n_fwd
        parts.append(fs._optimizer_program(optimizer, ema))
    prog = E.Program.of(parts, fs)
    io = {IO_X: eng.x_in.tensor, IO_COND: eng.cond.tensor, IO_OUT: eng.out.tensor, IO_BATCH: fs.batch, IO_Z: fs.z, IO_A: fs.a,
          IO_S: fs.s, IO_LOSS: fs.loss, IO_HYPER: fs.hyper, IO_GOUT: eng.gout.tensor, IO_GRAD: fs.flat.grad, IO_PARAMS: fs.flat.data}
    if fs.spec["likelihood_weighting"]:
        io[IO_G2] = fs.g2
    if eng.sig is not eng.cond:
        io[IO_SIGMA] = eng.sig.tensor
    if eng.std is not None:
        io[IO_STD] = eng.std.tensor
    if eng.drop_seed is not None:
        io[IO_DROP_SEED] = eng.drop_seed
    if eng.gx is not None:
        io[IO_GX] = eng.gx.tensor
    return _emit(PLAN_TRAIN, regions, prog.ops, prog.n, eng, fs.model, io, eng.n, (eng.channels, eng.h, eng.w), 1, 0,
                 seg=(seg0, seg1, seg2, seg3), n_flat=fs.flat.numel)


def export_ode_plan(rhs, method="RK45"):
    from . import ode
# ... 176 lines not shown
```

Baseline: 5.691 images/s.

## Pre-split 1x1 GEMM weights into bf16 planes for inference x6 path

Adds a weight-pack kind that stores matrix weights already split into three bf16 planes in a tile-friendly layout. The 1x1 GEMM kernels (both the pipelined and plain bf16x6 variants) read those planes directly instead of loading fp32 weights and calling split3 on every tile. This removes per-tile weight splitting arithmetic and cuts the fp32 weight traffic, at the cost of extra kernel instantiations and another packed copy of each weight. It is enabled only for inference plans and skipped where the GN wide tile would be chosen. Plan export changes so that sliced parameter views are stored correctly.

Result: no change. 5.694 images/s, median of 3 (+0.0%).

```diff
diff --git a/include/ssde.h b/include/ssde.h
--- a/include/ssde.h
+++ b/include/ssde.h
@@ -76,7 +76,8 @@
        SSDE_CONVF_X6_WIDE = 512u,
        SSDE_CONVF_X6_NO_WIDE = 1024u,
        SSDE_CONVF_KSPLIT2 = 2048u,
-       SSDE_CONVF_KSPLIT4 = 4096u };
+       SSDE_CONVF_KSPLIT4 = 4096u,
+       SSDE_CONVF_X6_WPLANES = 8192u };
 enum { SSDE_TILE_AUTO = 0, SSDE_TILE_256x64 = 1, SSDE_TILE_128x64 = 2, SSDE_TILE_64x64 = 3, SSDE_TILE_256x32 = 4,
        SSDE_TILE_WINOGRAD = 5,
        SSDE_TILE_WINOGRAD4 = 6,
@@ -334,7 +335,8 @@
 enum { SSDE_PACK_CONV3 = 1, SSDE_PACK_WINO3 = 2, SSDE_PACK_MATRIX = 3, SSDE_PACK_VECTOR = 4,
        SSDE_PACK_WINO4 = 5 ,
        SSDE_PACK_WINO4R = 6 ,
-       SSDE_PACK_WINO4P = 7  };
+       SSDE_PACK_WINO4P = 7 ,
+       SSDE_PACK_MATRIX_X6 = 8 };
 typedef struct ssde_pack_desc {
   const float* src;
   const float* src2;
diff --git a/score_sde_pytorch_amd/_lib.py b/score_sde_pytorch_amd/_lib.py
--- a/score_sde_pytorch_amd/_lib.py
+++ b/score_sde_pytorch_amd/_lib.py
@@ -12,6 +12,7 @@
 TILES_WINOGRAD4 = (TILE_WINOGRAD4, TILE_WINOGRAD4R, TILE_WINOGRAD4P)
 CONVF_V_GIVEN, CONVF_BF16X6, CONVF_NO_KSPLIT, CONVF_BKC8, CONVF_GEMM_PIPE, CONVF_NO_GEMM_PIPE, CONVF_X6_BM64, CONVF_X6_PF2, \
     CONVF_NO_SMALL_COUT, CONVF_X6_WIDE, CONVF_X6_NO_WIDE, CONVF_KSPLIT2, CONVF_KSPLIT4 = 1, 2, 4, 8, 16, 32, 64, 128, 256, 512, 1024, 2048, 4096
+CONVF_X6_WPLANES = 8192
 WGRADF_DIRECT, WGRADF_F2, WGRADF_F4_FORCE, WGRADF_NO_STREAMK, WGRADF_NO_XCD_ORDER, WGRADF_1X1_CHUNKED, WGRADF_XVEC1 = 1, 2, 4, 8, 16, 32, 64
 GNBWDF_THREE_KERNELS, GNBWDF_DEFER_PARAMS = 1, 2
 (OP_CONV, OP_GN_STATS, OP_UPFIRDN, OP_ATTN, OP_EMBED, OP_TO_NHWC, OP_TO_NCHW, OP_BIAS_ACT, OP_SUMSQ,
@@ -24,6 +25,7 @@
 FINISH_JOBS = 16
 COLSUMF_DEFER = 1
 PACK_CONV3, PACK_WINO3, PACK_MATRIX, PACK_VECTOR, PACK_WINO4, PACK_WINO4R, PACK_WINO4P = 1, 2, 3, 4, 5, 6, 7
+PACK_MATRIX_X6 = 8
 
 _fp = C.c_void_p
 
@@ -308,9 +310,11 @@
 _lib = None
 
 
-def conv_route_flags(env=None):
+def conv_route_flags(env=None, planes=False):
     e = os.environ if env is None else env
     f = 0
+    if planes and e.get("SSDE_MATRIX", "").startswith("b") and e.get("SSDE_X6_WPLANES", "1") != "0":
+        f |= CONVF_X6_WPLANES
     if e.get("SSDE_MATRIX", "").startswith("b"):
         f |= CONVF_BF16X6
     if e.get("SSDE_CONV_KSPLIT", "1") == "0":
diff --git a/score_sde_pytorch_amd/csrc/backward.hip b/score_sde_pytorch_amd/csrc/backward.hip
--- a/score_sde_pytorch_amd/csrc/backward.hip
+++ b/score_sde_pytorch_amd/csrc/backward.hip
@@ -919,6 +919,20 @@
   }
 }
 
+__global__ __launch_bounds__(256) void pack_matrix_x6_kernel(const ssde_pack_desc* __restrict__ table) {
+  const ssde_pack_desc d = table[blockIdx.y];
+  const int ld = (d.cout_l + 63) / 64 * 64;
+  unsigned short* dst = reinterpret_cast<unsigned short*>(d.dst);
+  for (size_t idx = (size_t)blockIdx.x * 256 + threadIdx.x; idx < (size_t)d.n; idx += (size_t)gridDim.x * 256) {
+    const int i = (int)(idx / d.cin), j = (int)(idx % d.cin);
+    const int row = ((d.flags & 1) ? j : i) + d.r_off, col = ((d.flags & 1) ? i : j) + d.c_off;
+    uint2 q[3];
+    ssde_split3(make_float4(d.src[idx], 0.f, 0.f, 0.f), q[0], q[1], q[2]);
+#pragma unroll
+    for (int k = 0; k < 3; ++k) dst[(((size_t)(col >> 4) * 3 + k) * ld + row) * 16 + (col & 15)] = (unsigned short)(q[k].x & 0xffffu);
+  }
+}
+
 __global__ __launch_bounds__(256) void pack_vector_kernel(const ssde_pack_desc* __restrict__ table) {
   const ssde_pack_desc d = table[blockIdx.y];
   for (size_t idx = (size_t)blockIdx.x * 256 + threadIdx.x; idx < (size_t)d.n; idx += (size_t)gridDim.x * 256)
@@ -940,6 +954,7 @@
     case SSDE_PACK_WINO4R: hipLaunchKernelGGL(pack_wino4_kernel<1>, grid, dim3(256), 0, st, a->table); break;
     case SSDE_PACK_WINO4P: hipLaunchKernelGGL(pack_wino4_kernel<2>, grid, dim3(256), 0, st, a->table); break;
     case SSDE_PACK_MATRIX: hipLaunchKernelGGL(pack_matrix_kernel, grid, dim3(256), 0, st, a->table); break;
+    case SSDE_PACK_MATRIX_X6: hipLaunchKernelGGL(pack_matrix_x6_kernel, grid, dim3(256), 0, st, a->table); break;
     case SSDE_PACK_VECTOR: hipLaunchKernelGGL(pack_vector_kernel, grid, dim3(256), 0, st, a->table); break;
     default: ssde_set_error("pack_weights: unknown kind %d", a->kind); return SSDE_EINVAL;
   }
diff --git a/score_sde_pytorch_amd/csrc/conv1x1.hip b/score_sde_pytorch_amd/csrc/conv1x1.hip
--- a/score_sde_pytorch_amd/csrc/conv1x1.hip
+++ b/score_sde_pytorch_amd/csrc/conv1x1.hip
@@ -237,10 +237,11 @@
   static constexpr int NBW = kBN / 64;
 };
 
-template <bool kGn, int kBM, int kPF, int kBN = 128>
+template <bool kGn, int kBM, int kPF, int kBN = 128, bool kWP = false>
 __global__ __launch_bounds__(kThreads, kBN == 256 ? 2 : (kBM == 64 ? 4 : 3) - (kPF == 2 ? SSDE_X6_PF2_OCC_LOSS : 0)) void gemm1x1_bf16x6_kernel(const GemmParams p) {
   using X = X6<kBM, kBN>;
-  constexpr int NA = X::NA, NB = X::NBW, NBW = X::NBW, RS = 64;
+  constexpr int NA = X::NA, NB = kWP ? 0 : X::NBW, NBW = X::NBW, RS = 64;
+  constexpr int NW = kWP ? kBN / 128 : 0;
   SSDE_LDS(smem);
   char* lds = reinterpret_cast<char*>(smem);
   const int tid = threadIdx.x, wave = tid >> 6, lane = tid & 63;
@@ -273,14 +274,24 @@
     arow[i] = aok[i] ? m : 0;
     aimg[i] = arow[i] / p.HW;
   }
-  bool bok[NB];
+  bool bok[NB + 1];
 #pragma unroll
   for (int i = 0; i < NB; ++i) bok[i] = (n0 + r0 + i * RS) < p.CoutPad;
   const float* bptr = p.wpk + ((size_t)n0 + r0) * 8 + (f & 1) * 4;
+  const size_t wplane = (size_t)p.CoutPad * (XBK * 2);
+  bool wok[NW + 1];
+  const char* wptr[NW + 1];
+#pragma unroll
+  for (int j = 0; j < NW; ++j) {
+    const int row = n0 + (tid >> 1) + j * 128;
+    wok[j] = row < p.CoutPad;
+    wptr[j] = reinterpret_cast<const char*>(p.wpk) + (size_t)(wok[j] ? row : n0) * (XBK * 2) + (tid & 1) * 16;
+  }
 
   struct ARegs { float4 av[NA]; };
   struct StageRegs {
-    float4 bv[NB];
+    float4 bv[NB + 1];
+    uint4 wq[3 * NW + 1];
     float mu[NA], rs[NA];
     float4 gam, bet;
   };
@@ -296,10 +307,17 @@
   };
   auto load_rest = [&](int st, StageRegs& R) __attribute__((always_inline)) {
     const int c_cur = st * XBK + f * 4;
-    const int cin8 = min(st * 2 + (f >> 1), ncin8 - 1);
-    const float* bp = bptr + (size_t)cin8 * p.CoutPad * 8;
-#pragma unroll
-    for (int i = 0; i < NB; ++i) R.bv[i] = *reinterpret_cast<const float4*>(bp + (bok[i] ? i * RS * 8 : 0));
+    if constexpr (kWP) {
+#pragma unroll
+      for (int q = 0; q < 3; ++q)
+#pragma unroll
+        for (int j = 0; j < NW; ++j) R.wq[q * NW + j] = *reinterpret_cast<const uint4*>(wptr[j] + ((size_t)st * 3 + q) * wplane);
+    } else {
+      const int cin8 = min(st * 2 + (f >> 1), ncin8 - 1);
+      const float* bp = bptr + (size_t)cin8 * p.CoutPad * 8;
+#pragma unroll
+      for (int i = 0; i < NB; ++i) R.bv[i] = *reinterpret_cast<const float4*>(bp + (bok[i] ? i * RS * 8 : 0));
+    }
     R.gam = make_float4(1.f, 1.f, 1.f, 1.f); R.bet = make_float4(0.f, 0.f, 0.f, 0.f);
 #pragma unroll
     for (int i = 0; i < NA; ++i) { R.mu[i] = 0.f; R.rs[i] = 1.f; }
@@ -341,6 +359,11 @@
       *reinterpret_cast<uint2*>(d + X::kPlaneB) = q1;
       *reinterpret_cast<uint2*>(d + 2 * X::kPlaneB) = q2;
     }
+#pragma unroll
+    for (int q = 0; q < 3; ++q)
+#pragma unroll
+      for (int j = 0; j < NW; ++j)
+        *reinterpret_cast<uint4*>(buf + 3 * X::kPlaneA + q * X::kPlaneB + (tid + j * 256) * 16) = wok[j] ? R.wq[q * NW + j] : make_uint4(0u, 0u, 0u, 0u);
   };
 
   f32x16 acc[NA][NBW];
@@ -464,8 +487,9 @@
 constexpr int kSlabLd = 68;
 constexpr int kSlabFloats = 8 * kSlabLd;
 
-template <bool kGn, bool kX6>
+template <bool kGn, bool kX6, bool kWP = false>
 __global__ __launch_bounds__(kThreads, 2) void gemm1x1_pipe_kernel(const GemmParams p) {
+  static_assert(kX6 || !kWP, "weight planes exist for the bf16 split only");
   SSDE_LDS(smem);
   constexpr int kStageB = kX6 ? X6<128>::kStageBytes : kStage * 4;
   constexpr int KB = 16;
@@ -597,6 +621,10 @@
       bok[i] = (n0 + r0 + i * RS) < p.CoutPad;
     }
     const float* bptr = p.wpk + ((size_t)n0 + r0) * 8 + (f & 1) * 4;
+    const bool wok = (n0 + (tid >> 1)) < p.CoutPad;
+    const size_t wplane = (size_t)p.CoutPad * (KB * 2);
+    const char* wptr = reinterpret_cast<const char*>(p.wpk) + (size_t)(wok ? n0 + (tid >> 1) : n0) * (KB * 2) + (tid & 1) * 16;
+    uint4 wq[3];
     float4 av[NI], bv[NI];
     float mu[NI] = {0.f, 0.f}, rs[NI] = {1.f, 1.f};
     float4 gam = make_float4(1.f, 1.f, 1.f, 1.f), bet = make_float4(0.f, 0.f, 0.f, 0.f);
@@ -610,10 +638,15 @@
       const float* ap = base + (c_cur < p.K ? cthr : 0);
 #pragma unroll
       for (int i = 0; i < NI; ++i) av[i] = *reinterpret_cast<const float4*>(ap + (size_t)arow[i] * C);
-      const int cin8 = min(st * 2 + (f >> 1), ncin8 - 1);
-      const float* bp = bptr + (size_t)cin8 * p.CoutPad * 8;
-#pragma unroll
-      for (int i = 0; i < NI; ++i) bv[i] = *reinterpret_cast<const float4*>(bp + (bok[i] ? i * RS * 8 : 0));
+      if constexpr (kWP) {
+#pragma unroll
+        for (int q = 0; q < 3; ++q) wq[q] = *reinterpret_cast<const uint4*>(wptr + ((size_t)st * 3 + q) * wplane);
+      } else {
+        const int cin8 = min(st * 2 + (f >> 1), ncin8 - 1);
+        const float* bp = bptr + (size_t)cin8 * p.CoutPad * 8;
+#pragma unroll
+        for (int i = 0; i < NI; ++i) bv[i] = *reinterpret_cast<const float4*>(bp + (bok[i] ? i * RS * 8 : 0));
+      }
       if (kGn) {
         const int cg = c_cur < p.K ? c_cur : 0;
         gam = *reinterpret_cast<const float4*>(s.gn_gamma + cg);
@@ -627,6 +660,12 @@
       }
     };
     auto store_stage = [&](int st, char* buf) __attribute__((always_inline)) {
+      if constexpr (kWP) {
+        using X = X6<128>;
+#pragma unroll
+        for (int q = 0; q < 3; ++q)
+          *reinterpret_cast<uint4*>(buf + 3 * X::kPlaneA + q * X::kPlaneB + tid * 16) = wok ? wq[q] : make_uint4(0u, 0u, 0u, 0u);
+      }
       const int cin8 = st * 2 + (f >> 1), c_cur = st * KB + f * 4;
       const bool k_ok = c_cur < p.K;
 #pragma unroll
@@ -635,7 +674,9 @@
         if (aok[i] && k_ok)
           v = ssde_pro_apply(av[i], mu[i], rs[i], gam, bet, (uint32_t)arow[i] * (uint32_t)Ctot + (uint32_t)c_cur, pro);
         float4 w = make_float4(0.f, 0.f, 0.f, 0.f);
-        if (bok[i] && cin8 < ncin8) w = bv[i];
+        if constexpr (!kWP) {
+          if (bok[i] && cin8 < ncin8) w = bv[i];
+        }
         if constexpr (kX6) {
           using X = X6<128>;
           uint2 q0, q1, q2;
@@ -644,10 +685,12 @@
           *reinterpret_cast<uint2*>(d) = q0;
           *reinterpret_cast<uint2*>(d + X::kPlaneA) = q1;
           *reinterpret_cast<uint2*>(d + 2 * X::kPlaneA) = q2;
-          ssde_split3(w, q0, q1, q2);
-          *reinterpret_cast<uint2*>(d + 3 * X::kPlaneA) = q0;
-          *reinterpret_cast<uint2*>(d + 3 * X::kPlaneA + X::kPlaneB) = q1;
-          *reinterpret_cast<uint2*>(d + 3 * X::kPlaneA + 2 * X::kPlaneB) = q2;
+          if constexpr (!kWP) {
+            ssde_split3(w, q0, q1, q2);
+            *reinterpret_cast<uint2*>(d + 3 * X::kPlaneA) = q0;
+            *reinterpret_cast<uint2*>(d + 3 * X::kPlaneA + X::kPlaneB) = q1;
+            *reinterpret_cast<uint2*>(d + 3 * X::kPlaneA + 2 * X::kPlaneB) = q2;
+          }
         } else {
           float* fb = reinterpret_cast<float*>(buf);
           float* d = fb + (r0 + i * RS) * LDK + f * 4;
@@ -756,6 +799,7 @@
 struct GemmPlan {
   GemmParams p;
   bool gn, x6, pipe;
+  bool wplanes;
   int xbm, xpf, xbn;
   int grid;
 };
@@ -778,6 +822,8 @@
   p.lHW = ssde_ilog2(p.HW);
   p.gn_entries = p.HW >= 64 ? a->n * (p.HW / 64) : a->n;
   const bool x6 = g->x6 = (a->flags & SSDE_CONVF_BF16X6) != 0;
+  g->wplanes = (a->flags & SSDE_CONVF_X6_WPLANES) != 0;
+  SSDE_REQUIRE(!g->wplanes || x6, "conv1x1: SSDE_CONVF_X6_WPLANES (weights as bf16 planes) without SSDE_CONVF_BF16X6");
   {
     const int total = ssde_cdiv(p.m_tiles, 8) * 8 * p.n_tiles;
     const int wgs = (2 * ssde_num_cus() + 7) / 8 * 8;
@@ -835,6 +881,14 @@
   if (int rc = gemm_plan(a, &g, &pl)) return rc;
   const int lds = pl.lds_bytes;
   const bool gn = g.gn;
+  if (g.wplanes) {
+    if (g.pipe) return gn ? gemm_go<gemm1x1_pipe_kernel<true, true, true>>(g, lds, st) : gemm_go<gemm1x1_pipe_kernel<false, true, true>>(g, lds, st);
+    if (g.xbn == 256) return gn ? gemm_go<gemm1x1_bf16x6_kernel<true, 128, 1, 256, true>>(g, lds, st) : gemm_go<gemm1x1_bf16x6_kernel<false, 128, 1, 256, true>>(g, lds, st);
+    if (g.xbm == 128 && g.xpf == 1) return gn ? gemm_go<gemm1x1_bf16x6_kernel<true, 128, 1, 128, true>>(g, lds, st) : gemm_go<gemm1x1_bf16x6_kernel<false, 128, 1, 128, true>>(g, lds, st);
+    if (g.xbm == 128) return gn ? gemm_go<gemm1x1_bf16x6_kernel<true, 128, 2, 128, true>>(g, lds, st) : gemm_go<gemm1x1_bf16x6_kernel<false, 128, 2, 128, true>>(g, lds, st);
+    if (g.xpf == 1) return gn ? gemm_go<gemm1x1_bf16x6_kernel<true, 64, 1, 128, true>>(g, lds, st) : gemm_go<gemm1x1_bf16x6_kernel<false, 64, 1, 128, true>>(g, lds, st);
+    return gn ? gemm_go<gemm1x1_bf16x6_kernel<true, 64, 2, 128, true>>(g, lds, st) : gemm_go<gemm1x1_bf16x6_kernel<false, 64, 2, 128, true>>(g, lds, st);
+  }
   if (g.pipe) return gn ? gemm_go<gemm1x1_pipe_kernel<true, true>>(g, lds, st) : gemm_go<gemm1x1_pipe_kernel<false, true>>(g, lds, st);
   if (!g.x6) return gn ? gemm_go<gemm1x1_kernel<true>>(g, lds, st) : gemm_go<gemm1x1_kernel<false>>(g, lds, st);
   if (g.xbn == 256) return gn ? gemm_go<gemm1x1_bf16x6_kernel<true, 128, 1, 256>>(g, lds, st) : gemm_go<gemm1x1_bf16x6_kernel<false, 128, 1, 256>>(g, lds, st);
diff --git a/score_sde_pytorch_amd/csrc/conv_mfma.hip b/score_sde_pytorch_amd/csrc/conv_mfma.hip
--- a/score_sde_pytorch_amd/csrc/conv_mfma.hip
+++ b/score_sde_pytorch_amd/csrc/conv_mfma.hip
@@ -497,6 +497,10 @@
     ssde_set_error("conv: pad_end %d with Winograd tile %d (end padding runs on the direct kernel only)", a->pad_end, a->tile);
     return nullptr;
   }
+  if ((a->flags & SSDE_CONVF_X6_WPLANES) && r->plan != ssde_conv1x1_plan) {
+    ssde_set_error("conv: SSDE_CONVF_X6_WPLANES on the %s route (the bf16 plane image of a matrix weight is read by the 1x1 GEMM only)", r->name);
+    return nullptr;
+  }
   return r;
 }
 
diff --git a/score_sde_pytorch_amd/engine.py b/score_sde_pytorch_amd/engine.py
--- a/score_sde_pytorch_amd/engine.py
+++ b/score_sde_pytorch_amd/engine.py
@@ -149,6 +149,10 @@
                 _fill(args, sub_fields)
                 if kind in _ROUTE and "flags" not in sub_fields:
                     args.flags = _ROUTE[kind]()
+                    if kind == L.OP_CONV and sub_fields.get("_w_aux_x6") is not None and sub_fields["ksize"] == 0 and sub_fields["w_aux"] is not None:
+                        args.flags = L.conv_route_flags(planes=True)
+                        if args.flags & L.CONVF_X6_WPLANES:
+                            args.w_aux = _ptr(sub_fields["_w_aux_x6"])
                 ops.append(L.make_op(kind, args, sub_class))
                 classes.append(sub_class)
                 flops.append(sub_fl)
@@ -355,6 +359,23 @@
 
 def pack_matrix(w):
     return pack_conv_weight(w.reshape(w.shape[0], w.shape[1], 1, 1))
+
+
+def split3_bf16(m):
+    m = m.to(torch.float32).contiguous()
+    top = lambda x: x.view(torch.int32) & -65536
+    a = top(m)
+    r = m - a.view(torch.float32)
+    b = top(r)
+    c = top(r - b.view(torch.float32))
+    return [(p >> 16).to(torch.int16) for p in (a, b, c)]
+
+
+def pack_matrix_x6(w):
+    cout, cin = w.shape
+    m = torch.nn.functional.pad(w.to(torch.float32), (0, -cin % 16, 0, -cout % 64))
+    planes = torch.stack(split3_bf16(m), dim=0)
+    return planes.unflatten(2, (-1, 16)).permute(2, 0, 1, 3).contiguous().view(torch.float32)
 
 
 class Conv3Route(NamedTuple):
@@ -455,6 +476,17 @@
         recipe = [dict(kind=L.PACK_MATRIX, src=d["param"], cout=d["param"].shape[0], cin=int(np.prod(d["param"].shape[1:])),
                        cout_l=rows, cin_l=0, flags=int(d["transpose"]), r_off=d["row0"], c_off=0, n="src") for d in desc]
         return self.add(params, lambda *ws: pack_matrix(logical(*ws)), meta, recipe)
+
+    def matrix_planes(self, packed):
+        meta = self.meta[id(packed)]
+        assert meta["kind"] == "matrix"
+        key = (id(packed), "x6_planes")
+        if key not in self.meta:
+            recipe = [dict(kind=L.PACK_MATRIX_X6, src=d["param"], cout=d["param"].shape[0], cin=int(np.prod(d["param"].shape[1:])),
+                           cout_l=meta["dims"][0], cin_l=0, flags=int(d["transpose"]), r_off=d["row0"], c_off=0, n="src")
+                      for d in meta["parts"]]
+            self.meta[key] = self.add(meta["sources"], lambda *ws: pack_matrix_x6(meta["logical"](*ws)), None, recipe)
+        return self.meta[key]
 
     def vector(self, params, mode="cat", pad_to=None):
         def fn(*vs):
@@ -711,7 +743,25 @@
                 part = self.b.buf(self.n, slices, c_out // 4, 3, name="gn_part")
                 fields["gn_part"] = part
                 self.parts[id(dst)] = (part, slices, c_out)
+        if getattr(self, "x6_planes", False) and (main is None or split_tmp is not None) and w_aux is not None and id(w_aux) in self.w.meta:
+            fl = L.conv_route_flags(planes=True)
+            if aux["gn_groups"] and self._gemm_takes_wide_tile(px, c_out, aux["c0"] + aux["c1"], fl):
+                fl = 0
+            if fl & L.CONVF_X6_WPLANES and int(L.load().ssde_conv_lds_bytes(C.byref(self._query_args(dict(fields, flags=fl))))) > 0:
+                assert self.w.meta[id(w_aux)]["dims"][1] == aux["c0"] + aux["c1"]
+                fields["_w_aux_x6"] = self.w.matrix_planes(w_aux)
         self.b.add(L.OP_CONV, fields, FC_CONV3 if main is not None else FC_CONV1, flops)
+
+    def _gemm_takes_wide_tile(self, px, c_out, k, flags):
+        if c_out % 256 or flags & (L.CONVF_X6_NO_WIDE | L.CONVF_X6_BM64 | L.CONVF_X6_PF2):
+            return False
+        fills = -(-px // 128) * (c_out // 256) >= 2 * self.cus
+        if flags & L.CONVF_GEMM_PIPE:
+            return False
+        if not flags & L.CONVF_NO_GEMM_PIPE and k >= 512 and -(-px // 128) * -(-c_out // 128) > (2 * self.cus + 7) // 8 * 8 \
+                and not (c_out >= 512 and fills):
+            return False
+        return fills or bool(flags & L.CONVF_X6_WIDE)
 
     def _wino4_two_kernels(self, h, w, c_out, c_in):
         return os.environ.get("SSDE_WINO4_TWO", "2") != "0" and wino4_v_floats(self.n, h, w, c_in) * 4 < 2 ** 32 and c_in % 8 == 0
@@ -802,6 +852,7 @@
         self.weights = WeightStore(device)
         self.low = Lowering(self.b, self.weights, batch)
         self.low.emit_wino_v = bool(getattr(self, "param_grads", False))
+        self.low.x6_planes = not train and not input_grad and not getattr(self, "param_grads", False)
         self.channels = model.channels
         self.x_in = self.b.buf(batch, self.channels, height, width, name="x_in", persistent=True)
         self.cond = self.b.buf(batch, name="cond", persistent=True)
diff --git a/score_sde_pytorch_amd/plan_export.py b/score_sde_pytorch_amd/plan_export.py
--- a/score_sde_pytorch_amd/plan_export.py
+++ b/score_sde_pytorch_amd/plan_export.py
@@ -49,17 +49,17 @@
     def __init__(self):
         self.by_ptr, self.list = {}, []
 
-    def add(self, t, kind, name):
+    def add(self, t, kind, name, view=False):
         if t is None:
             return None
         st = t.untyped_storage()
-        key = st.data_ptr()
+        key, nbytes = (t.data_ptr(), t.numel() * t.element_size()) if view else (st.data_ptr(), st.nbytes())
         if key in self.by_ptr:
             r = self.list[self.by_ptr[key]]
             r["kind"] = max(r["kind"], kind)
             return self.by_ptr[key]
         self.by_ptr[key] = len(self.list)
-        self.list.append(dict(ptr=key, bytes=st.nbytes(), kind=kind, name=name, keep=t))
+        self.list.append(dict(ptr=key, bytes=nbytes, kind=kind, name=name, keep=t, view=view))
         return len(self.list) - 1
 
     def freeze(self):
@@ -78,6 +78,8 @@
     def data(self, rid):
         r = self.list[rid]
         t = r["keep"]
+        if r.get("view"):
+            return bytes(t.detach().contiguous().cpu().reshape(-1).view(torch.uint8).numpy().tobytes())
         flat = torch.empty(0, dtype=torch.uint8).set_(t.untyped_storage().cpu() if t.is_cuda else t.untyped_storage())
         return bytes(flat.numpy().tobytes())
 
@@ -90,7 +92,8 @@
     for i, e in enumerate(eng.weights.entries):
         regions.add(e.packed, REGION_CONST, "packed%d" % i)
         for s in e.sources:
-            regions.add(s.detach(), REGION_CONST, "param")
+            sliced = s.untyped_storage().nbytes() != s.numel() * s.element_size()
+            regions.add(s.detach(), REGION_CONST, "param", view=sliced and not (eng.train or eng.input_grad))
     for i, (_, raw) in enumerate(eng.weights.pack_tables()):
         regions.add(raw, REGION_CONST, "packtab%d" % i)
 
```
